# DJATOM/x265-aMod

Hardware: AMD Instinct MI355X
Metric: encoded frames/sec at 1080p & 2160p --preset medium; bit-exact vs CPU ref (higher is better)
Workload: dtype u8

## Files before the change

### include/x265amd.h

```cpp
#ifndef X265AMD_H
#define X265AMD_H

#include <stdint.h>
#include <stddef.h>

#ifdef __cplusplus
extern "C" {
#endif

#ifndef X265AMD_DEPTH
#define X265AMD_DEPTH 8
#endif
#if X265AMD_DEPTH > 8
typedef uint16_t x265amd_pixel;
#else
typedef uint8_t x265amd_pixel;
#endif

#define X265AMD_OK 0
#define X265AMD_EINVAL (-1)
#define X265AMD_EHIP (-2)
#define X265AMD_ENOMEM (-3)

int x265amd_bit_depth(void);
// ... 33 lines not shown
void x265amd_cpy2Dto1D_shr(int cu, int16_t* dst, const int16_t* src, intptr_t srcStride, int shift);
void x265amd_cpy1Dto2D_shl(int cu, int16_t* dst, const int16_t* src, intptr_t dstStride, int shift);
void x265amd_cpy1Dto2D_shr(int cu, int16_t* dst, const int16_t* src, intptr_t dstStride, int shift);
uint32_t x265amd_copy_cnt(int cu, int16_t* coeff, const int16_t* residual, intptr_t resiStride);
int x265amd_count_nonzero(int cu, const int16_t* quantCoeff);

void x265amd_dct(int cu, const int16_t* src, int16_t* dst, intptr_t srcStride);
void x265amd_lowpass_dct(int cu, const int16_t* src, int16_t* dst, intptr_t srcStride);
void x265amd_idct(int cu, const int16_t* src, int16_t* dst, intptr_t dstStride);
void x265amd_dst4x4(const int16_t* src, int16_t* dst, intptr_t srcStride);
void x265amd_idst4x4(const int16_t* src, int16_t* dst, intptr_t dstStride);
uint32_t x265amd_quant(const int16_t* coef, const int32_t* quantCoeff, int32_t* deltaU, int16_t* qCoef, int qBits, int add, int numCoeff);
uint32_t x265amd_nquant(const int16_t* coef, const int32_t* quantCoeff, int16_t* qCoef, int qBits, int add, int numCoeff);
void x265amd_dequant_normal(const int16_t* quantCoef, int16_t* coef, int num, int scale, int shift);
void x265amd_dequant_scaling(const int16_t* src, const int32_t* dequantCoef, int16_t* dst, int num, int mcqp_miper, int shift);

void x265amd_intra_pred(int cu, int mode, pixel_t_* dst, intptr_t dstStride, const pixel_t_* srcPix, int bFilter);
void x265amd_intra_filter(int cu, const pixel_t_* references, pixel_t_* filtered);
void x265amd_intra_allangs(int cu, pixel_t_* dst, pixel_t_* refPix, pixel_t_* filtPix, int bLuma);

void x265amd_luma_hpp(int part, const pixel_t_* src, intptr_t srcStride, pixel_t_* dst, intptr_t dstStride, int coeffIdx);
void x265amd_luma_hps(int part, const pixel_t_* src, intptr_t srcStride, int16_t* dst, intptr_t dstStride, int coeffIdx, int isRowExt);
void x265amd_luma_vpp(int part, const pixel_t_* src, intptr_t srcStride, pixel_t_* dst, intptr_t dstStride, int coeffIdx);
void x265amd_luma_vps(int part, const pixel_t_* src, intptr_t srcStride, int16_t* dst, intptr_t dstStride, int coeffIdx);
void x265amd_luma_vsp(int part, const int16_t* src, intptr_t srcStride, pixel_t_* dst, intptr_t dstStride, int coeffIdx);
void x265amd_luma_vss(int part, const int16_t* src, intptr_t srcStride, int16_t* dst, intptr_t dstStride, int coeffIdx);
void x265amd_luma_hvpp(int part, const pixel_t_* src, intptr_t srcStride, pixel_t_* dst, intptr_t dstStride, int idxX, int idxY);
void x265amd_luma_p2s(int part, const pixel_t_* src, intptr_t srcStride, int16_t* dst, intptr_t dstStride);
void x265amd_chroma_hpp(int csp, int part, const pixel_t_* src, intptr_t srcStride, pixel_t_* dst, intptr_t dstStride, int coeffIdx);
void x265amd_chroma_hps(int csp, int part, const pixel_t_* src, intptr_t srcStride, int16_t* dst, intptr_t dstStride, int coeffIdx, int isRowExt);
void x265amd_chroma_vpp(int csp, int part, const pixel_t_* src, intptr_t srcStride, pixel_t_* dst, intptr_t dstStride, int coeffIdx);
void x265amd_chroma_vps(int csp, int part, const pixel_t_* src, intptr_t srcStride, int16_t* dst, intptr_t dstStride, int coeffIdx);
void x265amd_chroma_vsp(int csp, int part, const int16_t* src, intptr_t srcStride, pixel_t_* dst, intptr_t dstStride, int coeffIdx);
void x265amd_chroma_vss(int csp, int part, const int16_t* src, intptr_t srcStride, int16_t* dst, intptr_t dstStride, int coeffIdx);
void x265amd_chroma_p2s(int csp, int part, const pixel_t_* src, intptr_t srcStride, int16_t* dst, intptr_t dstStride);

enum x265amd_op
{
    X265AMD_OP_SAD = 0, X265AMD_OP_SAD_X3, X265AMD_OP_SAD_X4, X265AMD_OP_SATD, X265AMD_OP_SA8D, X265AMD_OP_SSE_PP,
    X265AMD_OP_SSE_SS, X265AMD_OP_SSD_S, X265AMD_OP_PSY_COST_PP, X265AMD_OP_VAR, X265AMD_OP_CHROMA_SATD, X265AMD_OP_CHROMA_SA8D,
    X265AMD_OP_SUB_PS = 32, X265AMD_OP_ADD_PS, X265AMD_OP_PIXELAVG_PP, X265AMD_OP_ADDAVG, X265AMD_OP_WEIGHT_PP, X265AMD_OP_WEIGHT_SP,
    X265AMD_OP_SCALE2D_64TO32, X265AMD_OP_SCALE1D_128TO64, X265AMD_OP_TRANSPOSE, X265AMD_OP_CPY2DTO1D_SHL, X265AMD_OP_CPY2DTO1D_SHR,
    X265AMD_OP_CPY1DTO2D_SHL, X265AMD_OP_CPY1DTO2D_SHR, X265AMD_OP_COPY_CNT, X265AMD_OP_COUNT_NONZERO,
    X265AMD_OP_DCT = 64, X265AMD_OP_IDCT, X265AMD_OP_DST4, X265AMD_OP_IDST4, X265AMD_OP_QUANT, X265AMD_OP_NQUANT,
    X265AMD_OP_DEQUANT_NORMAL, X265AMD_OP_DEQUANT_SCALING,
    X265AMD_OP_INTRA_PRED = 96, X265AMD_OP_INTRA_FILTER, X265AMD_OP_INTRA_ALLANGS,
    X265AMD_OP_IP_HPP = 128, X265AMD_OP_IP_HPS, X265AMD_OP_IP_VPP, X265AMD_OP_IP_VPS, X265AMD_OP_IP_VSP, X265AMD_OP_IP_VSS,
    X265AMD_OP_IP_HVPP, X265AMD_OP_IP_P2S
};
#define X265AMD_OP_LOWPASS_DCT 80

typedef struct x265amd_job
{
    int32_t op;
    int32_t size;
    int32_t p[6];
    uint64_t a, b, c, d;
    uint64_t e[2];
    int32_t sa, sb, sc, sd;
} x265amd_job;

int x265amd_run_jobs(void* stream, const x265amd_job* d_jobs, int n, int family);


enum { X265AMD_ME_DIA = 0, X265AMD_ME_HEX = 1, X265AMD_ME_UMH = 2, X265AMD_ME_STAR = 3, X265AMD_ME_SEA = 4, X265AMD_ME_FULL = 5 };
#define X265AMD_ME_MAX_CAND 12

typedef struct x265amd_me_job
{
    int16_t x, y;
    uint8_t w, h;
    uint8_t method, subme;
    uint8_t qp, num_cand;
    int16_t merange;
    int16_t mvmin[2], mvmax[2];
    int16_t mvp[2];
    int16_t mvc[X265AMD_ME_MAX_CAND][2];
} x265amd_me_job;

typedef struct x265amd_me_group
{
    int32_t first_job, num_jobs;
    int32_t ref;
    int16_t win_x, win_y;
    int16_t win_w, win_h;
    int16_t fenc_x, fenc_y;
} x265amd_me_group;

typedef struct x265amd_me_result { int16_t mv[2]; int32_t cost; } x265amd_me_result;

typedef struct x265amd_me_ctx x265amd_me_ctx;
x265amd_me_ctx* x265amd_me_open(void);
void x265amd_me_close(x265amd_me_ctx* ctx);
const uint16_t* x265amd_me_host_mvcost(x265amd_me_ctx* ctx, int qp);
int x265amd_me_plan(const x265amd_me_job* jobs, int n, int ref, int max_win_w, int max_win_h, x265amd_me_group* groups, int32_t* order);
int x265amd_me_search(x265amd_me_ctx* ctx, void* stream, const x265amd_pixel* d_fenc, const uint64_t* d_refs, intptr_t stride,
                      const x265amd_me_group* d_groups, int num_groups, const x265amd_me_job* d_jobs, x265amd_me_result* d_out,
                      int max_win_w, int max_win_h, int flags, const uint64_t* d_chroma, intptr_t cstride);
#define X265AMD_ME_FLAG_STAR 1
#define X265AMD_ME_FLAG_CHROMA 2
#define X265AMD_ME_FLAG_FULL 4
#define X265AMD_ME_CHROMA_SATD 0x80

typedef struct x265amd_tu_job
{
    uint64_t fenc, pred;
    uint64_t coeff;
    uint64_t resi;
    uint64_t recon;
    int32_t fenc_stride, pred_stride, resi_stride, recon_stride;
    uint8_t log2_tr_size, ttype, intra, dir_mode, slice_type, qp_scaled, sign_hide;
    uint8_t flags;
} x265amd_tu_job;
#define X265AMD_TU_LOWPASS 1

typedef struct x265amd_tu_result
{
    uint32_t num_sig;
    uint32_t zero_energy, nz_energy;
    uint32_t reserved;
    uint64_t zero_dist, nz_dist;
} x265amd_tu_result;

int x265amd_tu_chain(void* stream, const x265amd_tu_job* d_jobs, int n, x265amd_tu_result* d_out);

#define X265AMD_CTX_COUNT 157
#define X265AMD_CTX_STRIDE 160
typedef struct x265amd_est_bits { int32_t v[184]; } x265amd_est_bits;
typedef struct x265amd_tu_rdoq
{
    uint64_t est_bits;
    int64_t lambda2;
    int32_t lambda;
    int32_t psy_rdoq_scale;
    uint8_t rdoq_level;
    uint8_t tu_depth;
    uint8_t reserved[6];
} x265amd_tu_rdoq;

typedef struct x265amd_intra_tu_job
{
    x265amd_tu_job tu;
    uint64_t nb;
    uint64_t avail;
    int32_t nb_stride;
    uint8_t strong_smoothing;
    uint8_t reserved[11];
} x265amd_intra_tu_job;
int x265amd_intra_tu_chain(void* stream, const x265amd_intra_tu_job* d_jobs, const x265amd_tu_rdoq* d_rdoq, int n, x265amd_tu_result* d_out);

typedef struct x265amd_intra_pu_job
{
    x265amd_intra_tu_job tmpl;
    uint64_t lambda;
    uint32_t rbits, mpm_base;
    uint32_t slot_pixels, slot_coeffs;
    uint8_t preds[3], max_cand;
    uint8_t reserved[4];
} x265amd_intra_pu_job;
typedef struct x265amd_intra_pu_out { int32_t sa8d[35]; uint32_t num_cand; uint8_t modes[16]; } x265amd_intra_pu_out;
int x265amd_intra_pu(void* stream, const x265amd_intra_pu_job* d_job, x265amd_intra_pu_out* d_out, x265amd_tu_result* d_res);

typedef struct x265amd_intra_nxn_job
{
    x265amd_intra_tu_job tmpl[4];
    uint64_t pred_dst[4], layer_dst[4];
    uint64_t lambda, lambda2, psy_scale;
    uint64_t frac_start[4];
    uint32_t scan_frac;
    uint32_t slot_pixels, slot_coeffs;
    uint8_t left_mode[2], above_mode[2];
    uint8_t ctx[X265AMD_CTX_STRIDE];
    uint8_t max_cand, do_chroma;
    uint8_t num_units, unit_log2;
    uint8_t no_picture;
    uint8_t pick_sa8d;
    uint8_t reserved[2];
    x265amd_intra_tu_job ctmpl[2];
    uint64_t crecon_dst[2];
    uint64_t recon_dst[4];
    uint64_t levels_dst, clevels_dst;
    uint64_t chain;
    uint64_t peer;
    uint64_t cu_out;
    uint64_t peer_recon[3];
    uint64_t win_dst[3];
    uint64_t chain_token;
    uint8_t chain_role;
    uint8_t chain_first;
    uint8_t mode_src[4];
    uint8_t chain_index;
    uint8_t reserved2;
    int64_t rdoq_lambda2[3];
    int32_t rdoq_lambda[3];
    int32_t psy_rdoq_scale;
    uint8_t rdoq_level;
    uint8_t rdoq_tu_depth;
    uint8_t rdoq_general;
    uint8_t reserved3[5];
} x265amd_intra_nxn_job;
typedef struct x265amd_intra_chain { uint64_t seq, frac; uint8_t ctx[X265AMD_CTX_STRIDE]; uint8_t mode[4][4]; } x265amd_intra_chain;
typedef struct x265amd_intra_nxn_out
{
    uint8_t mode[4], num_cand[4]; x265amd_tu_result res[4]; int16_t levels[4][16];
    uint32_t psy_energy;
    uint32_t res_energy;
    uint32_t chroma_best, chroma_reserved;
    x265amd_tu_result cres[2];
    int16_t clevels[2][16];
} x265amd_intra_nxn_out;
typedef struct x265amd_intra_peer
{
    x265amd_intra_nxn_out out; uint64_t ready;
    uint8_t fctx[X265AMD_CTX_STRIDE]; uint64_t ffrac, fmv;
} x265amd_intra_peer;
typedef struct x265amd_intra_cu8_result
{
    uint64_t rd_cost, frac_bits;
    uint64_t other_cost;
    uint32_t total_bits, mv_bits, coeff_bits, psy_energy, res_energy, luma_dist, chroma_dist;
    uint32_t status;
    uint8_t part_size;
    uint8_t chroma_dir;
    uint8_t cbf_u, cbf_v, luma_dir[4], cbf_y[4], reserved[4];
    uint8_t ctx[X265AMD_CTX_STRIDE];
    int16_t levels[96];
} x265amd_intra_cu8_result;
int x265amd_intra_nxn(void* stream, const x265amd_intra_nxn_job* d_job, x265amd_intra_nxn_out* d_out);
int x265amd_intra_nxn_list(void* stream, const x265amd_intra_nxn_job* d_jobs, int n, size_t stride_bytes, x265amd_intra_nxn_out* d_out);

int x265amd_tu_chain_rdoq(void* stream, const x265amd_tu_job* d_jobs, const x265amd_tu_rdoq* d_rdoq, int n, x265amd_tu_result* d_out);
void x265amd_rdoq_lambda(int qpScaled, int64_t* lambda2, int32_t* lambda);

void x265amd_entropy_reset(int sliceType, int qp, uint8_t* ctx);
typedef struct x265amd_est_job { uint64_t ctx, est; uint8_t log2_tr_size, is_luma, reserved[6]; } x265amd_est_job;
int x265amd_est_bit(void* stream, const x265amd_est_job* d_jobs, int n);
typedef struct x265amd_coeff_bits_job
{
    uint64_t coeff, ctx_in, ctx_out;
    uint8_t log2_tr_size, ttype, intra, dir_mode, sign_hide, reserved[3];
} x265amd_coeff_bits_job;
int x265amd_coeff_bits(void* stream, const x265amd_coeff_bits_job* d_jobs, int n, uint64_t* d_bits);
int x265amd_coeff_bits_wave(void* stream, const x265amd_coeff_bits_job* d_jobs, int n, uint64_t* d_bits);
typedef struct x265amd_intra_cu_bits_job
{
    uint8_t ctx[X265AMD_CTX_STRIDE];
    uint64_t frac_bits;
    uint8_t log2_cu, nxn, code_part_size, inter_slice, skip_ctx, sign_hide, chroma_dir, cbf_u, cbf_v;
    uint8_t subdiv_flag;
    uint8_t reserved[2];
    uint8_t luma_dir[4], cbf_y[4], preds[4][3];
    uint64_t lev_y[4], lev_u, lev_v;
} x265amd_intra_cu_bits_job;
typedef struct x265amd_intra_cu_bits_out { uint8_t ctx[X265AMD_CTX_STRIDE]; uint64_t frac_bits, mv_frac, skip_frac; } x265amd_intra_cu_bits_out;
int x265amd_intra_cu_bits(void* stream, const x265amd_intra_cu_bits_job* d_jobs, int n, x265amd_intra_cu_bits_out* d_out);
void x265amd_est_bit_host(const uint8_t* ctx, int log2TrSize, int isLuma, int32_t* est);
uint64_t x265amd_code_coeff_bits(const int16_t* coeff, int log2TrSize, int ttype, int bIntra, int dirMode, int signHide, uint8_t* ctx);
uint32_t x265amd_transform_tu_rdoq(const x265amd_pixel* fenc, intptr_t fencStride, const int16_t* resi, intptr_t resiStride, int16_t* coeff,
                                   int log2TrSize, int ttype, int bIntra, int dirMode, int sliceType, int qpScaled, int signHide,
                                   int tuDepth, int rdoqLevel, int psyRdoqScale, const int32_t* est);

uint32_t x265amd_transform_tu(const x265amd_pixel* fenc, intptr_t fencStride, const int16_t* resi, intptr_t resiStride, int16_t* coeff,
                              int log2TrSize, int ttype, int bIntra, int dirMode, int sliceType, int qpScaled, int signHide);
void x265amd_invtransform_tu(int16_t* resi, intptr_t resiStride, const int16_t* coeff, int log2TrSize, int ttype, int bIntra, int qpScaled, uint32_t numSig);

typedef struct x265amd_intra_job
{
    uint64_t recon;
    uint64_t fenc;
    uint64_t avail;
    int32_t recon_stride, fenc_stride;
    uint8_t log2_tr_size;
    uint8_t strong_smoothing;
    uint8_t reserved[6];
} x265amd_intra_job;

int x265amd_intra_scan(void* stream, const x265amd_intra_job* d_jobs, int n, int32_t* d_sa8d, x265amd_pixel* d_neighbours);

typedef struct x265amd_weight { int16_t w, o; uint8_t denom, present; } x265amd_weight;
typedef struct x265amd_mc_job
{
    uint64_t dst_y, dst_u, dst_v;
    int32_t dst_stride, dst_cstride;
    int16_t x, y;
    int16_t cu_x, cu_y;
    uint8_t w, h;
    int8_t ref0, ref1;
    int16_t mv0[2], mv1[2];
    uint8_t slice_type;
    uint8_t flags;
    struct { int16_t w, o; uint8_t denom, present; } wp[2][3];
    uint8_t metric;
    uint8_t chroma_cost;
    uint8_t reserved[4];
} x265amd_mc_job;

int x265amd_motion_compensation(void* stream, const uint64_t* d_planes, intptr_t stride, intptr_t cstride, int pic_w, int pic_h,
                                const x265amd_mc_job* d_jobs, int n);

int x265amd_inter_cost(void* stream, const uint64_t* d_planes, intptr_t stride, intptr_t cstride, int pic_w, int pic_h,
                       const x265amd_mc_job* d_jobs, int n, const uint64_t* d_fenc_planes, intptr_t fenc_stride, intptr_t fenc_cstride,
                       uint32_t* d_cost);

int x265amd_extend_pic_border(void* stream, x265amd_pixel* d_pic, intptr_t stride, int width, int height, int marginX, int marginY);
int x265amd_extend_border_rows(void* stream, x265amd_pixel* d_pic, intptr_t stride, int width, int height, int marginX, int marginY, int y_begin, int y_end);
int x265amd_extend_border_band(void* stream, x265amd_pixel* d_pic, intptr_t stride, int width, int height, int marginX, int marginY, int y_begin, int y_end,
                               int x_begin, int x_end, int left, int right);
int x265amd_extend_border_band_420(void* stream, x265amd_pixel* d_y, x265amd_pixel* d_u, x265amd_pixel* d_v, intptr_t stride, intptr_t cstride, int width, int height,
                                   int marginX, int marginY, int y_begin, int y_end, int x_begin, int x_end, int left, int right);
int x265amd_weight_plane(void* stream, const x265amd_pixel* d_src, x265amd_pixel* d_dst, intptr_t stride, int width, int height,
                         int marginX, int marginY, int inputWeight, int inputOffset, int log2WeightDenom);

#ifndef X265AMD_SURFACE_DEFINED
#define X265AMD_SURFACE_DEFINED
typedef struct x265amd_surface {
    const void* planes[3];
    int32_t stride[3];
    int32_t bitDepth;
    int32_t layout;
    int32_t clipMin, clipMax;
    int32_t reserved;
} x265amd_surface;
#endif
int x265amd_ingest_picture(void* stream, const x265amd_surface* d_src, int srcW, int srcH,
                           x265amd_pixel* d_pic , int W, int H, int marginX, int marginY);
int x265amd_ingest_model(const x265amd_surface* src, int srcW, int srcH, x265amd_pixel* pic, int W, int H, int marginX, int marginY);

#define X265AMD_DB_INTRA 1
#define X265AMD_DB_CBF 2
#define X265AMD_DB_BYPASS 4
#define X265AMD_DB_TU_LEFT 8
#define X265AMD_DB_PU_LEFT 16
#define X265AMD_DB_TU_TOP 32
#define X265AMD_DB_PU_TOP 64
typedef struct x265amd_slice_info x265amd_slice_info;
typedef struct x265amd_mvpred_info x265amd_mvpred_info;
typedef struct x265amd_cu_unit x265amd_cu_unit;
typedef struct x265amd_mv_unit x265amd_mv_unit;
typedef struct x265amd_deblock_unit { uint8_t flags; int8_t qp; int8_t ref[2]; int16_t mv[2][2]; } x265amd_deblock_unit;
int x265amd_deblock_picture(void* stream, x265amd_pixel* d_y, x265amd_pixel* d_u, x265amd_pixel* d_v, intptr_t stride, intptr_t cstride,
                            int width, int height, const x265amd_deblock_unit* d_units, int betaOffsetDiv2, int tcOffsetDiv2,
                            int cbQpOffset, int crQpOffset, int bypassEnabled, int passes);

int x265amd_deblock_rows(void* stream, x265amd_pixel* d_y, x265amd_pixel* d_u, x265amd_pixel* d_v, intptr_t stride, intptr_t cstride,
                         int width, int height, const x265amd_deblock_unit* d_units, int betaOffsetDiv2, int tcOffsetDiv2,
                         int cbQpOffset, int crQpOffset, int bypassEnabled, int passes, int y4_begin, int y4_end);
int x265amd_deblock_rows_cols(void* stream, x265amd_pixel* d_y, x265amd_pixel* d_u, x265amd_pixel* d_v, intptr_t stride, intptr_t cstride,
                              int width, int height, const x265amd_deblock_unit* d_units, int betaOffsetDiv2, int tcOffsetDiv2,
                              int cbQpOffset, int crQpOffset, int bypassEnabled, int passes, int y4_begin, int y4_end, int ctu_col_begin, int ctu_col_end);

int x265amd_deblock_units(const x265amd_slice_info* si, const x265amd_mvpred_info* info, const x265amd_cu_unit* units, const x265amd_mv_unit* motion,
                          x265amd_deblock_unit* out);
int x265amd_deblock_units_rows(const x265amd_slice_info* si, const x265amd_mvpred_info* info, const x265amd_cu_unit* units, const x265amd_mv_unit* motion,
                               x265amd_deblock_unit* out, int y4_begin, int y4_end);
int x265amd_deblock_units_rect(const x265amd_slice_info* si, const x265amd_mvpred_info* info, const x265amd_cu_unit* units, const x265amd_mv_unit* motion,
                               x265amd_deblock_unit* out, int y4_begin, int y4_end, int x4_begin, int x4_end);

typedef struct x265amd_sao_ctu
{
    int8_t type[2];
    uint8_t band_pos[3];
    int8_t offset[3][4];
    uint8_t reserved[3];
} x265amd_sao_ctu;
int x265amd_sao_stats(void* stream, const uint64_t rec_planes[3], const uint64_t fenc_planes[3], intptr_t stride, intptr_t cstride,
                      int width, int height, int32_t* d_count, int32_t* d_offset_org);
int x265amd_sao_apply(void* stream, const uint64_t src_planes[3], const uint64_t dst_planes[3], intptr_t stride, intptr_t cstride,
                      int width, int height, const x265amd_sao_ctu* d_params);
int x265amd_sao_stats_rows(void* stream, const uint64_t rec_planes[3], const uint64_t fenc_planes[3], intptr_t stride, intptr_t cstride,
                           int width, int height, int32_t* d_count, int32_t* d_offset_org, int ctu_row_begin, int ctu_row_end);
int x265amd_sao_apply_rows(void* stream, const uint64_t src_planes[3], const uint64_t dst_planes[3], intptr_t stride, intptr_t cstride,
                           int width, int height, const x265amd_sao_ctu* d_params, int ctu_row_begin, int ctu_row_end);
int x265amd_sao_stats_rows_cols(void* stream, const uint64_t rec_planes[3], const uint64_t fenc_planes[3], intptr_t stride, intptr_t cstride,
                                int width, int height, int32_t* d_count, int32_t* d_offset_org, int ctu_row_begin, int ctu_row_end, int ctu_col_begin, int ctu_col_end);
int x265amd_sao_apply_rows_cols(void* stream, const uint64_t src_planes[3], const uint64_t dst_planes[3], intptr_t stride, intptr_t cstride,
                                int width, int height, const x265amd_sao_ctu* d_params, int ctu_row_begin, int ctu_row_end, int x_begin, int x_end);
enum { X265AMD_SAO_NON_DEBLOCK = 1, X265AMD_SAO_EO01_ONLY = 2 };
int x265amd_sao_stats_opt(void* stream, const uint64_t rec_planes[3], const uint64_t fenc_planes[3], intptr_t stride, intptr_t cstride,
                          int width, int height, int32_t* d_count, int32_t* d_offset_org, int flags);
int x265amd_sao_stats_opt_rows(void* stream, const uint64_t rec_planes[3], const uint64_t fenc_planes[3], intptr_t stride, intptr_t cstride,
                               int width, int height, int32_t* d_count, int32_t* d_offset_org, int flags, int ctu_row_begin, int ctu_row_end);
int x265amd_sao_stats_opt_rows_cols(void* stream, const uint64_t rec_planes[3], const uint64_t fenc_planes[3], intptr_t stride, intptr_t cstride,
                                    int width, int height, int32_t* d_count, int32_t* d_offset_org, int flags, int ctu_row_begin, int ctu_row_end, int ctu_col_begin, int ctu_col_end);
int x265amd_sao_stats_pre(void* stream, const uint64_t rec_planes[3], const uint64_t fenc_planes[3], intptr_t stride, intptr_t cstride,
                          int width, int height, int32_t* d_pre_count, int32_t* d_pre_offset_org);
int x265amd_sao_stats_pre_rows(void* stream, const uint64_t rec_planes[3], const uint64_t fenc_planes[3], intptr_t stride, intptr_t cstride,
                               int width, int height, int32_t* d_pre_count, int32_t* d_pre_offset_org, int ctu_row_begin, int ctu_row_end);
int x265amd_sao_stats_model(const void* const rec_planes[3], const void* const fenc_planes[3], const void* const pre_planes[3], intptr_t stride, intptr_t cstride,
                            int width, int height, int flags, int32_t* pre_count, int32_t* pre_offset_org, int32_t* count, int32_t* offset_org);

enum { X265AMD_FILTER_TOP = 0, X265AMD_FILTER_FULL = 1 };
typedef struct x265amd_filter_step { int32_t kind, row, col_begin, col_end, y4_begin, y4_end, rec_y4_end, rec_x4_begin, rec_x4_end; } x265amd_filter_step;
typedef struct x265amd_filter_finish { int32_t row, x_begin, x_end, y_begin, y_end; } x265amd_filter_finish;
int x265amd_filter_plan(int width, int height, const int32_t* analysed, int32_t* done_top, int32_t* done_full, int32_t* pub_x,
                        int min_chunk, int min_chunk_last, int early_top,
                        x265amd_filter_step* steps, int* num_steps, x265amd_filter_finish* finish, int* num_finish);
int x265amd_filter_ready(int width, int height, const int32_t* analysed, const int32_t* done_top, const int32_t* done_full,
                         int min_chunk, int min_chunk_last, int early_top);

enum { X265AMD_MODE_NONE = 0, X265AMD_MODE_INTER = 1, X265AMD_MODE_INTRA = 2, X265AMD_MODE_SKIP = 3 };
typedef struct x265amd_cu_unit
{
    uint8_t depth;
    uint8_t pred_mode;
    uint8_t part_size;
    uint8_t tu_depth;
    uint8_t luma_dir, chroma_dir;
    uint8_t merge_flag, inter_dir;
    uint8_t cbf[3];
    uint8_t tq_bypass;
    int8_t qp;
    int8_t ref_idx[2];
    uint8_t mvp_idx[2];
    uint8_t reserved;
    int16_t mvd[2][2];
} x265amd_cu_unit;
typedef struct x265amd_slice_info
{
    int32_t pic_width, pic_height;
    int32_t slice_type;
    int32_t slice_qp;
    int32_t num_ref_idx[2];
    int32_t max_num_merge_cand;
    int32_t use_dqp, max_cu_dqp_depth;
    int32_t sign_hide, tq_bypass_enabled;
    int32_t wpp;
    int32_t max_cu_depth;
    int32_t max_amp_depth;
    int32_t tu_log2_min, tu_log2_max;
    int32_t tu_max_depth_inter, tu_max_depth_intra;
} x265amd_slice_info;
#define X265AMD_SLICE_SIGN_HIDE 1
#define X265AMD_SLICE_LOWPASS_DCT 0x100
typedef struct x265amd_cabac x265amd_cabac;
x265amd_cabac* x265amd_cabac_open(const x265amd_slice_info* si, x265amd_cu_unit* units, int bits_only);
void x265amd_cabac_close(x265amd_cabac*);
void x265amd_cabac_set_contexts(x265amd_cabac*, const uint8_t* ctx);
void x265amd_cabac_get_contexts(const x265amd_cabac*, uint8_t* ctx);
int x265amd_cabac_encode_ctu(x265amd_cabac*, int ctu_addr, const int16_t* coeffY, const int16_t* coeffU, const int16_t* coeffV);
uint64_t x265amd_cabac_frac_bits(const x265amd_cabac*);
uint64_t x265amd_cabac_ctu_bits(const x265amd_cabac*);
size_t x265amd_cabac_finish_slice(x265amd_cabac*, uint8_t* out, size_t cap);

typedef struct x265amd_mv_unit { uint8_t pred_mode, inter_dir; int8_t ref_idx[2]; int16_t mv[2][2]; } x265amd_mv_unit;
typedef struct x265amd_mvpred_info
{
    int32_t pic_width, pic_height;
    int32_t is_inter_b, num_ref_idx[2], max_num_merge_cand;
    int32_t temporal_mvp;
    int32_t col_from_l0, check_ldc;
    int32_t poc, ref_poc[2][16];
    int32_t col_poc, col_ref_poc[2][16];
} x265amd_mvpred_info;
typedef struct x265amd_merge_cand { int16_t mv[2][2]; int8_t ref_idx[2]; uint8_t dir; uint8_t reserved; } x265amd_merge_cand;
int x265amd_merge_candidates(const x265amd_mvpred_info* info, const x265amd_mv_unit* cur, const x265amd_mv_unit* col, int cu_x, int cu_y, int log2_cu_size,
                             int part_size, int pu_idx, x265amd_merge_cand* out);
int x265amd_amvp_candidates(const x265amd_mvpred_info* info, const x265amd_mv_unit* cur, const x265amd_mv_unit* col, int cu_x, int cu_y, int log2_cu_size,
                            int part_size, int pu_idx, int list, int ref_idx, int16_t amvp[2][2], int16_t mvc[12][2]);

typedef struct x265amd_inter_search_params
{
    int32_t search_method, subpel_refine, search_range;
    int32_t qp;
    int32_t chroma_mc;
    int32_t ref_pic[2][16];
    int32_t frame_parallel;
    int32_t lazy_sync;
    int32_t lowres_blocks_in_row;
    int32_t me_pic[2][16];
    int32_t weighted;
    x265amd_weight wp[2][16][3];
    uint64_t lowres_mvs[2][16];
} x265amd_inter_search_params;
typedef struct x265amd_inter_cu { int16_t x, y; uint8_t log2_size, part_size; uint8_t reserved[2]; } x265amd_inter_cu;
typedef struct x265amd_pu_result
{
    uint8_t merge_flag, inter_dir;
    int8_t ref_idx[2];
    uint8_t mvp_idx[2];
    uint8_t reserved[2];
    int16_t mv[2][2], mvd[2][2];
} x265amd_pu_result;
int x265amd_pred_inter_search(x265amd_me_ctx* me, void* stream, const x265amd_mvpred_info* info, const x265amd_inter_search_params* sp,
                              x265amd_mv_unit* cur, const x265amd_mv_unit* col, const uint64_t* h_planes, int num_pics, intptr_t stride, intptr_t cstride,
                              const x265amd_inter_cu* cus, int n, x265amd_pu_result* out, int32_t* bits_out, uint64_t d_pred, size_t pred_bytes_per_cu);

typedef struct x265amd_me_detail
{
    int16_t mv[2][2], mvp[2][2];
    int16_t amvp[2][2][2];
    int8_t ref[2]; uint8_t mvp_idx[2];
    uint32_t bits[2], cost[2], mv_cost[2];
    uint32_t list_sel_bits[3];
} x265amd_me_detail;
int x265amd_pred_inter_search_ex(x265amd_me_ctx* me, void* stream, const x265amd_mvpred_info* info, const x265amd_inter_search_params* sp,
                                 x265amd_mv_unit* cur, const x265amd_mv_unit* col, const uint64_t* h_planes, int num_pics, intptr_t stride, intptr_t cstride,
                                 const x265amd_inter_cu* cus, int n, x265amd_pu_result* out, int32_t* bits_out, uint64_t d_pred, size_t pred_bytes_per_cu,
                                 x265amd_me_detail* detail, const uint32_t* ref_masks);

typedef struct x265amd_rd_params
{
    double psy_rd;
    int32_t rd_level;
    int32_t strong_intra_smoothing;
    int32_t rdoq_level;
    int32_t psy_rdoq_scale;
    int32_t fast_intra;
    int32_t limit_tu;
} x265amd_rd_params;
typedef struct x265amd_rd_cu
{
    int16_t x, y;
    uint8_t log2_size;
    int8_t qp;
    uint8_t reserved[2];
    uint64_t frac_bits;
    uint8_t ctx[X265AMD_CTX_STRIDE];
} x265amd_rd_cu;
typedef struct x265amd_rd_result
{
    uint64_t rd_cost, distortion;
    uint64_t frac_bits;
    uint32_t total_bits, mv_bits, coeff_bits, psy_energy, luma_distortion, chroma_distortion, res_energy, reserved;
    uint8_t ctx[X265AMD_CTX_STRIDE];
} x265amd_rd_result;
int x265amd_inter_residual_rd(void* stream, const x265amd_slice_info* si, const x265amd_rd_params* rp, x265amd_cu_unit* units,
                              const uint64_t* h_src, intptr_t stride, intptr_t cstride, const x265amd_rd_cu* cus, int n,
                              x265amd_cu_unit* cu_units, uint64_t d_pred, uint64_t d_recon, size_t tile_bytes,
                              x265amd_rd_result* out, int16_t* coeff_out);

typedef struct x265amd_cu_measure
{
    uint64_t sse[3]; uint32_t psy, sa8d;
    uint32_t sa8d_luma;
    uint32_t src_mean, src_homo, reserved;
} x265amd_cu_measure;
int x265amd_measure_tiles(void* stream, const uint64_t* h_src, intptr_t stride, intptr_t cstride, const x265amd_rd_cu* cus, int n,
                          uint64_t d_tiles, size_t tile_bytes, x265amd_cu_measure* out);
int x265amd_measure_tile_list(void* stream, const uint64_t* h_src, intptr_t stride, intptr_t cstride, const x265amd_rd_cu* cus, int n,
                              const uint64_t* tile_addrs, x265amd_cu_measure* out);
size_t x265amd_inter_rd_scratch_bytes(void);
int x265amd_inter_rd_plan(const x265amd_slice_info* si, const x265amd_rd_cu* cus, int n, const x265amd_cu_unit* cu_units, const uint64_t* src,
                          intptr_t stride, intptr_t cstride, uint64_t pred, size_t tile_bytes, uint64_t scratch, x265amd_tu_job* jobs_out, int cap);
int x265amd_inter_rd_walk(const x265amd_slice_info* si, const x265amd_rd_params* rp, x265amd_cu_unit* units, const x265amd_rd_cu* cus, int n,
                          x265amd_cu_unit* cu_units, const x265amd_tu_result* res, const int16_t* levels, size_t levels_stride_bytes,
                          const x265amd_cu_measure* zero_meas, uint8_t* sel, x265amd_rd_result* out, int16_t* coeff_out);
void x265amd_inter_rd_finish(const x265amd_slice_info* si, const x265amd_rd_params* rp, const x265amd_rd_cu* cus, int n,
                             const x265amd_cu_measure* final_meas, x265amd_rd_result* out);

int x265amd_skip_rd(void* stream, const x265amd_slice_info* si, const x265amd_rd_params* rp, x265amd_cu_unit* units,
                    const uint64_t* h_src, intptr_t stride, intptr_t cstride, const x265amd_rd_cu* cus, int n,
                    x265amd_cu_unit* cu_units, uint64_t d_pred, uint64_t d_recon, size_t tile_bytes, x265amd_rd_result* out);
int x265amd_skip_rd_host(const x265amd_slice_info* si, const x265amd_rd_params* rp, x265amd_cu_unit* units, const x265amd_rd_cu* cus, int n,
                         x265amd_cu_unit* cu_units, const x265amd_cu_measure* meas, x265amd_rd_result* out);

int x265amd_intra_in_inter(void* stream, const x265amd_slice_info* si, const x265amd_rd_params* rp, x265amd_cu_unit* units,
                           const uint64_t* h_src, const uint64_t* h_rec, intptr_t stride, intptr_t cstride, const x265amd_rd_cu* cu,
                           x265amd_cu_unit* cu_units, uint64_t d_pred, uint64_t d_recon, x265amd_rd_result* out, int16_t* coeff_out, uint64_t* info);

int x265amd_check_intra(void* stream, const x265amd_slice_info* si, const x265amd_rd_params* rp, x265amd_cu_unit* units,
                        const uint64_t* h_src, const uint64_t* h_rec, intptr_t stride, intptr_t cstride, const x265amd_rd_cu* cu, int part_size,
                        x265amd_cu_unit* cu_units, uint64_t d_pred, uint64_t d_recon, x265amd_rd_result* out, int16_t* coeff_out);

typedef struct x265amd_analysis_params
{
    double psy_rd;
    int32_t rd_level, early_skip, rskip, limit_refs, b_intra, rect, amp, limit_modes;
    int32_t strong_intra_smoothing;
    int32_t use_sao;
    int32_t rdoq_level, psy_rdoq_scale;
    int32_t fast_intra, limit_tu;
} x265amd_analysis_params;
typedef struct x265amd_cu_stat { uint32_t count[4]; uint32_t pad[2]; uint64_t avg_cost[4]; } x265amd_cu_stat;
typedef struct x265amd_ctu_result { uint64_t rd_cost, distortion, frac_bits; uint32_t total_bits, reserved; uint8_t ctx[X265AMD_CTX_STRIDE]; } x265amd_ctu_result;
int x265amd_compress_ctu_inter(x265amd_me_ctx* me, void* stream, const x265amd_mvpred_info* info, const x265amd_inter_search_params* sp,
                               const x265amd_slice_info* si, const x265amd_analysis_params* ap, x265amd_cu_unit* units, x265amd_mv_unit* cur,
                               const x265amd_mv_unit* col, const uint8_t* ref_depth, const int8_t* ref_qp0, const uint64_t* h_planes, int num_pics,
                               intptr_t stride, intptr_t cstride, x265amd_cu_stat* cu_stat, int ctu_addr, const uint8_t* ctx_in, uint64_t frac_in,
                               int16_t* coeff_out, x265amd_ctu_result* out);

int x265amd_analyse_frame(x265amd_me_ctx* me, void* stream, const x265amd_mvpred_info* info, const x265amd_inter_search_params* sp,
                          const x265amd_slice_info* si, const x265amd_analysis_params* ap, x265amd_cu_unit* units, x265amd_mv_unit* cur,
                          const x265amd_mv_unit* col, const uint8_t* ref_depth, const int8_t* ref_qp0, const uint64_t* h_planes, int num_pics,
                          intptr_t stride, intptr_t cstride, x265amd_cu_stat* cu_stat, int16_t* coeff_out, x265amd_ctu_result* results,
                          uint8_t* slice_data, size_t cap, uint32_t* substream_sizes, int* num_substreams);

typedef struct x265amd_slice_header
{
    int32_t nal_unit_type;
    int32_t temporal_id_plus1;
    int32_t first_in_access_unit;
    int32_t slice_type, poc, last_idr_poc, log2_max_poc_lsb;
    int32_t rps_idx, num_rps_in_sps;
    int32_t num_negative, num_positive, delta_poc[16], used[16];
    int32_t temporal_mvp_enabled, use_sao, sao_luma, sao_chroma, selective_sao;
    int32_t num_ref_idx[2], num_ref_idx_default[2], col_from_l0, col_ref_idx, max_num_merge_cand;
    int32_t slice_qp, pps_init_qp;
    int32_t chroma_qp_offsets_present, cb_qp_offset, cr_qp_offset;
    int32_t deblocking_disabled;
    int32_t slfase_flag;
    int32_t wpp;
    int32_t weighted_pred;
    int32_t luma_log2_weight_denom, chroma_log2_weight_denom;
    int32_t weighted_bipred;
    x265amd_weight wp[2][16][3];
} x265amd_slice_header;
// ... 174 lines not shown
```

### x265-amod_amd/csrc/device_queue.hip

```cpp
#define XA_SERVER_BYTES
#include "x265amd_dev.h"
#include "x265amd_host.h"
#include "xa_queue.h"
#include "xa_fiber.h"
#ifndef XA_PREFETCH_SLOT
#define XA_PREFETCH_SLOT 0
#endif
__shared__ unsigned long long xa_stage_acc[22];
__shared__ long long xa_stage_prev;
__shared__ unsigned long long xa_nxn_acc[4][10];
__shared__ unsigned long long xa_chain_acc[8];
__shared__ long long xa_chain_prev;
__shared__ long long xa_nxn_prev;
__shared__ int xa_nxn_kind;
#ifdef XA_PROFILE_STAGES
#define XA_STAGE(k) do { if (threadIdx.x == 0) { const long long t_ = wall_clock64(); xa_stage_acc[k] += (unsigned long long)(t_ - xa_stage_prev); xa_stage_prev = t_; } } while (0)
#define XA_CHAIN_START() do { if (threadIdx.x == 0) xa_chain_prev = wall_clock64(); } while (0)
#define XA_CHAIN(k) do { if (threadIdx.x == 0) { const long long t_ = wall_clock64(); xa_chain_acc[k] += (unsigned long long)(t_ - xa_chain_prev); xa_chain_prev = t_; } } while (0)
#define XA_NXN_START(kind) do { if (threadIdx.x == 0) { xa_nxn_kind = (kind); xa_nxn_prev = wall_clock64(); } } while (0)
#define XA_NXN(k) do { if (threadIdx.x == 0) { const long long t_ = wall_clock64(); xa_nxn_acc[xa_nxn_kind][k] += (unsigned long long)(t_ - xa_nxn_prev); xa_nxn_prev = t_; } } while (0)
#define XA_LINK_START()
#define XA_LINK(k)
#define XA_LINK_T(k)
#else
#define XA_STAGE(k)
#define XA_CHAIN_START()
#define XA_CHAIN(k)
#define XA_NXN_START(kind)
#define XA_NXN(k)
#define XA_LINK_START() do { if (threadIdx.x == 0) xa_chain_prev = wall_clock64(); } while (0)
#define XA_LINK(k) do { if (threadIdx.x == 0) xa_chain_acc[k] += (unsigned long long)(wall_clock64() - xa_chain_prev); } while (0)
#define XA_LINK_T(k) do { if (threadIdx.x == 0) { const long long t_ = wall_clock64(); xa_chain_acc[k] += (unsigned long long)(t_ - xa_chain_prev); xa_chain_prev = t_; } } while (0)
#endif
#include "tu_dev.h"
#include "intra_dev.h"
#include "mc_dev.h"
#include "me_dev.h"
#include "measure_dev.h"
#include "entropy_dev.h"
#include "intra_pu_dev.h"
#define XA_CHAIN_DEVICE
#include "inter_chain_dev.h"
#define XA_SEARCH_DEVICE
#include "inter_search_dev.h"
#include <immintrin.h>
#include <signal.h>
#include <atomic>
#include <chrono>
#include <condition_variable>
#include <mutex>
#include <string.h>
#include <thread>
#include <vector>

extern __shared__ __attribute__((aligned(16))) char xa_smem[];
__shared__ int xa_q_index;
__device__ uint64_t* xa_dbg_area[256];
#define XA_DBG(c, slot, v) do { if (((c).reserved & 2) && (threadIdx.x & 63) == 0) __hip_atomic_store(&xa_dbg_area[xa_q_index][((threadIdx.x >> 6) * 8 + (slot)) & 63], (uint64_t)(v), __ATOMIC_RELAXED, __HIP_MEMORY_SCOPE_SYSTEM); } while (0)

XA_DEV uint64_t xa_sys_load(const uint64_t* p) { return __hip_atomic_load(p, __ATOMIC_RELAXED, __HIP_MEMORY_SCOPE_SYSTEM); }
XA_DEV void xa_sys_store(uint64_t* p, uint64_t v) { __hip_atomic_store(p, v, __ATOMIC_RELAXED, __HIP_MEMORY_SCOPE_SYSTEM); }

template<bool HOSTDST> XA_DEV void block_copy(char* dst, const char* src, size_t bytes, int tid, int nthr)
{
    if (HOSTDST)
    {
        if ((((uintptr_t)dst | (uintptr_t)src) & 7) == 0)
        {
            const size_t n8 = bytes >> 3;
            for (size_t i = tid; i < n8; i += nthr) xa_sys_store(reinterpret_cast<uint64_t*>(dst) + i, reinterpret_cast<const uint64_t*>(src)[i]);
            for (size_t i = (n8 << 3) + tid; i < bytes; i += nthr) __hip_atomic_store(dst + i, src[i], __ATOMIC_RELAXED, __HIP_MEMORY_SCOPE_SYSTEM);
        }
        else
            for (size_t i = tid; i < bytes; i += nthr) __hip_atomic_store(dst + i, src[i], __ATOMIC_RELAXED, __HIP_MEMORY_SCOPE_SYSTEM);
        return;
    }
    if ((((uintptr_t)dst | (uintptr_t)src) & 15) == 0)
    {
        const size_t n16 = bytes >> 4;
        for (size_t i = tid; i < n16; i += nthr) reinterpret_cast<uint4*>(dst)[i] = reinterpret_cast<const uint4*>(src)[i];
        for (size_t i = (n16 << 4) + tid; i < bytes; i += nthr) dst[i] = src[i];
    }
    else
        for (size_t i = tid; i < bytes; i += nthr) dst[i] = src[i];
}

XA_DEV void block_copy_rects(const XaArgsRects& r, int tid, int nthr)
{
    for (int k = 0; k < r.n; k++)
    {
        const pixel* src = reinterpret_cast<const pixel*>(r.src[k]);
        pixel* dst = reinterpret_cast<pixel*>(r.dst[k]);
        const int w = r.w[k], total = w * r.h[k];
        for (int i = tid; i < total; i += nthr)
        {
            const int y = i / w, x = i - y * w;
            dst[(size_t)y * r.dst_stride[k] + x] = src[(size_t)y * r.src_stride[k] + x];
        }
    }
}

XA_DEV void xa_op_copy(const XaCmd& c, int tid)
{
    constexpr int NT = 64 * XA_SERVER_WAVES;
    const int lane = tid & 63, wv = tid >> 6;
    (void)NT; (void)lane; (void)wv;
    const bool serial = (c.reserved & 1) != 0;
    (void)serial;
    {
        const XaArgsCopy& a = *reinterpret_cast<const XaArgsCopy*>(c.args);
        block_copy<false>(reinterpret_cast<char*>(a.dst), reinterpret_cast<const char*>(a.src), a.bytes, tid, NT);
        if (tid == 0) XA_BYTES(2 * a.bytes);
    }
}

XA_DEV void xa_op_copy2d(const XaCmd& c, int tid)
{
    constexpr int NT = 64 * XA_SERVER_WAVES;
    const int lane = tid & 63, wv = tid >> 6;
    (void)NT; (void)lane; (void)wv;
    const bool serial = (c.reserved & 1) != 0;
    (void)serial;
    {
        const XaArgsCopy2D& a = *reinterpret_cast<const XaArgsCopy2D*>(c.args);
        for (uint64_t y = wv; y < a.height; y += XA_SERVER_WAVES)
            block_copy<false>(reinterpret_cast<char*>(a.dst + y * a.dpitch), reinterpret_cast<const char*>(a.src + y * a.spitch), a.width, lane, 64);
        if (tid == 0) XA_BYTES(2 * a.width * a.height);
    }
}

XA_DEV void xa_op_fill(const XaCmd& c, int tid)
{
    constexpr int NT = 64 * XA_SERVER_WAVES;
    const int lane = tid & 63, wv = tid >> 6;
    (void)NT; (void)lane; (void)wv;
    const bool serial = (c.reserved & 1) != 0;
    (void)serial;
    {
        const XaArgsFill& a = *reinterpret_cast<const XaArgsFill*>(c.args);
        char* d = reinterpret_cast<char*>(a.dst);
        for (size_t i = tid; i < a.bytes; i += NT) d[i] = (char)a.value;
        if (tid == 0) XA_BYTES(a.bytes);
    }
}

XA_DEV void xa_op_copy_rects(const XaCmd& c, int tid)
{
    constexpr int NT = 64 * XA_SERVER_WAVES;
    const int lane = tid & 63, wv = tid >> 6;
    (void)NT; (void)lane; (void)wv;
    const bool serial = (c.reserved & 1) != 0;
    (void)serial;
        block_copy_rects(*reinterpret_cast<const XaArgsRects*>(c.args), tid, NT);
        if (tid == 0)
        {
            const XaArgsRects& r = *reinterpret_cast<const XaArgsRects*>(c.args);
            unsigned long long b = 0;
            for (int k = 0; k < r.n; k++) b += 2ull * (unsigned)r.w[k] * (unsigned)r.h[k] * sizeof(pixel);
            XA_BYTES(b);
        }
}

__device__ __noinline__ void xa_op_mc(const XaCmd& c, int tid)
{
    const int lane = tid & 63, wv = tid >> 6;
    const XaArgsMc a = *reinterpret_cast<const XaArgsMc*>(c.args);
    if (c.op == XA_OP_MC_COST)
    {
        for (int ji = wv; ji < a.n; ji += XA_SERVER_WAVES) wave_mc_job<true>(a, ji, lane);
        return;
    }
    const int wpj = a.n >= XA_SERVER_WAVES ? 1 : XA_SERVER_WAVES / a.n, perRound = XA_SERVER_WAVES / wpj;
    for (int base = 0; base < a.n; base += perRound)
    {
        const int ji = base + wv / wpj, sub = wv % wpj;
        if (wv < perRound * wpj && ji < a.n) wave_mc_job<false>(a, ji, sub * 64 + lane, wpj * 64);
    }
}

__device__ __noinline__ void xa_op_cu_measure(const XaCmd& c, int tid)
{
    constexpr int NT = 64 * XA_SERVER_WAVES;
    const int lane = tid & 63, wv = tid >> 6;
    const XaArgsJobs4 a = *reinterpret_cast<const XaArgsJobs4*>(c.args);
    const CuMeasureJob* jobs = reinterpret_cast<const CuMeasureJob*>(a.a);
    CuMeasure* out = reinterpret_cast<CuMeasure*>(a.b);
    static_assert(sizeof(CuMeasureLds) <= XA_SERVER_LDS, "LDS budget");
    if (a.n <= 2 * XA_SERVER_WAVES)
    {
        CuMeasureLds& s = *reinterpret_cast<CuMeasureLds*>(xa_smem);
        for (int ji = 0; ji < a.n; ji++)
        {
            const CuMeasureJob j = xa_ld_record(jobs + ji);
            block_cu_measure_job(j, out + ji, s, tid, NT);
        }
        return;
    }
    constexpr int W = (XA_SERVER_LDS / (64 * 64 * (int)sizeof(pixel))) < XA_SERVER_WAVES ? (XA_SERVER_LDS / (64 * 64 * (int)sizeof(pixel))) : XA_SERVER_WAVES;
    if (wv < W)
        for (int ji = wv; ji < a.n; ji += W) wave_cu_measure_job(jobs, ji, out, reinterpret_cast<pixel*>(xa_smem) + wv * 64 * 64, lane);
}

__device__ __noinline__ void xa_op_tu_chain(const XaCmd& c, int tid)
{
    constexpr int NT = 64 * XA_SERVER_WAVES;
    const int lane = tid & 63, wv = tid >> 6;
    const XaArgsJobs4 a = *reinterpret_cast<const XaArgsJobs4*>(c.args);
    static_assert((XA_SERVER_WAVES + 1) * sizeof(TuLds) + 64 <= XA_SERVER_LDS, "LDS budget");
    const x265amd_tu_job* jobs = reinterpret_cast<const x265amd_tu_job*>(a.a);
    x265amd_tu_result* out = reinterpret_cast<x265amd_tu_result*>(a.c);
    TuLds& big = reinterpret_cast<TuLds*>(xa_smem)[XA_SERVER_WAVES];
    unsigned long long* red = reinterpret_cast<unsigned long long*>(xa_smem + (XA_SERVER_WAVES + 1) * sizeof(TuLds));
    const bool few = a.n <= 4 * XA_SERVER_WAVES;
    if (few)
        for (int ji = 0; ji < a.n; ji++)
            if (__hip_atomic_load(&jobs[ji].log2_tr_size, __ATOMIC_RELAXED, __HIP_MEMORY_SCOPE_SYSTEM) >= 4) block_tu_chain_job(jobs, ji, out, big, red, tid, NT);
    TuLds& s = reinterpret_cast<TuLds*>(xa_smem)[wv];
    int k = 0;
    for (int ji = 0; ji < a.n; ji++)
    {
        if (few && __hip_atomic_load(&jobs[ji].log2_tr_size, __ATOMIC_RELAXED, __HIP_MEMORY_SCOPE_SYSTEM) >= 4) continue;
        if ((k++ % XA_SERVER_WAVES) == wv) wave_tu_chain_job<false>(jobs, nullptr, ji, out, s, nullptr, lane);
    }
}

__device__ __noinline__ void xa_op_tu_chain_rdoq(const XaCmd& c, int tid)
{
    constexpr int NT = 64 * XA_SERVER_WAVES;
    const int lane = tid & 63, wv = tid >> 6;
    (void)NT; (void)lane; (void)wv;
    const bool serial = (c.reserved & 1) != 0;
    (void)serial;
    {
        const XaArgsJobs4& a = *reinterpret_cast<const XaArgsJobs4*>(c.args);
        constexpr int W = XA_SERVER_LDS / (int)(sizeof(TuLds) + sizeof(RdoqLds));
        static_assert(W >= 1, "LDS budget");
        if (wv < W)
        {
            TuLds& s = reinterpret_cast<TuLds*>(xa_smem)[wv];
            char* rdoqLds = xa_smem + W * sizeof(TuLds) + wv * sizeof(RdoqLds);
            for (int ji = serial ? (wv ? a.n : 0) : wv; ji < a.n; ji += serial ? 1 : W)
                wave_tu_chain_job<true>(reinterpret_cast<const x265amd_tu_job*>(a.a), reinterpret_cast<const x265amd_tu_rdoq*>(a.b), ji, reinterpret_cast<x265amd_tu_result*>(a.c), s, rdoqLds, lane);
        }
    }
}

__device__ __noinline__ void xa_op_intra_tu_chain(const XaCmd& c, int tid)
{
    constexpr int NT = 64 * XA_SERVER_WAVES;
    const int lane = tid & 63, wv = tid >> 6;
    (void)NT; (void)lane; (void)wv;
    const bool serial = (c.reserved & 1) != 0;
    (void)serial;
    {
        const XaArgsJobs4& a = *reinterpret_cast<const XaArgsJobs4*>(c.args);
        static_assert(XA_SERVER_WAVES * (sizeof(TuLds) + sizeof(IntraTuLds)) <= XA_SERVER_LDS, "LDS budget");
        TuLds& s = reinterpret_cast<TuLds*>(xa_smem)[wv];
        IntraTuLds& ip = reinterpret_cast<IntraTuLds*>(xa_smem + XA_SERVER_WAVES * sizeof(TuLds))[wv];
        for (int ji = serial ? (wv ? a.n : 0) : wv; ji < a.n; ji += serial ? 1 : XA_SERVER_WAVES)
            wave_intra_tu_chain_job<false>(reinterpret_cast<const x265amd_intra_tu_job*>(a.a), nullptr, ji, reinterpret_cast<x265amd_tu_result*>(a.c), s, ip, nullptr, lane);
    }
}

__device__ __noinline__ void xa_op_intra_tu_chain_rdoq(const XaCmd& c, int tid)
{
    constexpr int NT = 64 * XA_SERVER_WAVES;
    const int lane = tid & 63, wv = tid >> 6;
    (void)NT; (void)lane; (void)wv;
    const bool serial = (c.reserved & 1) != 0;
    (void)serial;
    {
        const XaArgsJobs4& a = *reinterpret_cast<const XaArgsJobs4*>(c.args);
        constexpr int W = XA_SERVER_LDS / (int)(sizeof(TuLds) + sizeof(IntraTuLds) + sizeof(RdoqLds));
        static_assert(W >= 1, "LDS budget");
        if (wv < W)
        {
            TuLds& s = reinterpret_cast<TuLds*>(xa_smem)[wv];
            IntraTuLds& ip = reinterpret_cast<IntraTuLds*>(xa_smem + W * sizeof(TuLds))[wv];
            char* rdoqLds = xa_smem + W * (sizeof(TuLds) + sizeof(IntraTuLds)) + wv * sizeof(RdoqLds);
            for (int ji = serial ? (wv ? a.n : 0) : wv; ji < a.n; ji += serial ? 1 : W)
                wave_intra_tu_chain_job<true>(reinterpret_cast<const x265amd_intra_tu_job*>(a.a), reinterpret_cast<const x265amd_tu_rdoq*>(a.b), ji,
                                              reinterpret_cast<x265amd_tu_result*>(a.c), s, ip, rdoqLds, lane);
        }
    }
}

__device__ __noinline__ void xa_op_intra_scan(const XaCmd& c, int tid)
{
    constexpr int NT = 64 * XA_SERVER_WAVES;
    const int lane = tid & 63, wv = tid >> 6;
    const XaArgsJobs4 a = *reinterpret_cast<const XaArgsJobs4*>(c.args);
    static_assert(XA_SERVER_WAVES * sizeof(IntraLds) <= XA_SERVER_LDS && sizeof(IntraScanLds) <= XA_SERVER_LDS, "LDS budget");
    const x265amd_intra_job* jobs = reinterpret_cast<const x265amd_intra_job*>(a.a);
    int32_t* out = reinterpret_cast<int32_t*>(a.b);
    pixel* nbOut = reinterpret_cast<pixel*>(a.c);
    if (a.n <= 2 * XA_SERVER_WAVES)
    {
        IntraScanLds& s = *reinterpret_cast<IntraScanLds*>(xa_smem);
        for (int ji = 0; ji < a.n; ji++)
        {
            const x265amd_intra_job j = xa_ld_record(jobs + ji);
            block_intra_scan_job(j, out + (size_t)ji * 35, nbOut ? nbOut + (size_t)ji * 2 * 129 : nullptr, s, tid, NT);
        }
        return;
    }
    IntraLds& s = reinterpret_cast<IntraLds*>(xa_smem)[wv];
    for (int ji = wv; ji < a.n; ji += XA_SERVER_WAVES) wave_intra_scan_job(jobs, ji, out, nbOut, s, lane);
}

__device__ __noinline__ void xa_op_est_bit(const XaCmd& c, int tid)
{
    constexpr int NT = 64 * XA_SERVER_WAVES;
    const int lane = tid & 63, wv = tid >> 6;
    (void)NT; (void)lane; (void)wv;
    const bool serial = (c.reserved & 1) != 0;
    (void)serial;
    {
        const XaArgsJobs4& a = *reinterpret_cast<const XaArgsJobs4*>(c.args);
        for (int ji = serial ? (wv ? a.n : 0) : wv; ji < a.n; ji += serial ? 1 : XA_SERVER_WAVES) wave_est_bit_job(reinterpret_cast<const x265amd_est_job*>(a.a), ji, lane);
    }
}

__device__ __noinline__ void xa_op_intra_pu(const XaCmd& c, int tid)
{
    const XaArgsJobs4 a = *reinterpret_cast<const XaArgsJobs4*>(c.args);
    static_assert(sizeof(IntraScanLds) <= XA_SERVER_LDS && XA_SERVER_WAVES * (sizeof(TuLds) + sizeof(IntraTuLds)) <= XA_SERVER_LDS, "LDS budget");
    block_intra_pu(reinterpret_cast<const x265amd_intra_pu_job*>(a.a), reinterpret_cast<x265amd_intra_pu_out*>(a.b), reinterpret_cast<x265amd_tu_result*>(a.c), xa_smem, tid,
                   64 * XA_SERVER_WAVES);
}

__device__ __noinline__ void xa_op_intra_nxn(const XaCmd& c, int tid)
{
    static_assert(XA_SERVER_WAVES * (sizeof(TuLds) + sizeof(IntraTuLds)) + sizeof(Nxn4Lds) <= XA_SERVER_LDS, "LDS budget (block_intra_nxn: chromaAhead)");
    const XaArgsJobs4 a = *reinterpret_cast<const XaArgsJobs4*>(c.args);
    for (int i = 0; i < (a.n > 0 ? a.n : 1); i++)
        block_intra_nxn(reinterpret_cast<const x265amd_intra_nxn_job*>(a.a + (uint64_t)i * a.c), reinterpret_cast<x265amd_intra_nxn_out*>(a.b), xa_smem, tid, 64 * XA_SERVER_WAVES, XA_SERVER_LDS);
}

__device__ __noinline__ void xa_op_inter_chain(const XaCmd& c, int tid)
// ... 1054 lines not shown
```

### x265-amod_amd/csrc/inter_chain_dev.h

```cpp
#ifndef X265AMD_INTER_CHAIN_DEV_H
#define X265AMD_INTER_CHAIN_DEV_H
#include <stdint.h>

struct alignas(16) XaMapUnit { uint8_t pred_mode, inter_dir; int8_t ref_idx[2]; int16_t mv[2][2]; uint8_t depth, pad[3]; };

struct XaChainNode { int16_t x, y; uint8_t log2, flags, next, parent; };
enum { XA_CHAIN_END = 0, XA_CHAIN_NOTSKIP = 1, XA_CHAIN_GUARD = 2 };
enum { XA_CHAIN_MAX_NODES = 85 };

struct XaChainCuOut
{
    uint32_t node; uint8_t cand, dir; int8_t ref_idx[2];
    int16_t mv[2][2];
    x265amd_cu_measure meas;
};
struct XaChainStop
{
    uint32_t valid, node;
    uint8_t cand, dir; int8_t ref_idx[2]; int16_t mv[2][2];
    uint8_t cbf[3], reserved0;
    uint32_t total_bits, mv_bits, coeff_bits, psy_energy, sa8d, sa8d_luma;
    uint64_t rd_cost, luma_dist, chroma_dist, frac;
    x265amd_cu_measure meas;
    uint8_t ctx[X265AMD_CTX_STRIDE];
    int16_t levels[1024 + 2 * 256];
};
struct alignas(8) XaChainStopHead
{
    uint32_t valid, node; uint8_t cand, dir; int8_t ref_idx[2]; int16_t mv[2][2]; uint8_t cbf[3], reserved0;
    uint32_t total_bits, mv_bits, coeff_bits, psy_energy, sa8d, sa8d_luma; uint64_t rd_cost, luma_dist, chroma_dist, frac; x265amd_cu_measure meas;
};
static_assert(sizeof(XaChainStopHead) == offsetof(XaChainStop, ctx), "the stop record's head");
struct XaChainOut { uint32_t count, stop_node, reason, reserved; uint64_t frac; uint64_t ticks[8]; uint8_t ctx[X265AMD_CTX_STRIDE]; XaChainStop stop; XaChainCuOut cu[XA_CHAIN_MAX_NODES]; };

struct alignas(8) XaChainJob
{
    x265amd_mvpred_info info;
    int32_t ref_pic[2][16];
    uint64_t planes;
    uint64_t cur, col;
    uint64_t tiles; uint64_t tile_bytes;
    uint64_t out;
    uint64_t nodes;
    int32_t stride, cstride, num_pics, w4;
    int32_t start, end, num_nodes;
    int32_t tiles_per_depth, cand_tile0, split_recon_tile;
    int32_t skip_recon_tile, merge_recon_tile, chain64_off;
    int32_t frame_parallel, search_range, chroma_sa8d, slice_type, qp_luma, qp_chroma, tu_log2_max;
    int32_t guard_on, guard_r0, guard_r1, guard_need;
    int32_t ctu_x, ctu_y, tu_flags;
    uint64_t lambda;
    uint64_t lambda2;
    uint32_t psy_rd;
    int32_t rd_level, sign_hide, max_cu_depth, dbg;
    uint64_t scratch;
    uint64_t frac;
    uint8_t ctx[X265AMD_CTX_STRIDE];
    int32_t use_dqp, max_dqp_depth;
    int32_t first_qp;
    int32_t previous_qp;
    int32_t prev_qp;
    int32_t dqp_reserved;
    struct QpSet { uint64_t lambda, lambda2; uint32_t psy_rd; int32_t qp_luma, qp_chroma, qp; } qps[5];
    int8_t last_src[4];
    int8_t last_val[4], left_val[4], above_val[4];
    uint8_t anc_flags[4];
    uint8_t dqp_pad[4];
};

#ifdef XA_CHAIN_DEVICE

struct ChainCand { int16_t mv[2][2]; int8_t ref_idx[2]; uint8_t dir, valid; };

struct ChainLds
{
    XaChainJob job;
    XaChainNode nodes[XA_CHAIN_MAX_NODES + 3];
    x265amd_mc_job mc[5];
    CuMeasureJob mj;
    x265amd_cu_measure meas[5];
    ChainCand cand[5];
    int nc, stop, best, anyLevel, count, skipWins;
    unsigned int acc[5][3][16];
    unsigned long long red[XA_SERVER_WAVES];
    x265amd_tu_job tu[12];
    x265amd_tu_result tr[12];
    uint64_t frac;
    uint8_t ctx[X265AMD_CTX_STRIDE], ctxS[X265AMD_CTX_STRIDE], ctxB[X265AMD_CTX_STRIDE], ctxD[X265AMD_CTX_STRIDE], ctxQ[X265AMD_CTX_STRIDE];
    uint64_t fracS, fracD;
    uint32_t rdBits[3], rdPsy, rdCbf[3], rdPad; uint64_t rdCost, rdLuma, rdChroma;
    uint32_t step[256];
    unsigned long long ticks[8]; long long tprev;
    uint8_t used[XA_CHAIN_MAX_NODES + 3];
    int firstQp, dqp, dqpTwice;
    int qgVal[4]; uint32_t qgDone;
};
#define XA_CHAIN_HEADER 8192
#define XA_CHAIN_T(k) do { if (tid == 0) { const long long t_ = wall_clock64(); S.ticks[k] += (unsigned long long)(t_ - S.tprev); S.tprev = t_; } } while (0)

XA_DEV XaMapUnit chain_ld_unit(const XaMapUnit* p)
{
    union { XaMapUnit u; uint64_t w[2]; } v;
    v.w[0] = __hip_atomic_load(reinterpret_cast<const uint64_t*>(p), __ATOMIC_RELAXED, __HIP_MEMORY_SCOPE_SYSTEM);
    v.w[1] = __hip_atomic_load(reinterpret_cast<const uint64_t*>(p) + 1, __ATOMIC_RELAXED, __HIP_MEMORY_SCOPE_SYSTEM);
    return v.u;
}
XA_DEV void chain_st_unit(XaMapUnit* p, const XaMapUnit& u)
{
    union { XaMapUnit u; uint64_t w[2]; } v;
    v.u = u;
    __hip_atomic_store(reinterpret_cast<uint64_t*>(p), v.w[0], __ATOMIC_RELAXED, __HIP_MEMORY_SCOPE_SYSTEM);
    __hip_atomic_store(reinterpret_cast<uint64_t*>(p) + 1, v.w[1], __ATOMIC_RELAXED, __HIP_MEMORY_SCOPE_SYSTEM);
}

XA_DEV unsigned chain_z(int x, int y)
{
    unsigned r = 0;
#pragma unroll
    for (int b = 0; b < 4; b++) r |= (((unsigned)(x >> 2) >> b) & 1u) << (2 * b) | (((unsigned)(y >> 2) >> b) & 1u) << (2 * b + 1);
    return r;
}
XA_DEV bool chain_inter(bool have, const XaMapUnit& u) { return have && (u.pred_mode == X265AMD_MODE_INTER || u.pred_mode == X265AMD_MODE_SKIP); }
XA_DEV bool chain_same_motion(const XaMapUnit& a, const XaMapUnit& b)
{
    if (a.inter_dir != b.inter_dir) return false;
    for (int l = 0; l < 2; l++)
        if ((a.inter_dir & (1 << l)) && (a.mv[l][0] != b.mv[l][0] || a.mv[l][1] != b.mv[l][1] || a.ref_idx[l] != b.ref_idx[l])) return false;
    return true;
}
XA_DEV void chain_scale(int& mx, int& my, int curPOC, int curRefPOC, int colPOC, int colRefPOC)
{
    const int d = colPOC - colRefPOC, b = curPOC - curRefPOC;
    if (d == b) return;
    const int tdb = b < -128 ? -128 : (b > 127 ? 127 : b), tdd = d < -128 ? -128 : (d > 127 ? 127 : d);
    const int x = (0x4000 + abs(tdd / 2)) / tdd;
    int s = (tdb * x + 32) >> 6;
    s = s < -4096 ? -4096 : (s > 4095 ? 4095 : s);
    int ax = (s * mx + 127 + (s * mx < 0)) >> 8, ay = (s * my + 127 + (s * my < 0)) >> 8;
    mx = ax < -32768 ? -32768 : (ax > 32767 ? 32767 : ax); my = ay < -32768 ? -32768 : (ay > 32767 ? 32767 : ay);
}
XA_DEV bool chain_col_mvp(const XaChainJob& J, int& mx, int& my, int list, const XaMapUnit& u, const XaMapUnit& c)
{
    const x265amd_mvpred_info& I = J.info;
    if (u.pred_mode == X265AMD_MODE_NONE || c.pred_mode == X265AMD_MODE_INTRA) return false;
    int cl = I.check_ldc ? list : I.col_from_l0;
    int ci = c.ref_idx[cl];
    if (ci < 0) { cl = !cl; ci = c.ref_idx[cl]; if (ci < 0) return false; }
    mx = c.mv[cl][0]; my = c.mv[cl][1];
    chain_scale(mx, my, I.poc, I.ref_poc[list][0], I.col_poc, I.col_ref_poc[cl][ci]);
    return true;
}

XA_DEV int chain_merge_candidates(const XaChainJob& J, int px, int py, int size, ChainCand* out)
{
    const x265amd_mvpred_info& I = J.info;
    const XaMapUnit* cur = reinterpret_cast<const XaMapUnit*>(J.cur);
    const int maxCand = I.max_num_merge_cand, isB = I.is_inter_b, w4 = J.w4, W = I.pic_width, H = I.pic_height;
    for (int i = 0; i < 5; i++) { out[i].mv[0][0] = out[i].mv[0][1] = out[i].mv[1][0] = out[i].mv[1][1] = 0; out[i].ref_idx[0] = out[i].ref_idx[1] = -1; out[i].dir = 0; out[i].valid = 0; }
    const int ltx = px, lty = py, rtx = px + size - 4, lby = py + size - 4;
    bool hA1 = ltx - 4 >= 0, hB1 = lty - 4 >= 0, hB2 = ltx - 4 >= 0 && lty - 4 >= 0, hB0, hA0;
    {
        hB0 = false;
        if (rtx + 4 < W && lty - 4 >= 0)
        {
            const int ux = rtx & 63, uy = lty & 63;
            if (ux < 60) hB0 = uy ? chain_z(ux, uy) > chain_z(ux + 4, uy - 4) : true;
            else hB0 = uy == 0;
        }
        hA0 = false;
        if (lby + 4 < H && ltx - 4 >= 0)
        {
            const int ux = ltx & 63, uy = lby & 63;
            if (uy < 60) hA0 = ux ? chain_z(ux, uy) > chain_z(ux - 4, uy + 4) : true;
        }
    }
    XaMapUnit a1, b1, b0, a0, b2;
    a1 = b1 = b0 = a0 = b2 = XaMapUnit{};
    if (hA1) a1 = chain_ld_unit(cur + (lby >> 2) * w4 + ((ltx - 4) >> 2));
    if (hB1) b1 = chain_ld_unit(cur + ((lty - 4) >> 2) * w4 + (rtx >> 2));
    if (hB0) b0 = chain_ld_unit(cur + ((lty - 4) >> 2) * w4 + ((rtx + 4) >> 2));
    if (hA0) a0 = chain_ld_unit(cur + ((lby + 4) >> 2) * w4 + ((ltx - 4) >> 2));
    if (hB2) b2 = chain_ld_unit(cur + ((lty - 4) >> 2) * w4 + ((ltx - 4) >> 2));
    XaMapUnit hU = XaMapUnit{}, hC = XaMapUnit{}, cU = XaMapUnit{}, cC = XaMapUnit{};
    bool haveH = false;
    if (I.temporal_mvp)
    {
        const XaMapUnit* col = reinterpret_cast<const XaMapUnit*>(J.col);
        const int rbx = px + size - 4, rby = py + size - 4;
        if (rbx + 4 < W && rby + 4 < H && (rby & 63) < 60)
        {
            const int hx = rbx + 4, hy = rby + 4;
            haveH = true;
            hU = chain_ld_unit(col + (hy >> 2) * w4 + (hx >> 2)); hC = chain_ld_unit(col + ((hy & ~15) >> 2) * w4 + ((hx & ~15) >> 2));
        }
        const int cx = px + size / 2, cy = py + size / 2;
        cU = chain_ld_unit(col + (cy >> 2) * w4 + (cx >> 2)); cC = chain_ld_unit(col + ((cy & ~15) >> 2) * w4 + ((cx & ~15) >> 2));
    }
    int count = 0;
    auto take = [&](const XaMapUnit& u) {
        out[count].dir = u.inter_dir;
        out[count].mv[0][0] = u.mv[0][0]; out[count].mv[0][1] = u.mv[0][1]; out[count].ref_idx[0] = u.ref_idx[0];
        if (isB) { out[count].mv[1][0] = u.mv[1][0]; out[count].mv[1][1] = u.mv[1][1]; out[count].ref_idx[1] = u.ref_idx[1]; }
        return ++count == maxCand;
    };
    const bool availA1 = chain_inter(hA1, a1);
    if (availA1 && take(a1)) return maxCand;
    const bool availB1 = chain_inter(hB1, b1);
    if (availB1 && (!availA1 || !chain_same_motion(a1, b1)) && take(b1)) return maxCand;
    const bool availB0 = chain_inter(hB0, b0);
    if (availB0 && (!availB1 || !chain_same_motion(b1, b0)) && take(b0)) return maxCand;
    const bool availA0 = chain_inter(hA0, a0);
    if (availA0 && (!availA1 || !chain_same_motion(a1, a0)) && take(a0)) return maxCand;
    if (count < 4)
    {
        if (chain_inter(hB2, b2) && (!availA1 || !chain_same_motion(a1, b2)) && (!availB1 || !chain_same_motion(b1, b2)) && take(b2)) return maxCand;
    }
    if (I.temporal_mvp)
    {
        int dir = 0;
        for (int list = 0; list < (isB ? 2 : 1); list++)
        {
            int mx = 0, my = 0;
            bool ok = haveH && chain_col_mvp(J, mx, my, list, hU, hC);
            if (!ok) ok = chain_col_mvp(J, mx, my, list, cU, cC);
            if (ok) { dir |= 1 << list; out[count].mv[list][0] = (int16_t)mx; out[count].mv[list][1] = (int16_t)my; out[count].ref_idx[list] = 0; }
        }
        if (dir) { out[count].dir = (uint8_t)dir; if (++count == maxCand) return maxCand; }
    }
    if (isB)
    {
        const unsigned cutoff = (unsigned)(count * (count - 1));
        unsigned pl0 = 0xEDC984, pl1 = 0xB73621;
        for (unsigned k = 0; k < cutoff; k++, pl0 >>= 2, pl1 >>= 2)
        {
            const int i = pl0 & 3, j = pl1 & 3;
            if ((out[i].dir & 1) && (out[j].dir & 2))
            {
                const int r0 = out[i].ref_idx[0], r1 = out[j].ref_idx[1];
                if (!(I.ref_poc[0][r0] == I.ref_poc[1][r1] && out[i].mv[0][0] == out[j].mv[1][0] && out[i].mv[0][1] == out[j].mv[1][1]))
                {
                    out[count].mv[0][0] = out[i].mv[0][0]; out[count].mv[0][1] = out[i].mv[0][1]; out[count].ref_idx[0] = (int8_t)r0;
                    out[count].mv[1][0] = out[j].mv[1][0]; out[count].mv[1][1] = out[j].mv[1][1]; out[count].ref_idx[1] = (int8_t)r1;
                    out[count].dir = 3;
                    if (++count == maxCand) return maxCand;
                }
            }
        }
    }
    const int numRef = isB ? (I.num_ref_idx[0] < I.num_ref_idx[1] ? I.num_ref_idx[0] : I.num_ref_idx[1]) : I.num_ref_idx[0];
    int r = 0, refcnt = 0;
    while (count < maxCand)
    {
        out[count].dir = isB ? 3 : 1;
        out[count].mv[0][0] = out[count].mv[0][1] = 0; out[count].ref_idx[0] = (int8_t)r;
        if (isB) { out[count].mv[1][0] = out[count].mv[1][1] = 0; out[count].ref_idx[1] = (int8_t)r; }
        count++;
        if (refcnt == numRef - 1) r = 0;
        else { ++r; ++refcnt; }
    }
    return count;
}

XA_DEV bool chain_reach_ok(const XaChainJob& J, int x, int y, int size, const ChainCand& c)
{
    if (!J.guard_on) return true;
    const int W = J.info.pic_width, H = J.info.pic_height;
    for (int l = 0; l < 2; l++)
    {
        if (!(c.dir & (1 << l)) || c.ref_idx[l] < 0) continue;
        const int xmax = (W + 8 - x - 1) << 2, xmin = -((64 + 8 + x - 1) << 2), ymax = (H + 8 - y - 1) << 2, ymin = -((64 + 8 + y - 1) << 2);
        const int mvx = min(xmax, max(xmin, (int)c.mv[l][0])), mvy = min(ymax, max(ymin, (int)c.mv[l][1]));
        const int y0 = y + (mvy >> 2) - 4, y1 = y + size - 1 + (mvy >> 2) + 5, x1 = x + size - 1 + (mvx >> 2) + 5;
        const int need = x1 >= W - 1 ? W : max(0, x1 + 1);
        const int r0 = min(max(y0, 0), H - 1) >> 6, r1 = min(max(y1, 0), H - 1) >> 6;
        if (r0 < J.guard_r0 || r1 > J.guard_r1 || need > J.guard_need) return false;
    }
    return true;
}

template<class V> XA_DEV void chain_copy_rows(pixel* dst, long ds, const pixel* src, int ss, int log2N, int tid, int nthr)
{
    constexpr int U = (int)(sizeof(V) / sizeof(pixel));
    const int N = 1 << log2N, perRow = N / U, total = perRow * N;
    for (int i = tid; i < total; i += nthr)
    {
        const int yy = i / perRow, xx = (i - yy * perRow) * U;
        *reinterpret_cast<V*>(dst + (long)yy * ds + xx) = *reinterpret_cast<const V*>(src + yy * ss + xx);
    }
}
XA_DEV void chain_copy_plane(pixel* dst, long ds, const pixel* src, int ss, int log2N, bool chroma, int tid, int nthr)
{
    if (sizeof(pixel) == 1) { if (chroma) chain_copy_rows<uint32_t>(dst, ds, src, ss, log2N, tid, nthr); else chain_copy_rows<uint64_t>(dst, ds, src, ss, log2N, tid, nthr); }
    else { if (chroma) chain_copy_rows<uint64_t>(dst, ds, src, ss, log2N, tid, nthr); else chain_copy_rows<uint4>(dst, ds, src, ss, log2N, tid, nthr); }
}

template<int TAPS> XA_DEV int chain_pred_tile(const x265amd_mc_job& j, const McSetup& su, const McPlane& P, const pixel* fenc, int fs, int tx, int ty, int lane)
{
    const int x = 8 * tx + (lane & 7), y = 8 * ty + (lane >> 3);
    const int v = mc_one<TAPS>(P, j, su.mode, su.lsel, x, y);
    P.dst[(long)y * P.dstStride + x] = (pixel)v;
    return xa_wave_sum(abs(xa_lane_had8x8((int)fenc[y * fs + x] - v, lane)));
}

template<class G> XA_DEV uint32_t chain_tu_levels(TuLds& s, const pixel* fenc, int fs, const pixel* pred, int ps, int log2N, int ttype, int sliceType, int qpScaled, int lowpass, const G& g)
{
    const int N = 1 << log2N;
    for (int i = g.idx; i < N * N; i += g.step())
    {
        const int y = i >> log2N, x = i & (N - 1);
        s.a[i] = (int16_t)((int)fenc[y * fs + x] - (int)pred[y * ps + x]);
    }
    g.sync();
    return grp_tu_forward(s, log2N, ttype, 0, 0, sliceType, qpScaled, 0, lowpass, g);
}


#if XA_DEPTH < 10
typedef uint32_t chain_sse_t;
#else
typedef uint64_t chain_sse_t;
#endif
XA_DEV uint64_t chain_cost(const XaChainJob& J, chain_sse_t dist, uint32_t bits, uint32_t energy)
{
    return J.psy_rd ? (uint64_t)dist + ((J.lambda * J.psy_rd * energy) >> 24) + (((uint64_t)bits * J.lambda2) >> 8) : (uint64_t)dist + (((uint64_t)bits * J.lambda2 + 128) >> 8);
}
enum { CC_SPLIT = 0, CC_SKIP = 3, CC_MERGE_FLAG = 6, CC_MERGE_IDX = 7, CC_PART_SIZE = 8, CC_PRED_MODE = 12, CC_QT_CBF = 28, CC_QT_ROOT_CBF = 38 };
XA_DEV uint64_t chain_merge_index(uint8_t* ctx, uint32_t idx, uint32_t numCand)
{
    uint64_t f = 0;
    if (numCand > 1)
    {
        f += cb_bin(ctx + CC_MERGE_IDX, idx != 0);
        if (idx != 0) f += 32768ull * (idx - (idx == numCand - 1));
    }
    return f;
}
XA_DEV int chain_split_ctx(const XaChainJob& J, int x, int y, int depth)
{
    const XaMapUnit* cur = reinterpret_cast<const XaMapUnit*>(J.cur);
    int c = 0;
    if (x > 0) { const XaMapUnit l = chain_ld_unit(cur + (y >> 2) * J.w4 + ((x - 4) >> 2)); c += l.pred_mode != X265AMD_MODE_NONE && l.depth > depth; }
    if (y > 0) { const XaMapUnit a = chain_ld_unit(cur + ((y - 4) >> 2) * J.w4 + (x >> 2)); c += a.pred_mode != X265AMD_MODE_NONE && a.depth > depth; }
    return c;
}
XA_DEV int chain_skip_ctx(const XaChainJob& J, int x, int y)
{
    const XaMapUnit* cur = reinterpret_cast<const XaMapUnit*>(J.cur);
    int c = 0;
    if (x > 0) { const XaMapUnit l = chain_ld_unit(cur + (y >> 2) * J.w4 + ((x - 4) >> 2)); c += l.pred_mode == X265AMD_MODE_SKIP; }
    if (y > 0) { const XaMapUnit a = chain_ld_unit(cur + ((y - 4) >> 2) * J.w4 + (x >> 2)); c += a.pred_mode == X265AMD_MODE_SKIP; }
    return c;
}
XA_DEV void chain_split_flag(const XaChainJob& J, uint8_t* ctx, uint64_t& frac, int x, int y, int depth, uint32_t flag)
{
    if (J.rd_level == 2) return;
    frac &= 32767;
    frac += cb_bin(ctx + CC_SPLIT + chain_split_ctx(J, x, y, depth), flag);
}

XA_DEV uint64_t chain_dqp_bits(uint8_t* cx, int dqp)
{
    const uint32_t a = (uint32_t)(dqp < 0 ? -dqp : dqp);
    uint64_t f = cb_bin(&cx[16], a ? 1u : 0u);
    if (a)
    {
        uint32_t sym = a < 5 ? a : 5;
        const bool codeLast = 5 > sym;
        while (--sym) f += cb_bin(&cx[17], 1u);
        if (codeLast) f += cb_bin(&cx[17], 0u);
        if (a >= 5)
        {
            uint32_t symbol = a - 5, count = 0, n = 0;
            while (symbol >= (1u << count)) { n++; symbol -= 1u << count; count++; }
            f += (uint64_t)32768 * (n + 1 + count);
        }
        f += 32768;
    }
    return f;
}
XA_DEV int chain_qg_qp(const ChainLds& S, int j, int hostVal) { return (S.qgDone >> j) & 1u ? S.qgVal[j] : hostVal; }
XA_DEV int chain_ref_qp(const ChainLds& S, int k)
{
    const XaChainJob& J = S.job;
    const int last = J.last_src[k] < 0 ? J.prev_qp : chain_qg_qp(S, J.last_src[k], J.last_val[k]);
    if (J.max_dqp_depth == 0 || k == 0) return last;
    const int l = (k & 1) ? chain_qg_qp(S, k - 1, J.left_val[k]) : last;
    const int a = (k & 2) ? chain_qg_qp(S, k - 2, J.above_val[k]) : last;
    return (l + a + 1) >> 1;
}

XA_DEV void chain_merge_rd(ChainLds& S, int x, int y, int log2, int best, int lane)
{
    const XaChainJob& J = S.job;
    const uint32_t numCand = (uint32_t)J.info.max_num_merge_cand;
    for (int i = lane; i < X265AMD_CTX_STRIDE; i += 64) { const uint8_t v = S.ctx[i]; S.ctxS[i] = v; S.ctxB[i] = v; S.ctxD[i] = v; }
    xa_wave_sync();
    const int skipCtx = chain_skip_ctx(J, x, y);
    const x265amd_cu_measure m0 = S.meas[best];
    const chain_sse_t predDist = (chain_sse_t)((chain_sse_t)m0.sse[0] + (chain_sse_t)m0.sse[1] + (chain_sse_t)m0.sse[2]);
    const uint32_t predPsy = J.psy_rd ? m0.psy : 0;
    uint64_t fS = S.frac & 32767;
    if (lane == 0)
    {
        fS += cb_bin(S.ctxS + CC_SKIP + skipCtx, 1);
        fS += chain_merge_index(S.ctxS, (uint32_t)best, numCand);
        S.fracS = fS;
    }
    xa_wave_sync();
    fS = S.fracS;
    const uint64_t skipCost = chain_cost(J, predDist, (uint32_t)(fS >> 15), predPsy);
    bool anyLevel = false;
    for (int p = 0; p < 3; p++) anyLevel |= S.tr[p].num_sig != 0;
    if (!anyLevel) { if (lane == 0) S.skipWins = 1; return; }
    const int logs[3] = { log2, log2 - 1 < 2 ? 2 : log2 - 1, log2 - 1 < 2 ? 2 : log2 - 1 };
    uint32_t cbf[3], singleBits[3];
    chain_sse_t singleDist[3];
    uint32_t energyY = 0;
    uint64_t fB = S.frac & 32767;
    for (int p = 0; p < 3; p++)
    {
        const x265amd_tu_result r = S.tr[p];
        cbf[p] = r.num_sig != 0;
        const uint32_t latest = (uint32_t)(fB >> 15);
        if (cbf[p]) fB += wave_coeff_bits(S.ctxB, S.ctxB, reinterpret_cast<const int16_t*>(S.tu[p].coeff), logs[p], p, 0, 0, J.sign_hide, S.step, lane);
        xa_wave_sync();
        singleBits[p] = (uint32_t)(fB >> 15) - (p ? latest : 0);
        const chain_sse_t zeroDist = (chain_sse_t)r.zero_dist;
        const uint32_t zeroEnergy = J.psy_rd ? r.zero_energy : 0;
        if (cbf[p])
        {
            const uint8_t st = S.ctxB[CC_QT_CBF + (p ? 2 : 1)];
            const uint32_t nzCbfBits = (uint32_t)(((fB & 32767) + en_bits[st ^ 1]) >> 15), nullBits = (uint32_t)(((fB & 32767) + en_bits[st ^ 0]) >> 15);
            const chain_sse_t nzDist = (chain_sse_t)r.nz_dist;
            const uint32_t nzEnergy = J.psy_rd ? r.nz_energy : 0;
            const uint64_t singleCost = chain_cost(J, nzDist, nzCbfBits + singleBits[p], nzEnergy), nullCost = chain_cost(J, zeroDist, nullBits, zeroEnergy);
            if (nullCost < singleCost) { cbf[p] = 0; singleBits[p] = 0; singleDist[p] = zeroDist; if (!p) energyY = zeroEnergy; }
            else { singleDist[p] = nzDist; if (!p) energyY = nzEnergy; }
        }
        else { singleBits[p] = 0; singleDist[p] = zeroDist; if (!p) energyY = zeroEnergy; }
    }
    chain_sse_t fullDist = 0;
    fullDist += singleDist[0]; fullDist += singleDist[1]; fullDist += singleDist[2];
    const uint64_t fullCost = chain_cost(J, fullDist, singleBits[0] + singleBits[1] + singleBits[2], energyY);
    const uint32_t cbf0Bits = (uint32_t)(((S.frac & 32767) + en_bits[S.ctx[CC_QT_ROOT_CBF] ^ 0]) >> 15);
    if (chain_cost(J, predDist, cbf0Bits, predPsy) < fullCost) cbf[0] = cbf[1] = cbf[2] = 0;
    if (!(cbf[0] | cbf[1] | cbf[2])) { if (lane == 0) S.skipWins = 1; return; }
    uint64_t fD = S.frac & 32767;
    if (lane == 0)
    {
        fD += cb_bin(S.ctxD + CC_SKIP + skipCtx, 0);
        S.rdBits[2] = (uint32_t)(fD >> 15);
        fD += cb_bin(S.ctxD + CC_PRED_MODE, 0);
        fD += cb_bin(S.ctxD + CC_PART_SIZE, 1);
        fD += cb_bin(S.ctxD + CC_MERGE_FLAG, 1);
        fD += chain_merge_index(S.ctxD, (uint32_t)best, numCand);
        S.rdBits[1] = (uint32_t)(fD >> 15) - S.rdBits[2];
        fD += cb_bin(S.ctxD + CC_QT_CBF + 2, cbf[1]);
        fD += cb_bin(S.ctxD + CC_QT_CBF + 2, cbf[2]);
        if (cbf[1] | cbf[2]) fD += cb_bin(S.ctxD + CC_QT_CBF + 1, cbf[0]);
        if (J.use_dqp) fD += chain_dqp_bits(S.ctxD, S.dqp);
    }
    xa_wave_sync();
    fD = __shfl(fD, 0, 64);
    for (int p = 0; p < 3; p++)
    {
        if (cbf[p]) fD += wave_coeff_bits(S.ctxD, S.ctxD, reinterpret_cast<const int16_t*>(S.tu[p].coeff), logs[p], p, 0, 0, J.sign_hide, S.step, lane);
        xa_wave_sync();
    }
    const uint32_t bits0 = (uint32_t)(fD >> 15);
    uint32_t again = 0;
    if (J.use_dqp && S.dqpTwice)
    {
        if (lane == 0) S.fracD = (fD & 32767) + chain_dqp_bits(S.ctxD, S.dqp);
        xa_wave_sync();
        fD = S.fracD;
        again = (uint32_t)(fD >> 15);
    }
    chain_sse_t dist = 0;
    dist += cbf[0] ? (chain_sse_t)S.tr[0].nz_dist : (chain_sse_t)S.tr[0].zero_dist;
    chain_sse_t cd = cbf[1] ? (chain_sse_t)S.tr[1].nz_dist : (chain_sse_t)S.tr[1].zero_dist;
    cd += cbf[2] ? (chain_sse_t)S.tr[2].nz_dist : (chain_sse_t)S.tr[2].zero_dist;
    dist += cd;
    const uint32_t psy = J.psy_rd ? (cbf[0] ? S.tr[0].nz_energy : S.tr[0].zero_energy) : 0;
    const uint32_t totalBits = bits0 + again;
    const uint64_t mergeCost = chain_cost(J, dist, totalBits, psy);
    if (lane == 0)
    {
        S.skipWins = mergeCost < skipCost ? 0 : 1;
        S.fracD = fD; S.rdBits[0] = totalBits; S.rdPad = again; S.rdPsy = psy; S.rdCbf[0] = cbf[0]; S.rdCbf[1] = cbf[1]; S.rdCbf[2] = cbf[2];
        S.rdCost = mergeCost; S.rdLuma = (uint64_t)(dist - cd); S.rdChroma = (uint64_t)cd;
    }
}

XA_DEV void chain_merge_rd64(ChainLds& S, int x, int y, int log2, int best, int lane, uint32_t sig)
{
    const XaChainJob& J = S.job;
    const uint32_t numCand = (uint32_t)J.info.max_num_merge_cand;
    const int L = log2 - 1, C = L - 1;
    for (int i = lane; i < X265AMD_CTX_STRIDE; i += 64) { const uint8_t v = S.ctx[i]; S.ctxS[i] = v; S.ctxB[i] = v; S.ctxD[i] = v; S.ctxQ[i] = v; }
    xa_wave_sync();
    const int skipCtx = chain_skip_ctx(J, x, y);
    const x265amd_cu_measure m0 = S.meas[best];
    const chain_sse_t predDist = (chain_sse_t)((chain_sse_t)m0.sse[0] + (chain_sse_t)m0.sse[1] + (chain_sse_t)m0.sse[2]);
    const uint32_t predPsy = J.psy_rd ? m0.psy : 0;
    uint64_t fS = S.frac & 32767;
    if (lane == 0)
    {
        fS += cb_bin(S.ctxS + CC_SKIP + skipCtx, 1);
        fS += chain_merge_index(S.ctxS, (uint32_t)best, numCand);
        S.fracS = fS;
    }
    xa_wave_sync();
    fS = S.fracS;
    const uint64_t skipCost = chain_cost(J, predDist, (uint32_t)(fS >> 15), predPsy);
    uint32_t cbf[12];
    uint32_t treeBits = 0, treeEnergy = predPsy;
    chain_sse_t treeDist = predDist;
    uint64_t fN = S.frac & 32767;
    for (int q = 0; q < 4; q++)
    {
        uint64_t fB = fN & 32767;
        for (int p = 0; p < 3; p++)
        {
            const int k = p * 4 + q, lg = p ? C : L;
            if (!((sig >> k) & 1)) { cbf[k] = 0; continue; }
            const x265amd_tu_result r = S.tr[k];
            uint32_t c = r.num_sig != 0;
            const uint32_t latest = (uint32_t)(fB >> 15);
            if (c) fB += wave_coeff_bits(S.ctxB, S.ctxB, reinterpret_cast<const int16_t*>(S.tu[k].coeff), lg, p, 0, 0, J.sign_hide, S.step, lane);
            xa_wave_sync();
            uint32_t single = (uint32_t)(fB >> 15) - (p ? latest : 0);
            const chain_sse_t zeroDist = (chain_sse_t)r.zero_dist;
            const uint32_t zeroEnergy = J.psy_rd ? r.zero_energy : 0;
            chain_sse_t dist = zeroDist;
            uint32_t energy = zeroEnergy;
            if (c)
            {
                const uint8_t st = S.ctxB[CC_QT_CBF + (p ? 3 : 0)];
                const uint32_t nzCbfBits = (uint32_t)(((fB & 32767) + en_bits[st ^ 1]) >> 15), nullBits = (uint32_t)(((fB & 32767) + en_bits[st ^ 0]) >> 15);
                const chain_sse_t nzDist = (chain_sse_t)r.nz_dist;
                const uint32_t nzEnergy = J.psy_rd ? r.nz_energy : 0;
                const uint64_t singleCost = chain_cost(J, nzDist, nzCbfBits + single, nzEnergy), nullCost = chain_cost(J, zeroDist, nullBits, zeroEnergy);
                if (nullCost < singleCost) { c = 0; single = 0; }
                else { dist = nzDist; energy = nzEnergy; }
            }
            else single = 0;
            cbf[k] = c;
            treeBits += single; treeDist = treeDist - zeroDist + dist;
            if (!p) treeEnergy = treeEnergy - zeroEnergy + energy;
        }
        for (int i = lane; i < X265AMD_CTX_STRIDE; i += 64) S.ctxB[i] = S.ctxQ[i];
        xa_wave_sync();
        if (lane == 0)
        {
            uint64_t f = fN & 32767;
            f += cb_bin(S.ctxB + CC_QT_CBF + 3, cbf[4 + q]);
            f += cb_bin(S.ctxB + CC_QT_CBF + 3, cbf[8 + q]);
            f += cb_bin(S.ctxB + CC_QT_CBF + 0, cbf[q]);
            S.fracD = f;
        }
        xa_wave_sync();
        fN = S.fracD;
        for (int i = lane; i < X265AMD_CTX_STRIDE; i += 64) S.ctxQ[i] = S.ctxB[i];
        xa_wave_sync();
    }
    const uint32_t ycbf = cbf[0] | cbf[1] | cbf[2] | cbf[3], ucbf = cbf[4] | cbf[5] | cbf[6] | cbf[7], vcbf = cbf[8] | cbf[9] | cbf[10] | cbf[11];
    for (int i = lane; i < X265AMD_CTX_STRIDE; i += 64) S.ctxQ[i] = S.ctx[i];
    xa_wave_sync();
    if (lane == 0)
    {
        uint64_t f = S.frac & 32767;
        f += cb_bin(S.ctxQ + CC_QT_CBF + 2, ucbf);
        f += cb_bin(S.ctxQ + CC_QT_CBF + 2, vcbf);
        for (int q = 0; q < 4; q++)
        {
            if (ucbf) f += cb_bin(S.ctxQ + CC_QT_CBF + 3, cbf[4 + q]);
            if (vcbf) f += cb_bin(S.ctxQ + CC_QT_CBF + 3, cbf[8 + q]);
            f += cb_bin(S.ctxQ + CC_QT_CBF + 0, cbf[q]);
        }
        S.fracD = f;
    }
    xa_wave_sync();
    treeBits += (uint32_t)(S.fracD >> 15);
    const uint64_t treeCost = chain_cost(J, treeDist, treeBits, treeEnergy);
    const uint32_t cbf0Bits = (uint32_t)(((S.frac & 32767) + en_bits[S.ctx[CC_QT_ROOT_CBF] ^ 0]) >> 15);
    if (chain_cost(J, predDist, cbf0Bits, predPsy) < treeCost || !(ycbf | ucbf | vcbf)) { if (lane == 0) S.skipWins = 1; return; }
    uint64_t fD = S.frac & 32767;
    if (lane == 0)
    {
        fD += cb_bin(S.ctxD + CC_SKIP + skipCtx, 0);
        fD += cb_bin(S.ctxD + CC_PRED_MODE, 0);
        fD += cb_bin(S.ctxD + CC_PART_SIZE, 1);
        fD += cb_bin(S.ctxD + CC_MERGE_FLAG, 1);
        fD += chain_merge_index(S.ctxD, (uint32_t)best, numCand);
        fD += cb_bin(S.ctxD + CC_QT_CBF + 2, ucbf);
        fD += cb_bin(S.ctxD + CC_QT_CBF + 2, vcbf);
    }
    bool dqpPending = J.use_dqp != 0;
    for (int q = 0; q < 4; q++)
    {
        const bool any = (cbf[q] | cbf[4 + q] | cbf[8 + q]) != 0;
        if (lane == 0)
        {
            if (ucbf) fD += cb_bin(S.ctxD + CC_QT_CBF + 3, cbf[4 + q]);
            if (vcbf) fD += cb_bin(S.ctxD + CC_QT_CBF + 3, cbf[8 + q]);
            fD += cb_bin(S.ctxD + CC_QT_CBF + 0, cbf[q]);
            if (any && dqpPending) fD += chain_dqp_bits(S.ctxD, S.dqp);
        }
        if (any) dqpPending = false;
        xa_wave_sync();
        fD = __shfl(fD, 0, 64);
        for (int p = 0; p < 3; p++)
        {
            const int k = p * 4 + q;
            if (cbf[k]) fD += wave_coeff_bits(S.ctxD, S.ctxD, reinterpret_cast<const int16_t*>(S.tu[k].coeff), p ? C : L, p, 0, 0, J.sign_hide, S.step, lane);
            xa_wave_sync();
        }
    }
    const uint32_t bits0 = (uint32_t)(fD >> 15);
    uint32_t again = 0;
    if (J.use_dqp && S.dqpTwice)
    {
        if (lane == 0) S.fracD = (fD & 32767) + chain_dqp_bits(S.ctxD, S.dqp);
        xa_wave_sync();
        again = (uint32_t)(S.fracD >> 15);
    }
    chain_sse_t dist = predDist;
    uint32_t psy = predPsy;
    for (int k = 0; k < 12; k++) if (cbf[k]) dist = dist - (chain_sse_t)S.tr[k].zero_dist + (chain_sse_t)S.tr[k].nz_dist;
    if (J.psy_rd) for (int k = 0; k < 4; k++) if (cbf[k]) psy = psy - S.tr[k].zero_energy + S.tr[k].nz_energy;
    const uint64_t mergeCost = chain_cost(J, dist, bits0 + again, psy);
    if (lane == 0) S.skipWins = mergeCost < skipCost ? 0 : 1;
}

XA_DEV void block_inter_chain(const XaChainJob* jobAddr, char* smem, int tid)
{
    constexpr int NT = 64 * XA_SERVER_WAVES;
    const int lane = tid & 63, wv = tid >> 6;
    static_assert(sizeof(ChainLds) <= XA_CHAIN_HEADER, "chain header");
    static_assert(XA_CHAIN_HEADER + sizeof(CuMeasureLds) <= XA_SERVER_LDS && XA_CHAIN_HEADER + (XA_SERVER_WAVES + 1) * sizeof(TuLds) <= XA_SERVER_LDS, "LDS budget");
    ChainLds& S = *reinterpret_cast<ChainLds*>(smem);
    CuMeasureLds& ML = *reinterpret_cast<CuMeasureLds*>(smem + XA_CHAIN_HEADER);
    TuLds* TL = reinterpret_cast<TuLds*>(smem + XA_CHAIN_HEADER);
    __syncthreads();
    {
        const uint64_t* src = reinterpret_cast<const uint64_t*>(jobAddr);
        uint64_t* dst = reinterpret_cast<uint64_t*>(&S.job);
        for (int i = tid; i < (int)(sizeof(XaChainJob) / 8); i += NT) dst[i] = __hip_atomic_load(src + i, __ATOMIC_RELAXED, __HIP_MEMORY_SCOPE_SYSTEM);
    }
    __syncthreads();
    {
        const uint64_t* src = reinterpret_cast<const uint64_t*>(S.job.nodes);
        uint64_t* dst = reinterpret_cast<uint64_t*>(S.nodes);
        for (int i = tid; i < S.job.num_nodes; i += NT) dst[i] = __hip_atomic_load(src + i, __ATOMIC_RELAXED, __HIP_MEMORY_SCOPE_SYSTEM);
        if (tid == 0)
        {
            S.count = 0; S.stop = 0; S.frac = S.job.frac; for (int k = 0; k < 8; k++) S.ticks[k] = 0; S.tprev = wall_clock64();
            S.firstQp = S.job.first_qp; S.qgDone = 0; S.dqp = 0; S.dqpTwice = 0; S.rdPad = 0;
        }
        for (int i = tid; i < 256; i += NT) S.step[i] = en_step.v[i];
        if (tid == 1) __hip_atomic_store(reinterpret_cast<uint64_t*>(&reinterpret_cast<XaChainOut*>(S.job.out)->stop), (uint64_t)0, __ATOMIC_RELAXED, __HIP_MEMORY_SCOPE_SYSTEM);
        for (int i = tid; i < X265AMD_CTX_STRIDE; i += NT) S.ctx[i] = S.job.ctx[i];
    }
    __syncthreads();
    const XaChainJob& J = S.job;
    if (tid == 0)
        for (int p = S.nodes[J.start].parent; p != 255; p = S.nodes[p].parent) S.used[p] = J.anc_flags[(6 - S.nodes[p].log2) & 3];
    const uint64_t* planes = reinterpret_cast<const uint64_t*>(J.planes);
    const uint64_t* srcPlanes = planes + 3 * (J.num_pics - 1);
    const uint64_t* recPlanes = planes + 3 * (J.num_pics - 2);
    XaChainOut* out = reinterpret_cast<XaChainOut*>(J.out);
    const size_t isz = sizeof(pixel);
    int node = J.start, reason = XA_CHAIN_END;
    while (node < J.end)
    {
        const XaChainNode N = S.nodes[node];
        const int flags = S.firstQp >= J.previous_qp ? N.flags & 3 : (N.flags >> 2) & 3;
        if (tid == 0) S.used[node] = (uint8_t)flags;
        if (!(flags & 1)) { node++; continue; }
        const int x = N.x, y = N.y, log2 = N.log2, size = 1 << log2, depth = 6 - log2;
        const int qg = J.max_dqp_depth == 0 ? 0 : ((y - J.ctu_y) >> 5) * 2 + ((x - J.ctu_x) >> 5);
        if (J.use_dqp)
        {
            __syncthreads();
            if (tid == 0)
            {
                const XaChainJob::QpSet q = J.qps[J.max_dqp_depth == 0 || depth == 0 ? 0 : 1 + qg];
                XaChainJob& W = S.job;
                W.lambda = q.lambda; W.lambda2 = q.lambda2; W.psy_rd = q.psy_rd; W.qp_luma = q.qp_luma; W.qp_chroma = q.qp_chroma;
                const int bd = 6 * (X265AMD_DEPTH - 8);
                S.dqp = (q.qp - chain_ref_qp(S, depth == 0 ? 0 : qg) + 78 + bd + (bd / 2)) % (52 + bd) - 26 - (bd / 2);
                S.dqpTwice = depth <= J.max_dqp_depth;
            }
            __syncthreads();
        }
        if (wv == 0)
        {
            ChainCand* cand = S.cand;
            const int nc = chain_merge_candidates(J, x, y, size, cand);
            bool stop = false;
            for (int i = 0; i < nc; i++)
            {
                const bool below = J.frame_parallel && (cand[i].mv[0][1] >= (J.search_range + 1) * 4 || cand[i].mv[1][1] >= (J.search_range + 1) * 4);
                cand[i].valid = !below;
                if (!below && !chain_reach_ok(J, x, y, size, cand[i])) stop = true;
            }
            if (lane == 0)
            {
                S.nc = nc; S.stop = stop ? XA_CHAIN_GUARD : 0; S.anyLevel = 0;
                for (int i = 0; i < nc; i++)
                {
                    x265amd_mc_job& j = S.mc[i];
                    const uint64_t tile = J.tiles + (uint64_t)(depth * J.tiles_per_depth + J.cand_tile0 + i) * J.tile_bytes;
                    j = x265amd_mc_job{};
                    j.dst_y = tile; j.dst_u = tile + 4096 * isz; j.dst_v = j.dst_u + 1024 * isz;
                    j.dst_stride = 64; j.dst_cstride = 32;
                    j.x = (int16_t)x; j.y = (int16_t)y; j.cu_x = (int16_t)x; j.cu_y = (int16_t)y; j.w = (uint8_t)size; j.h = (uint8_t)size;
                    j.ref0 = (cand[i].dir & 1) && cand[i].ref_idx[0] >= 0 ? (int8_t)J.ref_pic[0][cand[i].ref_idx[0]] : -1;
                    j.ref1 = (cand[i].dir & 2) && cand[i].ref_idx[1] >= 0 ? (int8_t)J.ref_pic[1][cand[i].ref_idx[1]] : -1;
                    j.mv0[0] = cand[i].mv[0][0]; j.mv0[1] = cand[i].mv[0][1]; j.mv1[0] = cand[i].mv[1][0]; j.mv1[1] = cand[i].mv[1][1];
                    j.slice_type = (uint8_t)!J.info.is_inter_b; j.flags = 3;
                }
            }
        }
        __syncthreads();
        XA_CHAIN_T(0);
        if (S.stop) { reason = S.stop; break; }
        const int nc = S.nc;
        if (tid == 0)
        {
            unsigned long long b = 9ull * sizeof(XaMapUnit) + 3ull * size * size / 2 * sizeof(pixel) * 3;
            for (int i = 0; i < nc; i++)
                if (S.cand[i].valid)
                    b += (unsigned long long)((S.cand[i].dir & 1) + ((S.cand[i].dir >> 1) & 1)) * ((unsigned)(size + 7) * (size + 7) + 2u * (unsigned)(size / 2 + 3) * (size / 2 + 3)) * sizeof(pixel) +
                         3ull * size * size / 2 * sizeof(pixel);
            XA_BYTES(b);
        }
        for (int i = tid; i < 5 * 3 * 16; i += NT) (&S.acc[0][0][0])[i] = 0;
        __syncthreads();
        {
            const int C = size >> 1;
            const int tY = size >> 3, nY = tY * tY, tC = C >> 3, nC = tC * tC;
            const int perCand = nY + (nC ? 2 * nC : 1);
            const int total = nc * perCand;
            for (int t0 = wv; t0 < total; t0 += 4 * XA_SERVER_WAVES)
            {
                int v[4], sv[4], grp[4], pl4[4], ci4[4];
                pixel* dp[4];
#pragma unroll
                for (int q = 0; q < 4; q++)
                {
                    const int t = t0 + q * XA_SERVER_WAVES;
                    grp[q] = -1; v[q] = 0; sv[q] = 0; dp[q] = nullptr; pl4[q] = 0; ci4[q] = 0;
                    if (t >= total) continue;
                    const int ci = t / perCand, r = t - ci * perCand;
                    if (!S.cand[ci].valid) continue;
                    const x265amd_mc_job& j = S.mc[ci];
                    const McSetup su = mc_setup(j, J.info.pic_width, J.info.pic_height);
                    ci4[q] = ci;
                    if (r < nY)
                    {
                        const McPlane P = mc_plane_of(j, su, planes, J.stride, J.cstride, 0);
                        const int ty = r / tY, tx = r - ty * tY, xx = 8 * tx + (lane & 7), yy = 8 * ty + (lane >> 3);
                        v[q] = mc_one<8>(P, j, su.mode, su.lsel, xx, yy);
                        sv[q] = (reinterpret_cast<const pixel*>(srcPlanes[0]) + (size_t)y * J.stride + x)[(size_t)yy * J.stride + xx];
                        dp[q] = P.dst + (long)yy * P.dstStride + xx;
                        pl4[q] = 0; grp[q] = size == 8 ? 0 : (ty >> 1) * (size >> 4) + (tx >> 1);
                    }
                    else if (nC)
                    {
                        const int u = r - nY, pl = 1 + u / nC, k = u % nC, ty = k / tC, tx = k - ty * tC, xx = 8 * tx + (lane & 7), yy = 8 * ty + (lane >> 3);
                        const McPlane P = mc_plane_of(j, su, planes, J.stride, J.cstride, pl);
                        v[q] = mc_one<4>(P, j, su.mode, su.lsel, xx, yy);
                        sv[q] = (reinterpret_cast<const pixel*>(srcPlanes[pl]) + (size_t)(y >> 1) * J.cstride + (x >> 1))[(size_t)yy * J.cstride + xx];
                        dp[q] = P.dst + (long)yy * P.dstStride + xx;
                        pl4[q] = pl; grp[q] = C == 8 ? 0 : (ty >> 1) * (C >> 4) + (tx >> 1);
                    }
                    else
                    {
                        const int pl = 1 + ((lane >> 4) & 1), l = lane & 15, xx = l & 3, yy = l >> 2;
                        if (lane < 32)
                        {
                            const McPlane P = mc_plane_of(j, su, planes, J.stride, J.cstride, pl);
                            v[q] = mc_one<4>(P, j, su.mode, su.lsel, xx, yy);
                            sv[q] = (reinterpret_cast<const pixel*>(srcPlanes[pl]) + (size_t)(y >> 1) * J.cstride + (x >> 1))[yy * J.cstride + xx];
                            dp[q] = P.dst + (long)yy * P.dstStride + xx;
                        }
                        grp[q] = 64;
                    }
                }
#pragma unroll
                for (int q = 0; q < 4; q++)
                {
                    if (grp[q] < 0) continue;
                    if (dp[q]) *dp[q] = (pixel)v[q];
                    if (grp[q] == 64)
                    {
                        const int sum = xa_row16_sum(abs(xa_lane_had4x4(sv[q] - v[q], lane)));
                        if (lane < 32 && (lane & 15) == 0) S.acc[ci4[q]][1 + ((lane >> 4) & 1)][0] = (unsigned int)sum;
                    }
                    else
                    {
                        const int raw = xa_wave_sum(abs(xa_lane_had8x8(sv[q] - v[q], lane)));
                        if (lane == 0) atomicAdd(&S.acc[ci4[q]][pl4[q]][grp[q]], (unsigned int)raw);
                    }
                }
            }
        }
        asm volatile("s_waitcnt vmcnt(0)" ::: "memory");
        __syncthreads();
        XA_CHAIN_T(1);
        if (tid == 0)
        {
            uint64_t bestCost = ~0ull;
            int best = -1;
            const uint64_t lambda = J.lambda;
            const int C = size >> 1, gY = size == 8 ? 1 : (size >> 4) * (size >> 4), gC = C <= 8 ? 1 : (C >> 4) * (C >> 4);
            for (int i = 0; i < nc; i++)
            {
                if (!S.cand[i].valid) continue;
                unsigned int sy = 0, sc = 0;
                for (int k = 0; k < gY; k++) sy += (S.acc[i][0][k] + 2) >> 2;
                for (int pl = 1; pl < 3; pl++)
                {
                    if (C == 4) sc += S.acc[i][pl][0] >> 1;
                    else for (int k = 0; k < gC; k++) sc += (S.acc[i][pl][k] + 2) >> 2;
                }
                S.meas[i].sa8d_luma = sy; S.meas[i].sa8d = sy + sc;
                const uint32_t bits = (uint32_t)(i + (i < nc - 1));
                const uint32_t d = J.chroma_sa8d ? sy + sc : sy;
                const uint64_t c = d + ((bits * lambda + 128) >> 8);
                if (c < bestCost) { bestCost = c; best = i; }
            }
            S.best = best;
        }
        __syncthreads();
        XA_CHAIN_T(2);
        const int best = S.best;
        if (best < 0) { reason = XA_CHAIN_NOTSKIP; break; }
        if (log2 > J.tu_log2_max)
        {
            const int L = J.tu_log2_max, C = L - 1;
            const int ntL = size >> L, ntC = (size >> 1) >> C, nLuma = ntL * ntL, nChroma = ntC * ntC;
            const pixel* tile = reinterpret_cast<const pixel*>(S.mc[best].dst_y);
            const int total = nLuma + 2 * nChroma;
            auto geo = [&](int k, const pixel*& fenc, int& fs, const pixel*& pred, int& ps, int& lg, int& tt, int& qp) {
                if (k < nLuma)
                {
                    const int ty = k / ntL, tx = k - ty * ntL, n = 1 << L;
                    fenc = reinterpret_cast<const pixel*>(srcPlanes[0]) + (size_t)(y + ty * n) * J.stride + x + tx * n; fs = J.stride;
                    pred = tile + (size_t)ty * n * 64 + tx * n; ps = 64; lg = L; tt = 0; qp = J.qp_luma;
                }
                else
                {
                    const int p = 1 + (k - nLuma) / nChroma, kk = (k - nLuma) % nChroma, ty = kk / ntC, tx = kk - ty * ntC, n = 1 << C;
                    fenc = reinterpret_cast<const pixel*>(srcPlanes[p]) + (size_t)((y >> 1) + ty * n) * J.cstride + (x >> 1) + tx * n; fs = J.cstride;
                    pred = tile + 4096 + (size_t)(p - 1) * 1024 + (size_t)ty * n * 32 + tx * n; ps = 32; lg = C; tt = p; qp = J.qp_chroma;
                }
            };
            const bool tree = nLuma == 4 && L == 5 && XA_SERVER_WAVES >= 8 && !J.chain64_off;
            int small = 0;
            for (int k = 0; k < total; k++)
            {
                const pixel* fenc; const pixel* pred; int fs, ps, lg, tt, qp;
                geo(k, fenc, fs, pred, ps, lg, tt, qp);
                if (lg >= 5)
                {
                    __syncthreads();
                    const uint32_t ns = chain_tu_levels(TL[XA_SERVER_WAVES], fenc, fs, pred, ps, lg, tt, J.slice_type, qp, J.tu_flags, XaBlock{ tid, NT, S.red });
                    if (ns && tid == 0) S.anyLevel |= 1 << k;
                    __syncthreads();
                    if (S.anyLevel && !tree) break;
                }
                else
                {
                    if ((small % XA_SERVER_WAVES) == wv)
                    {
                        const uint32_t ns = chain_tu_levels(TL[wv], fenc, fs, pred, ps, lg, tt, J.slice_type, qp, J.tu_flags, XaWave{ lane });
                        if (ns && lane == 0) atomicOr(&S.anyLevel, 1 << k);
                    }
                    small++;
                }
            }
            __syncthreads();
            const uint32_t sig = (uint32_t)S.anyLevel;
            auto hand_over = [&]() {
                if (tid == 64)
                {
                    const ChainCand c = S.cand[best];
                    XaChainStopHead h{};
                    h.valid = 2; h.node = (uint32_t)node; h.cand = (uint8_t)best; h.dir = c.dir;
                    for (int l = 0; l < 2; l++) { const bool used = (c.dir >> l) & 1; h.ref_idx[l] = used ? c.ref_idx[l] : -1; h.mv[l][0] = used ? c.mv[l][0] : 0; h.mv[l][1] = used ? c.mv[l][1] : 0; }
                    h.sa8d = S.meas[best].sa8d; h.sa8d_luma = S.meas[best].sa8d_luma;
                    xa_st_result(reinterpret_cast<XaChainStopHead*>(&out->stop), h);
                }
                asm volatile("s_waitcnt vmcnt(0)" ::: "memory");
                __syncthreads();
            };
            if (sig && !tree) { hand_over(); reason = XA_CHAIN_NOTSKIP; break; }
            if (tid == 0)
            {
                CuMeasureJob& m = S.mj;
                m.fenc[0] = srcPlanes[0] + ((uint64_t)y * J.stride + x) * isz;
                m.fenc[1] = srcPlanes[1] + ((uint64_t)(y >> 1) * J.cstride + (x >> 1)) * isz;
                m.fenc[2] = srcPlanes[2] + ((uint64_t)(y >> 1) * J.cstride + (x >> 1)) * isz;
                m.pred = S.mc[best].dst_y;
                m.recon = J.tiles + (uint64_t)(depth * J.tiles_per_depth + J.cand_tile0 + 5) * J.tile_bytes;
                m.resi = 0; m.sel = 0; m.fenc_stride = J.stride; m.fenc_cstride = J.cstride; m.log2_size = log2; m.assemble = 0;
            }
            __syncthreads();
            block_cu_measure_job(S.mj, &S.meas[best], ML, tid, NT);
            __syncthreads();
            if (sig)
            {
                if (tid < 12)
                {
                    const int k = tid, p = k >> 2;
                    x265amd_tu_job& j = S.tu[k];
                    j = x265amd_tu_job{};
                    S.tr[k] = x265amd_tu_result{};
                    if ((sig >> k) & 1)
                    {
                        const pixel* fenc; const pixel* pred; int fs, ps, lg, tt, qp;
                        geo(k, fenc, fs, pred, ps, lg, tt, qp);
                        const int n = 1 << lg;
                        const uint64_t off = p ? 4096 + (uint64_t)(k - 4) * 256 : (uint64_t)k * 1024;
                        j.fenc = (uint64_t)(uintptr_t)fenc; j.pred = (uint64_t)(uintptr_t)pred;
                        j.coeff = J.scratch + off * 2;
                        j.resi = J.scratch + 6144 * 2 + off * 2;
                        j.recon = J.scratch + 6144 * 4 + off * isz;
                        j.fenc_stride = fs; j.pred_stride = ps; j.resi_stride = n; j.recon_stride = n;
                        j.log2_tr_size = (uint8_t)lg; j.ttype = (uint8_t)tt; j.intra = 0; j.dir_mode = 0; j.slice_type = (uint8_t)J.slice_type;
                        j.qp_scaled = (uint8_t)qp; j.sign_hide = (uint8_t)J.sign_hide; j.flags = (uint8_t)J.tu_flags;
                    }
                }
                __syncthreads();
                for (int k = 0; k < 4; k++)
                    if ((sig >> k) & 1)
                    {
                        grp_tu_measure<false>(TL[XA_SERVER_WAVES], nullptr, S.tu[k], nullptr, reinterpret_cast<const pixel*>(S.tu[k].pred), 64, &S.tr[k], XaBlock{ tid, NT, S.red });
                        __syncthreads();
                    }
                {
                    int idx = 0;
                    for (int k = 4; k < 12; k++)
                        if ((sig >> k) & 1)
                        {
                            if (idx == wv) wave_tu_measure<false>(TL[wv], nullptr, S.tu[k], nullptr, reinterpret_cast<const pixel*>(S.tu[k].pred), 32, &S.tr[k], lane);
                            idx++;
                        }
                }
                asm volatile("s_waitcnt vmcnt(0)" ::: "memory");
                __syncthreads();
                if (wv == 0) chain_merge_rd64(S, x, y, log2, best, lane, sig);
                __syncthreads();
                if (!S.skipWins) { hand_over(); reason = XA_CHAIN_NOTSKIP; break; }
            }
            if (wv == 0)
            {
                for (int i = lane; i < X265AMD_CTX_STRIDE; i += 64) S.ctxS[i] = S.ctx[i];
                xa_wave_sync();
                if (lane == 0)
                {
                    uint64_t fS = S.frac & 32767;
                    fS += cb_bin(S.ctxS + CC_SKIP + chain_skip_ctx(J, x, y), 1);
                    fS += chain_merge_index(S.ctxS, (uint32_t)best, (uint32_t)J.info.max_num_merge_cand);
                    S.fracS = fS;
                }
            }
            __syncthreads();
            XA_CHAIN_T(3);
        }
        else
        {
            const int C = log2 - 1 < 2 ? 2 : log2 - 1;
            if (tid < 3)
            {
                const int p = tid, n = p ? 1 << C : size;
                x265amd_tu_job& j = S.tu[p];
                j = x265amd_tu_job{};
                const pixel* tile = reinterpret_cast<const pixel*>(S.mc[best].dst_y);
                j.fenc = p ? srcPlanes[p] + ((uint64_t)(y >> 1) * J.cstride + (x >> 1)) * isz : srcPlanes[0] + ((uint64_t)y * J.stride + x) * isz;
                j.pred = (uint64_t)(uintptr_t)(p ? tile + 4096 + (size_t)(p - 1) * 1024 : tile);
                const uint64_t off = p ? 1024 + (uint64_t)(p - 1) * 256 : 0;
                j.coeff = J.scratch + off * 2;
                j.resi = J.scratch + 1536 * 2 + off * 2;
                j.recon = J.scratch + 1536 * 4 + off * isz;
                j.fenc_stride = p ? J.cstride : J.stride; j.pred_stride = p ? 32 : 64; j.resi_stride = n; j.recon_stride = n;
                j.log2_tr_size = (uint8_t)(p ? C : log2); j.ttype = (uint8_t)p; j.intra = 0; j.dir_mode = 0; j.slice_type = (uint8_t)J.slice_type;
                j.qp_scaled = (uint8_t)(p ? J.qp_chroma : J.qp_luma); j.sign_hide = (uint8_t)J.sign_hide; j.flags = (uint8_t)J.tu_flags;
            }
            __syncthreads();
            if (log2 == 5)
            {
                grp_tu_measure<false>(TL[XA_SERVER_WAVES], nullptr, S.tu[0], nullptr, reinterpret_cast<const pixel*>(S.tu[0].pred), 64, &S.tr[0], XaBlock{ tid, NT, S.red });
                __syncthreads();
                if (wv < 2) wave_tu_measure<false>(TL[wv], nullptr, S.tu[1 + wv], nullptr, reinterpret_cast<const pixel*>(S.tu[1 + wv].pred), 32, &S.tr[1 + wv], lane);
            }
            else if (wv < 3) wave_tu_measure<false>(TL[wv], nullptr, S.tu[wv], nullptr, reinterpret_cast<const pixel*>(S.tu[wv].pred), wv ? 32 : 64, &S.tr[wv], lane);
            asm volatile("s_waitcnt vmcnt(0)" ::: "memory");
            __syncthreads();
            XA_CHAIN_T(3);
            if (tid == 0)
            {
                x265amd_cu_measure& m = S.meas[best];
                m.sse[0] = S.tr[0].zero_dist; m.sse[1] = S.tr[1].zero_dist; m.sse[2] = S.tr[2].zero_dist; m.psy = S.tr[0].zero_energy;
                m.src_mean = 0; m.src_homo = 0; m.reserved = 0;
            }
            __syncthreads();
            if (wv == 0) chain_merge_rd(S, x, y, log2, best, lane);
            __syncthreads();
            XA_CHAIN_T(4);
            if (!S.skipWins)
            {
                const pixel* tile = reinterpret_cast<const pixel*>(S.mc[best].dst_y);
                pixel* tm = reinterpret_cast<pixel*>(J.tiles + (uint64_t)(depth * J.tiles_per_depth + J.merge_recon_tile) * J.tile_bytes);
                pixel* ts = reinterpret_cast<pixel*>(J.tiles + (uint64_t)(depth * J.tiles_per_depth + J.skip_recon_tile) * J.tile_bytes);
                for (int p = 0; p < 3; p++)
                {
                    const int lg = p ? C : log2, off = p ? 4096 + (p - 1) * 1024 : 0, st = p ? 32 : 64;
                    chain_copy_plane(ts + off, st, tile + off, st, lg, p != 0, tid, NT);
                    if (S.rdCbf[p]) chain_copy_plane(tm + off, st, reinterpret_cast<const pixel*>(S.tu[p].recon), 1 << lg, lg, p != 0, tid, NT);
                    else chain_copy_plane(tm + off, st, tile + off, st, lg, p != 0, tid, NT);
                }
                XaChainStop* sp = &out->stop;
                for (int p = 0; p < 3; p++)
                {
                    const int lg = p ? C : log2, n2 = 1 << (2 * lg);
                    const int16_t* lv = reinterpret_cast<const int16_t*>(S.tu[p].coeff);
                    int16_t* dst = sp->levels + (p ? 1024 + (p - 1) * 256 : 0);
                    for (int i = tid; i < n2 / 4; i += NT)
                    {
                        const uint64_t w = *reinterpret_cast<const uint64_t*>(lv + 4 * i);
                        __hip_atomic_store(reinterpret_cast<uint64_t*>(dst + 4 * i), w, __ATOMIC_RELAXED, __HIP_MEMORY_SCOPE_SYSTEM);
                    }
                }
                if (tid < X265AMD_CTX_STRIDE / 8) __hip_atomic_store(reinterpret_cast<uint64_t*>(sp->ctx) + tid, reinterpret_cast<const uint64_t*>(S.ctxD)[tid], __ATOMIC_RELAXED, __HIP_MEMORY_SCOPE_SYSTEM);
                if (tid == 64)
                {
                    const ChainCand c = S.cand[best];
                    XaChainStopHead h;
                    h.valid = 1; h.node = (uint32_t)node; h.cand = (uint8_t)best; h.dir = c.dir;
                    for (int l = 0; l < 2; l++) { const bool used = (c.dir >> l) & 1; h.ref_idx[l] = used ? c.ref_idx[l] : -1; h.mv[l][0] = used ? c.mv[l][0] : 0; h.mv[l][1] = used ? c.mv[l][1] : 0; }
                    h.cbf[0] = (uint8_t)S.rdCbf[0]; h.cbf[1] = (uint8_t)S.rdCbf[1]; h.cbf[2] = (uint8_t)S.rdCbf[2]; h.reserved0 = 0;
                    h.total_bits = S.rdBits[0]; h.mv_bits = S.rdBits[1]; h.coeff_bits = S.rdBits[0] - S.rdPad - S.rdBits[1] - S.rdBits[2]; h.psy_energy = S.rdPsy;
                    h.sa8d = S.meas[best].sa8d; h.sa8d_luma = S.meas[best].sa8d_luma;
                    h.rd_cost = S.rdCost; h.luma_dist = S.rdLuma; h.chroma_dist = S.rdChroma; h.frac = S.fracD; h.meas = S.meas[best];
                    xa_st_result(reinterpret_cast<XaChainStopHead*>(sp), h);
                }
                asm volatile("s_waitcnt vmcnt(0)" ::: "memory");
                __syncthreads();
                reason = XA_CHAIN_NOTSKIP; break;
            }
        }
        {
            const ChainCand c = S.cand[best];
            XaMapUnit u{};
            u.pred_mode = X265AMD_MODE_SKIP; u.inter_dir = c.dir; u.depth = (uint8_t)depth;
            for (int l = 0; l < 2; l++)
            {
                const bool used = (c.dir >> l) & 1;
                u.ref_idx[l] = used ? c.ref_idx[l] : -1; u.mv[l][0] = used ? c.mv[l][0] : 0; u.mv[l][1] = used ? c.mv[l][1] : 0;
            }
            XaMapUnit* cur = reinterpret_cast<XaMapUnit*>(J.cur);
            const int n4 = size >> 2;
            if (!(J.dbg & 1)) for (int i = tid; i < n4 * n4; i += NT) chain_st_unit(cur + ((y >> 2) + i / n4) * J.w4 + (x >> 2) + (i % n4), u);
            const pixel* s0 = reinterpret_cast<const pixel*>(S.mc[best].dst_y);
            const int half = size >> 1;
            if (!(J.dbg & 2)) {
            chain_copy_plane(reinterpret_cast<pixel*>(recPlanes[0]) + (size_t)y * J.stride + x, J.stride, s0, 64, log2, false, tid, NT);
            chain_copy_plane(reinterpret_cast<pixel*>(recPlanes[1]) + (size_t)(y >> 1) * J.cstride + (x >> 1), J.cstride, s0 + 4096, 32, log2 - 1, true, tid, NT);
            chain_copy_plane(reinterpret_cast<pixel*>(recPlanes[2]) + (size_t)(y >> 1) * J.cstride + (x >> 1), J.cstride, s0 + 5120, 32, log2 - 1, true, tid, NT);
            }
            (void)half;
            for (int da = depth - 1; da >= 0 && !(J.dbg & 4); da--)
            {
                const int asize = 64 >> da, ax = J.ctu_x + ((x - J.ctu_x) & ~(asize - 1)), ay = J.ctu_y + ((y - J.ctu_y) & ~(asize - 1));
                pixel* t = reinterpret_cast<pixel*>(J.tiles + (uint64_t)(da * J.tiles_per_depth + J.split_recon_tile) * J.tile_bytes);
                chain_copy_plane(t + (size_t)(y - ay) * 64 + (x - ax), 64, s0, 64, log2, false, tid, NT);
                chain_copy_plane(t + 4096 + (size_t)((y - ay) >> 1) * 32 + ((x - ax) >> 1), 32, s0 + 4096, 32, log2 - 1, true, tid, NT);
                chain_copy_plane(t + 5120 + (size_t)((y - ay) >> 1) * 32 + ((x - ax) >> 1), 32, s0 + 5120, 32, log2 - 1, true, tid, NT);
            }
            if (tid == 0)
            {
                XA_BYTES((unsigned long long)(size >> 2) * (size >> 2) * sizeof(XaMapUnit) + 3ull * size * size / 2 * sizeof(pixel) * (1 + depth) + sizeof(XaChainCuOut));
                XaChainCuOut o{};
                o.node = (uint32_t)node; o.cand = (uint8_t)best; o.dir = c.dir; o.ref_idx[0] = u.ref_idx[0]; o.ref_idx[1] = u.ref_idx[1];
                o.mv[0][0] = u.mv[0][0]; o.mv[0][1] = u.mv[0][1]; o.mv[1][0] = u.mv[1][0]; o.mv[1][1] = u.mv[1][1];
                o.meas = S.meas[best];
                if (!(J.dbg & 8)) xa_st_result(&out->cu[S.count], o);
                S.count++;
            }
        }
        asm volatile("s_waitcnt vmcnt(0)" ::: "memory");
        __syncthreads();
        XA_CHAIN_T(5);
        if (tid < X265AMD_CTX_STRIDE) S.ctx[tid] = S.ctxS[tid];
        __syncthreads();
        if (tid == 0)
        {
            uint64_t f = S.fracS;
            if (depth < J.max_cu_depth) chain_split_flag(J, S.ctx, f, x, y, depth, 0);
            for (int p = N.parent; p != 255 && S.nodes[p].next == N.next; p = S.nodes[p].parent)
                if (S.used[p] & 2) chain_split_flag(J, S.ctx, f, S.nodes[p].x, S.nodes[p].y, 6 - S.nodes[p].log2, 1);
            S.frac = f;
            S.ticks[6] += 1;
            if (J.use_dqp)
            {
                const bool origin = x == J.ctu_x && y == J.ctu_y;
                if (depth <= J.max_dqp_depth)
// ... 37 lines not shown
```

### x265-amod_amd/csrc/inter_search_dev.h

```cpp
#ifndef X265AMD_INTER_SEARCH_DEV_H
#define X265AMD_INTER_SEARCH_DEV_H
#include <stdint.h>

struct XaSearchRef { int16_t amvp[2][2]; int16_t mvc[12][2]; int32_t num_mvc, ref_pic, ref_idx, reserved; };
enum { XA_SEARCH_MAX_REFS = 8 };

struct alignas(8) XaSearchJob
{
    XaSearchRef ref[XA_SEARCH_MAX_REFS];
    int32_t num_refs, x, y, log2;
    int32_t pic_w, pic_h, stride, cstride, num_pics, num_ref_idx0;
    int32_t search_method, subme, merange, me_qp, frame_parallel, search_range, lag_pixels, list_sel_bits0;
    uint64_t me_lambda;
    uint64_t mvcost, bitsize, me_tables;
    uint64_t planes, luma_tab;
    uint64_t pred_tile, recon_tile, scratch, out;
    uint64_t lambda, lambda2;
    uint32_t psy_rd;
    int32_t qp_luma, qp_chroma, sign_hide, chroma_sa8d, rd_level, skip_ctx, do_rd, slice_type;
    int32_t dqp;
    int32_t tu_flags, reserved2;
    uint64_t frac;
    uint8_t ctx[X265AMD_CTX_STRIDE];
};

struct XaSearchOut
{
    uint32_t valid; int32_t best;
    int16_t mv[2], mvp[2]; int32_t mvp_idx; uint32_t bits, cost, mv_cost;
    uint32_t sa8d, sa8d_luma;
    uint8_t cbf[3], rd_done;
    uint32_t total_bits, mv_bits, coeff_bits, psy_energy, res_energy, reserved1;
    uint64_t rd_cost, luma_dist, chroma_dist, frac;
    uint8_t ctx[X265AMD_CTX_STRIDE];
    int16_t levels[1024 + 2 * 256];
};

#ifdef XA_SEARCH_DEVICE

struct SearchLds
{
    XaSearchJob job;
    x265amd_mc_job mc[2 * XA_SEARCH_MAX_REFS];
    uint32_t cost[4 * XA_SEARCH_MAX_REFS];
    XaCmd cmd;
    int mvpIdx[XA_SEARCH_MAX_REFS];
    int best, bestMvpIdx; int bestMv[2], bestMvp[2]; uint32_t bestBits, bestCost, bestMvCost;
    unsigned int acc[3][16];
    uint32_t sa8d, sa8dLuma;
    x265amd_tu_job tu[3];
    x265amd_tu_result tr[3];
    uint8_t ctxB[X265AMD_CTX_STRIDE], ctxD[X265AMD_CTX_STRIDE];
    uint32_t rdBits[3], rdPsy, rdCbf[3], rdPad; uint64_t rdCost, rdLuma, rdChroma, fracD;
    uint32_t step[256];
    unsigned long long red[XA_SERVER_WAVES];
};
#define XA_SEARCH_HEADER 8192
#define XA_SEARCH_LDS_BELOW (XA_SERVER_LDS - XA_SEARCH_HEADER)

XA_DEV void search_clip_mv(int& mx, int& my, int cuX, int cuY, int picW, int picH)
{
    const int xmax = (picW + 8 - cuX - 1) << 2, xmin = -((64 + 8 + cuX - 1) << 2), ymax = (picH + 8 - cuY - 1) << 2, ymin = -((64 + 8 + cuY - 1) << 2);
    mx = min(xmax, max(xmin, mx)); my = min(ymax, max(ymin, my));
}
XA_DEV uint32_t search_bitcost(const float* bs, int mx, int my, int px, int py) { return (uint32_t)(bs[abs(mx - px)] + bs[abs(my - py)] + 0.5f); }

XA_DEV uint64_t search_amvp_bits(uint8_t* ctx, int refIdx, int numRefIdx, int mvdx, int mvdy, int mvpIdx)
{
    enum { C_REF_NO = 24, C_MV_RES = 26, C_MVP_IDX = 151 };
    uint64_t f = 0;
    if (numRefIdx > 1)
    {
        uint32_t ref = (uint32_t)refIdx;
        f += cb_bin(ctx + C_REF_NO, ref > 0);
        if (ref > 0)
        {
            const uint32_t refNum = (uint32_t)numRefIdx - 2;
            if (refNum)
            {
                ref--;
                f += cb_bin(ctx + C_REF_NO + 1, ref > 0);
                if (ref > 0) f += 32768ull * (ref - (ref == refNum));
            }
        }
    }
    f += cb_bin(ctx + C_MV_RES, mvdx != 0); f += cb_bin(ctx + C_MV_RES, mvdy != 0);
    const uint32_t ha = (uint32_t)abs(mvdx), va = (uint32_t)abs(mvdy);
    if (mvdx) f += cb_bin(ctx + C_MV_RES + 1, ha > 1);
    if (mvdy) f += cb_bin(ctx + C_MV_RES + 1, va > 1);
    auto egBins = [](uint32_t symbol) { uint32_t count = 1, n = 0; while (symbol >= (1u << count)) { n++; symbol -= 1u << count; count++; } return n + 1 + count; };
    if (mvdx) { if (ha > 1) f += 32768ull * egBins(ha - 2); f += 32768ull; }
    if (mvdy) { if (va > 1) f += 32768ull * egBins(va - 2); f += 32768ull; }
    f += cb_bin(ctx + C_MVP_IDX, (uint32_t)mvpIdx);
    return f;
}

template<class JOB> XA_DEV uint64_t search_cost(const JOB& J, chain_sse_t dist, uint32_t bits, uint32_t energy)
{
    return J.psy_rd ? (uint64_t)dist + ((J.lambda * J.psy_rd * energy) >> 24) + (((uint64_t)bits * J.lambda2) >> 8) : (uint64_t)dist + (((uint64_t)bits * J.lambda2 + 128) >> 8);
}

XA_DEV void search_inter_rd(SearchLds& S, int log2, int lane)
{
    const XaSearchJob& J = S.job;
    for (int i = lane; i < X265AMD_CTX_STRIDE; i += 64) { const uint8_t v = J.ctx[i]; S.ctxB[i] = v; S.ctxD[i] = v; }
    xa_wave_sync();
    const chain_sse_t predDist = (chain_sse_t)((chain_sse_t)S.tr[0].zero_dist + (chain_sse_t)S.tr[1].zero_dist + (chain_sse_t)S.tr[2].zero_dist);
    const uint32_t predPsy = J.psy_rd ? S.tr[0].zero_energy : 0;
    const int logs[3] = { log2, log2 - 1 < 2 ? 2 : log2 - 1, log2 - 1 < 2 ? 2 : log2 - 1 };
    uint32_t cbf[3], singleBits[3];
    chain_sse_t singleDist[3];
    uint32_t energyY = 0;
    uint64_t fB = J.frac & 32767;
    bool anyLevel = false;
    for (int p = 0; p < 3; p++) anyLevel |= S.tr[p].num_sig != 0;
    if (anyLevel)
    {
        for (int p = 0; p < 3; p++)
        {
            const x265amd_tu_result r = S.tr[p];
            cbf[p] = r.num_sig != 0;
            const uint32_t latest = (uint32_t)(fB >> 15);
            if (cbf[p]) fB += wave_coeff_bits(S.ctxB, S.ctxB, reinterpret_cast<const int16_t*>(S.tu[p].coeff), logs[p], p, 0, 0, J.sign_hide, S.step, lane);
            xa_wave_sync();
            singleBits[p] = (uint32_t)(fB >> 15) - (p ? latest : 0);
            const chain_sse_t zeroDist = (chain_sse_t)r.zero_dist;
            const uint32_t zeroEnergy = J.psy_rd ? r.zero_energy : 0;
            if (cbf[p])
            {
                const uint8_t st = S.ctxB[CC_QT_CBF + (p ? 2 : 1)];
                const uint32_t nzCbfBits = (uint32_t)(((fB & 32767) + en_bits[st ^ 1]) >> 15), nullBits = (uint32_t)(((fB & 32767) + en_bits[st ^ 0]) >> 15);
                const chain_sse_t nzDist = (chain_sse_t)r.nz_dist;
                const uint32_t nzEnergy = J.psy_rd ? r.nz_energy : 0;
                const uint64_t singleCost = search_cost(J, nzDist, nzCbfBits + singleBits[p], nzEnergy), nullCost = search_cost(J, zeroDist, nullBits, zeroEnergy);
                if (nullCost < singleCost) { cbf[p] = 0; singleBits[p] = 0; singleDist[p] = zeroDist; if (!p) energyY = zeroEnergy; }
                else { singleDist[p] = nzDist; if (!p) energyY = nzEnergy; }
            }
            else { singleBits[p] = 0; singleDist[p] = zeroDist; if (!p) energyY = zeroEnergy; }
        }
        chain_sse_t fullDist = 0;
        fullDist += singleDist[0]; fullDist += singleDist[1]; fullDist += singleDist[2];
        const uint64_t fullCost = search_cost(J, fullDist, singleBits[0] + singleBits[1] + singleBits[2], energyY);
        const uint32_t cbf0Bits = (uint32_t)(((J.frac & 32767) + en_bits[J.ctx[CC_QT_ROOT_CBF] ^ 0]) >> 15);
        if (search_cost(J, predDist, cbf0Bits, predPsy) < fullCost) cbf[0] = cbf[1] = cbf[2] = 0;
    }
    else
    {
        cbf[0] = cbf[1] = cbf[2] = 0;
    }
    const uint32_t rootCbf = cbf[0] | cbf[1] | cbf[2];
    uint64_t fD = J.frac & 32767;
    if (lane == 0)
    {
        const XaSearchRef& R = J.ref[S.best];
        fD += cb_bin(S.ctxD + CC_SKIP + J.skip_ctx, 0);
        S.rdBits[2] = (uint32_t)(fD >> 15);
        fD += cb_bin(S.ctxD + CC_PRED_MODE, 0);
        fD += cb_bin(S.ctxD + CC_PART_SIZE, 1);
        fD += cb_bin(S.ctxD + CC_MERGE_FLAG, 0);
        fD += search_amvp_bits(S.ctxD, R.ref_idx, J.num_ref_idx0, S.bestMv[0] - S.bestMvp[0], S.bestMv[1] - S.bestMvp[1], S.bestMvpIdx);
        S.rdBits[1] = (uint32_t)(fD >> 15) - S.rdBits[2];
        fD += cb_bin(S.ctxD + CC_QT_ROOT_CBF, rootCbf);
        if (rootCbf)
        {
            fD += cb_bin(S.ctxD + CC_QT_CBF + 2, cbf[1]);
            fD += cb_bin(S.ctxD + CC_QT_CBF + 2, cbf[2]);
            if (cbf[1] | cbf[2]) fD += cb_bin(S.ctxD + CC_QT_CBF + 1, cbf[0]);
            if (J.dqp) fD += chain_dqp_bits(S.ctxD, (int)(int8_t)(J.dqp & 0xff));
        }
    }
    xa_wave_sync();
    fD = __shfl(fD, 0, 64);
    if (rootCbf)
        for (int p = 0; p < 3; p++)
        {
            if (cbf[p]) fD += wave_coeff_bits(S.ctxD, S.ctxD, reinterpret_cast<const int16_t*>(S.tu[p].coeff), logs[p], p, 0, 0, J.sign_hide, S.step, lane);
            xa_wave_sync();
        }
    chain_sse_t dist = 0;
    dist += cbf[0] ? (chain_sse_t)S.tr[0].nz_dist : (chain_sse_t)S.tr[0].zero_dist;
    chain_sse_t cd = cbf[1] ? (chain_sse_t)S.tr[1].nz_dist : (chain_sse_t)S.tr[1].zero_dist;
    cd += cbf[2] ? (chain_sse_t)S.tr[2].nz_dist : (chain_sse_t)S.tr[2].zero_dist;
    dist += cd;
    const uint32_t psy = J.psy_rd ? (cbf[0] ? S.tr[0].nz_energy : S.tr[0].zero_energy) : 0;
    if (lane == 0)
    {
        uint32_t bits = (uint32_t)(fD >> 15), again = 0;
        if (rootCbf && (J.dqp >> 17))
        {
            fD = (fD & 32767) + chain_dqp_bits(S.ctxD, (int)(int8_t)(J.dqp & 0xff));
            again = (uint32_t)(fD >> 15);
            bits += again;
        }
        S.fracD = fD; S.rdBits[0] = bits; S.rdPad = again; S.rdPsy = psy; S.rdCbf[0] = cbf[0]; S.rdCbf[1] = cbf[1]; S.rdCbf[2] = cbf[2];
        S.rdCost = search_cost(J, dist, bits, psy); S.rdLuma = (uint64_t)(dist - cd); S.rdChroma = (uint64_t)cd;
    }
}

__device__ __noinline__ void xa_op_me_call(int which, const XaCmd& c, int tid);

XA_DEV void block_inter_search(const XaSearchJob* jobAddr, char* smem, int tid)
{
    constexpr int NT = 64 * XA_SERVER_WAVES;
    const int lane = tid & 63, wv = tid >> 6;
    static_assert(sizeof(SearchLds) <= XA_SEARCH_HEADER, "search header");
    static_assert((XA_SERVER_WAVES + 1) * sizeof(TuLds) <= XA_SEARCH_LDS_BELOW, "LDS budget");
    SearchLds& S = *reinterpret_cast<SearchLds*>(smem + XA_SEARCH_LDS_BELOW);
    TuLds* TL = reinterpret_cast<TuLds*>(smem);
    __syncthreads();
    {
        const uint64_t* src = reinterpret_cast<const uint64_t*>(jobAddr);
        uint64_t* dst = reinterpret_cast<uint64_t*>(&S.job);
        for (int i = tid; i < (int)(sizeof(XaSearchJob) / 8); i += NT) dst[i] = __hip_atomic_load(src + i, __ATOMIC_RELAXED, __HIP_MEMORY_SCOPE_SYSTEM);
        for (int i = tid; i < 256; i += NT) S.step[i] = en_step.v[i];
    }
    __syncthreads();
    const XaSearchJob& J = S.job;
    const uint64_t* planes = reinterpret_cast<const uint64_t*>(J.planes);
    const uint64_t* srcPlanes = planes + 3 * (J.num_pics - 1);
    XaSearchOut* out = reinterpret_cast<XaSearchOut*>(J.out);
    const size_t isz = sizeof(pixel);
    const int x = J.x, y = J.y, log2 = J.log2, size = 1 << log2, nr = J.num_refs;
    x265amd_me_job* meJobs = reinterpret_cast<x265amd_me_job*>(J.scratch);
    x265amd_me_group* meGroups = reinterpret_cast<x265amd_me_group*>(J.scratch + 4096);
    x265amd_me_result* meOut = reinterpret_cast<x265amd_me_result*>(J.scratch + 5120);
    const uint64_t predScratch = J.scratch + 8192, tuScratch = J.scratch + 8192 + (uint64_t)2 * XA_SEARCH_MAX_REFS * 4096 * isz;
    if (tid == 0)
        for (int r = 0; r < nr; r++)
            for (int k = 0; k < 2; k++)
            {
                x265amd_mc_job& j = S.mc[2 * r + k];
                j = x265amd_mc_job{};
                int mx = J.ref[r].amvp[k][0], my = J.ref[r].amvp[k][1];
                search_clip_mv(mx, my, x, y, J.pic_w, J.pic_h);
                j.dst_y = predScratch + (uint64_t)(2 * r + k) * 4096 * isz; j.dst_stride = size;
                j.x = (int16_t)x; j.y = (int16_t)y; j.cu_x = (int16_t)x; j.cu_y = (int16_t)y; j.w = (uint8_t)size; j.h = (uint8_t)size;
                j.ref0 = (int8_t)J.ref[r].ref_pic; j.ref1 = -1; j.mv0[0] = (int16_t)mx; j.mv0[1] = (int16_t)my;
                j.slice_type = 1; j.flags = 1; j.metric = 1; j.chroma_cost = 0;
                S.cost[2 * (2 * r + k)] = 0;
            }
    __syncthreads();
    {
        XaArgsMc a;
        a.planes = planes; a.stride = J.stride; a.cstride = J.cstride; a.picW = J.pic_w; a.picH = J.pic_h; a.jobs = nullptr; a.n = 2 * nr;
        a.fencPlanes = srcPlanes; a.fstride = J.stride; a.fcstride = J.cstride; a.cost = S.cost;
        for (int t = wv; t < 2 * nr; t += XA_SERVER_WAVES)
        {
            const int r = t >> 1;
            const bool differ = J.ref[r].amvp[0][0] != J.ref[r].amvp[1][0] || J.ref[r].amvp[0][1] != J.ref[r].amvp[1][1];
            if (differ) wave_mc_rec<true>(a, S.mc[t], t, lane);
        }
    }
    __syncthreads();
    if (tid == 0)
    {
        int maxW = 80, maxH = 80;
        for (int r = 0; r < nr; r++)
        {
            const XaSearchRef& R = J.ref[r];
            int idx = 0;
            if (R.amvp[0][0] != R.amvp[1][0] || R.amvp[0][1] != R.amvp[1][1])
            {
                uint32_t c2[2] = { S.cost[2 * (2 * r)], S.cost[2 * (2 * r + 1)] };
                if (J.frame_parallel)
                    for (int k = 0; k < 2; k++) if (R.amvp[k][1] >= (J.search_range + 1) * 4) c2[k] = 1u << 28;
                idx = c2[0] <= c2[1] ? 0 : 1;
            }
            S.mvpIdx[r] = idx;
            const int mvpx = R.amvp[idx][0], mvpy = R.amvp[idx][1];
            int mnx = mvpx - (J.merange << 2), mny = mvpy - (J.merange << 2), mxx = mvpx + (J.merange << 2), mxy = mvpy + (J.merange << 2);
            search_clip_mv(mnx, mny, x, y, J.pic_w, J.pic_h); search_clip_mv(mxx, mxy, x, y, J.pic_w, J.pic_h);
            const int maxLen = (1 << 15) - 1;
            mnx = max(mnx, -maxLen); mny = max(mny, -maxLen); mxx = min(mxx, maxLen); mxy = min(mxy, maxLen);
            mnx >>= 2; mny >>= 2; mxx >>= 2; mxy >>= 2;
            mny = min(mny, J.lag_pixels); mxy = min(mxy, J.lag_pixels);
            mxy = max(mxy, mny);
            x265amd_me_job j{};
            j.x = (int16_t)x; j.y = (int16_t)y; j.w = (uint8_t)size; j.h = (uint8_t)size;
            j.method = (uint8_t)J.search_method; j.subme = (uint8_t)J.subme; j.qp = (uint8_t)J.me_qp; j.num_cand = (uint8_t)R.num_mvc; j.merange = (int16_t)J.merange;
            j.mvmin[0] = (int16_t)mnx; j.mvmin[1] = (int16_t)mny; j.mvmax[0] = (int16_t)mxx; j.mvmax[1] = (int16_t)mxy;
            j.mvp[0] = (int16_t)mvpx; j.mvp[1] = (int16_t)mvpy;
            for (int k = 0; k < R.num_mvc; k++) { j.mvc[k][0] = R.mvc[k][0]; j.mvc[k][1] = R.mvc[k][1]; }
            meJobs[r] = j;
            int x0 = x + mnx - 6, y0 = y + mny - 6, x1 = x + size + mxx + 10, y1 = y + size + mxy + 7;
            int w = (x1 - x0 + 3) & ~3, h = y1 - y0;
            if (w > 192) { x0 += (w - 192) / 2; w = 192; }
            if (h > 192) { y0 += (h - 192) / 2; h = 192; }
            x265amd_me_group g{};
            g.first_job = r; g.num_jobs = 1; g.ref = R.ref_pic; g.win_x = (int16_t)x0; g.win_y = (int16_t)y0; g.win_w = (int16_t)w; g.win_h = (int16_t)h;
            g.fenc_x = (int16_t)((x >> 6) << 6); g.fenc_y = (int16_t)((y >> 6) << 6);
            meGroups[r] = g;
            maxW = max(maxW, w); maxH = max(maxH, h);
        }
        MeParams p;
        p.fenc = reinterpret_cast<const pixel*>(srcPlanes[0]); p.refs = reinterpret_cast<const uint64_t*>(J.luma_tab); p.chroma = nullptr; p.stride = J.stride; p.cstride = J.cstride;
        p.groups = meGroups; p.jobs = meJobs; p.out = meOut; p.tables = reinterpret_cast<const uint16_t*>(J.me_tables); p.maxWinW = maxW; p.maxWinH = maxH;
        S.cmd = XaCmd{};
        S.cmd.count = (uint32_t)nr;
        static_assert(sizeof(MeParams) <= sizeof(S.cmd.args), "MeParams is a command's argument record");
        *reinterpret_cast<MeParams*>(S.cmd.args) = p;
    }
    asm volatile("s_waitcnt vmcnt(0)" ::: "memory");
    __syncthreads();
    xa_op_me_call((J.search_method & 0x7f) == X265AMD_ME_STAR ? 1 : 0, S.cmd, tid);
    __syncthreads();
    xa_op_me_call(2, S.cmd, tid);
    asm volatile("s_waitcnt vmcnt(0)" ::: "memory");
    __syncthreads();
    if (tid == 0)
    {
        const float* bs = reinterpret_cast<const float*>(J.bitsize);
        const uint16_t* mvc = reinterpret_cast<const uint16_t*>(J.mvcost);
        auto getCost = [&](uint32_t bits) { return (uint32_t)((bits * J.me_lambda + 128) >> 8); };
        S.best = -1; S.bestCost = 0xFFFFFFFFu;
        for (int r = 0; r < nr; r++)
        {
            const XaSearchRef& R = J.ref[r];
            const x265amd_me_result res = meOut[r];
            int mvpIdx = S.mvpIdx[r];
            const int mx = res.mv[0], my = res.mv[1];
            uint32_t bits = (uint32_t)J.list_sel_bits0 + 1 + (uint32_t)(R.ref_idx + (R.ref_idx < J.num_ref_idx0 - 1));
            bits += search_bitcost(bs, mx, my, R.amvp[mvpIdx][0], R.amvp[mvpIdx][1]);
            const uint32_t mvCost = (uint32_t)mvc[mx - R.amvp[mvpIdx][0]] + (uint32_t)mvc[my - R.amvp[mvpIdx][1]];
            uint32_t cc = ((uint32_t)res.cost - mvCost) + getCost(bits);
            const int diffBits = (int)search_bitcost(bs, mx, my, R.amvp[!mvpIdx][0], R.amvp[!mvpIdx][1]) - (int)search_bitcost(bs, mx, my, R.amvp[mvpIdx][0], R.amvp[mvpIdx][1]);
            if (diffBits < 0)
            {
                mvpIdx = !mvpIdx;
                const uint32_t orig = bits;
                bits = orig + diffBits;
                cc = (cc - getCost(orig)) + getCost(bits);
            }
            if (cc < S.bestCost)
            {
                S.best = r; S.bestCost = cc; S.bestBits = bits; S.bestMvCost = mvCost; S.bestMvpIdx = mvpIdx;
                S.bestMv[0] = mx; S.bestMv[1] = my; S.bestMvp[0] = R.amvp[mvpIdx][0]; S.bestMvp[1] = R.amvp[mvpIdx][1];
            }
        }
        if (S.best >= 0)
        {
            x265amd_mc_job& j = S.mc[0];
            j = x265amd_mc_job{};
            j.dst_y = J.pred_tile; j.dst_u = J.pred_tile + 4096 * isz; j.dst_v = j.dst_u + 1024 * isz; j.dst_stride = 64; j.dst_cstride = 32;
            j.x = (int16_t)x; j.y = (int16_t)y; j.cu_x = (int16_t)x; j.cu_y = (int16_t)y; j.w = (uint8_t)size; j.h = (uint8_t)size;
            j.ref0 = (int8_t)J.ref[S.best].ref_pic; j.ref1 = -1; j.mv0[0] = (int16_t)S.bestMv[0]; j.mv0[1] = (int16_t)S.bestMv[1];
            j.slice_type = 1; j.flags = 3;
        }
    }
    if (tid == 0)
        XA_BYTES(sizeof(XaSearchJob) + (unsigned long long)2 * nr * ((unsigned)(size + 7) * (size + 7) + (unsigned)size * size) * sizeof(pixel) +
                 ((unsigned long long)(size + 7) * (size + 7) + 2ull * (size / 2 + 3) * (size / 2 + 3) + 6ull * size * size) * sizeof(pixel) + 256 + 3ull * size * size);
    for (int i = tid; i < 3 * 16; i += NT) (&S.acc[0][0])[i] = 0;
    __syncthreads();
    if (S.best < 0)
    {
        if (tid == 0) { struct alignas(8) H { uint32_t valid; int32_t best; } h{ 1u, -1 }; xa_st_result(reinterpret_cast<H*>(out), h); }
        return;
    }
    {
        const int C = size >> 1;
        const int tY = size >> 3, nY = tY * tY, tC = C >> 3, nC = tC * tC;
        const int total = nY + (nC ? 2 * nC : 1);
        const x265amd_mc_job& j = S.mc[0];
        const McSetup su = mc_setup(j, J.pic_w, J.pic_h);
        for (int t = wv; t < total; t += XA_SERVER_WAVES)
        {
            if (t < nY)
            {
                const McPlane P = mc_plane_of(j, su, planes, J.stride, J.cstride, 0);
                const int ty = t / tY, tx = t - ty * tY;
                const int raw = chain_pred_tile<8>(j, su, P, reinterpret_cast<const pixel*>(srcPlanes[0]) + (size_t)y * J.stride + x, J.stride, tx, ty, lane);
                if (lane == 0) atomicAdd(&S.acc[0][size == 8 ? 0 : (ty >> 1) * (size >> 4) + (tx >> 1)], (unsigned int)raw);
            }
            else if (nC)
            {
                const int u = t - nY, pl = 1 + u / nC, k = u % nC, ty = k / tC, tx = k - ty * tC;
                const McPlane P = mc_plane_of(j, su, planes, J.stride, J.cstride, pl);
                const int raw = chain_pred_tile<4>(j, su, P, reinterpret_cast<const pixel*>(srcPlanes[pl]) + (size_t)(y >> 1) * J.cstride + (x >> 1), J.cstride, tx, ty, lane);
                if (lane == 0) atomicAdd(&S.acc[pl][C == 8 ? 0 : (ty >> 1) * (C >> 4) + (tx >> 1)], (unsigned int)raw);
            }
            else
            {
                const int pl = 1 + ((lane >> 4) & 1), l = lane & 15, xx = l & 3, yy = l >> 2;
                int d = 0;
                if (lane < 32)
                {
                    const McPlane P = mc_plane_of(j, su, planes, J.stride, J.cstride, pl);
                    const int v = mc_one<4>(P, j, su.mode, su.lsel, xx, yy);
                    P.dst[(long)yy * P.dstStride + xx] = (pixel)v;
                    d = (int)(reinterpret_cast<const pixel*>(srcPlanes[pl]) + (size_t)(y >> 1) * J.cstride + (x >> 1))[yy * J.cstride + xx] - v;
                }
                const int sum = xa_row16_sum(abs(xa_lane_had4x4(d, lane)));
                if (lane < 32 && l == 0) S.acc[pl][0] = (unsigned int)sum;
            }
        }
    }
    asm volatile("s_waitcnt vmcnt(0)" ::: "memory");
    __syncthreads();
    if (tid == 0)
    {
        const int C = size >> 1, gY = size == 8 ? 1 : (size >> 4) * (size >> 4), gC = C <= 8 ? 1 : (C >> 4) * (C >> 4);
        unsigned int sy = 0, sc = 0;
        for (int k = 0; k < gY; k++) sy += (S.acc[0][k] + 2) >> 2;
        for (int pl = 1; pl < 3; pl++)
        {
            if (C == 4) sc += S.acc[pl][0] >> 1;
            else for (int k = 0; k < gC; k++) sc += (S.acc[pl][k] + 2) >> 2;
        }
        S.sa8dLuma = sy; S.sa8d = sy + sc;
    }
    const bool doRd = J.do_rd && log2 <= 5;
    if (doRd)
    {
        const int C = log2 - 1 < 2 ? 2 : log2 - 1;
        if (tid < 3)
        {
            const int p = tid, n = p ? 1 << C : size;
            x265amd_tu_job& j = S.tu[p];
            j = x265amd_tu_job{};
            const pixel* tile = reinterpret_cast<const pixel*>(J.pred_tile);
            j.fenc = p ? srcPlanes[p] + ((uint64_t)(y >> 1) * J.cstride + (x >> 1)) * isz : srcPlanes[0] + ((uint64_t)y * J.stride + x) * isz;
            j.pred = (uint64_t)(uintptr_t)(p ? tile + 4096 + (size_t)(p - 1) * 1024 : tile);
            const uint64_t off = p ? 1024 + (uint64_t)(p - 1) * 256 : 0;
            j.coeff = tuScratch + off * 2;
            j.resi = tuScratch + 1536 * 2 + off * 2;
            j.recon = tuScratch + 1536 * 4 + off * isz;
            j.fenc_stride = p ? J.cstride : J.stride; j.pred_stride = p ? 32 : 64; j.resi_stride = n; j.recon_stride = n;
            j.log2_tr_size = (uint8_t)(p ? C : log2); j.ttype = (uint8_t)p; j.intra = 0; j.dir_mode = 0; j.slice_type = (uint8_t)J.slice_type;
            j.qp_scaled = (uint8_t)(p ? J.qp_chroma : J.qp_luma); j.sign_hide = (uint8_t)J.sign_hide; j.flags = (uint8_t)J.tu_flags;
        }
        __syncthreads();
        if (log2 == 5)
        {
            grp_tu_measure<false>(TL[XA_SERVER_WAVES], nullptr, S.tu[0], nullptr, reinterpret_cast<const pixel*>(S.tu[0].pred), 64, &S.tr[0], XaBlock{ tid, NT, S.red });
            __syncthreads();
            if (wv < 2) wave_tu_measure<false>(TL[wv], nullptr, S.tu[1 + wv], nullptr, reinterpret_cast<const pixel*>(S.tu[1 + wv].pred), 32, &S.tr[1 + wv], lane);
        }
        else if (wv < 3) wave_tu_measure<false>(TL[wv], nullptr, S.tu[wv], nullptr, reinterpret_cast<const pixel*>(S.tu[wv].pred), wv ? 32 : 64, &S.tr[wv], lane);
        asm volatile("s_waitcnt vmcnt(0)" ::: "memory");
        __syncthreads();
        if (wv == 0) search_inter_rd(S, log2, lane);
        __syncthreads();
        const pixel* tile = reinterpret_cast<const pixel*>(J.pred_tile);
        pixel* tr = reinterpret_cast<pixel*>(J.recon_tile);
        for (int p = 0; p < 3; p++)
        {
            const int lg = p ? C : log2, off = p ? 4096 + (p - 1) * 1024 : 0, st = p ? 32 : 64;
            if (S.rdCbf[p]) chain_copy_plane(tr + off, st, reinterpret_cast<const pixel*>(S.tu[p].recon), 1 << lg, lg, p != 0, tid, NT);
            else chain_copy_plane(tr + off, st, tile + off, st, lg, p != 0, tid, NT);
        }
        for (int p = 0; p < 3; p++)
        {
            const int lg = p ? C : log2, n2 = 1 << (2 * lg);
            const int16_t* lv = reinterpret_cast<const int16_t*>(S.tu[p].coeff);
            int16_t* dst = out->levels + (p ? 1024 + (p - 1) * 256 : 0);
            for (int i = tid; i < n2 / 4; i += NT)
                __hip_atomic_store(reinterpret_cast<uint64_t*>(dst + 4 * i), *reinterpret_cast<const uint64_t*>(lv + 4 * i), __ATOMIC_RELAXED, __HIP_MEMORY_SCOPE_SYSTEM);
        }
        if (tid < X265AMD_CTX_STRIDE / 8) __hip_atomic_store(reinterpret_cast<uint64_t*>(out->ctx) + tid, reinterpret_cast<const uint64_t*>(S.ctxD)[tid], __ATOMIC_RELAXED, __HIP_MEMORY_SCOPE_SYSTEM);
    }
    __syncthreads();
    if (tid == 64)
    {
        struct alignas(8) Head
        {
            uint32_t valid; int32_t best; int16_t mv[2], mvp[2]; int32_t mvp_idx; uint32_t bits, cost, mv_cost; uint32_t sa8d, sa8d_luma; uint8_t cbf[3], rd_done;
            uint32_t total_bits, mv_bits, coeff_bits, psy_energy, res_energy, reserved1; uint64_t rd_cost, luma_dist, chroma_dist, frac;
        } h;
        h.valid = 1; h.best = S.best; h.mv[0] = (int16_t)S.bestMv[0]; h.mv[1] = (int16_t)S.bestMv[1]; h.mvp[0] = (int16_t)S.bestMvp[0]; h.mvp[1] = (int16_t)S.bestMvp[1];
        h.mvp_idx = S.bestMvpIdx; h.bits = S.bestBits; h.cost = S.bestCost; h.mv_cost = S.bestMvCost; h.sa8d = S.sa8d; h.sa8d_luma = S.sa8dLuma;
        h.cbf[0] = doRd ? (uint8_t)S.rdCbf[0] : 0; h.cbf[1] = doRd ? (uint8_t)S.rdCbf[1] : 0; h.cbf[2] = doRd ? (uint8_t)S.rdCbf[2] : 0; h.rd_done = doRd ? 1 : 0;
        h.total_bits = doRd ? S.rdBits[0] : 0; h.mv_bits = doRd ? S.rdBits[1] : 0; h.coeff_bits = doRd ? S.rdBits[0] - S.rdPad - S.rdBits[1] - S.rdBits[2] : 0;
        h.psy_energy = doRd ? S.rdPsy : 0; h.res_energy = doRd ? (uint32_t)S.tr[0].zero_dist : 0; h.reserved1 = 0;
        h.rd_cost = doRd ? S.rdCost : 0; h.luma_dist = doRd ? S.rdLuma : 0; h.chroma_dist = doRd ? S.rdChroma : 0; h.frac = doRd ? S.fracD : 0;
        static_assert(sizeof(Head) == offsetof(XaSearchOut, ctx), "the search result's head");
        xa_st_result(reinterpret_cast<Head*>(out), h);
    }
}

#endif
#endif
```

### x265-amod_amd/csrc/mc_kernels.hip

```cpp
#include "x265amd_dev.h"
#include "x265amd_host.h"

#include "mc_dev.h"
#include "xa_queue.h"

template<bool COST>
__global__ __launch_bounds__(64 * MC_WAVES) void k_motion_compensation(XaArgsMc a)
{
    const int ji = blockIdx.x * MC_WAVES + (threadIdx.x >> 6);
    if (ji >= a.n) return;
    wave_mc_job<COST>(a, ji, xa_lane());
}

extern "C" int x265amd_motion_compensation(void* stream, const uint64_t* d_planes, intptr_t stride, intptr_t cstride, int pic_w, int pic_h,
                                           const x265amd_mc_job* d_jobs, int n)
{
    if (n <= 0) return X265AMD_OK;
    if (!d_planes || !d_jobs) return xa_fail(X265AMD_EINVAL, "x265amd_motion_compensation: bad arguments");
    const XaArgsMc qa = { d_planes, (long)stride, (long)cstride, pic_w, pic_h, d_jobs, n, nullptr, 0L, 0L, nullptr };
    hipError_t e;
    XA_LAUNCH(e, stream, XA_OP_MC, n, qa, k_motion_compensation<false>, dim3((n + MC_WAVES - 1) / MC_WAVES), dim3(64 * MC_WAVES), 0, qa);
    if (e != hipSuccess) return xa_fail(X265AMD_EHIP, hipGetErrorString(e));
    return X265AMD_OK;
}

extern "C" int x265amd_inter_cost(void* stream, const uint64_t* d_planes, intptr_t stride, intptr_t cstride, int pic_w, int pic_h,
                                  const x265amd_mc_job* d_jobs, int n, const uint64_t* d_fenc_planes, intptr_t fenc_stride, intptr_t fenc_cstride,
                                  uint32_t* d_cost)
{
    if (n <= 0) return X265AMD_OK;
    if (!d_planes || !d_jobs || !d_fenc_planes || !d_cost) return xa_fail(X265AMD_EINVAL, "x265amd_inter_cost: bad arguments");
    const XaArgsMc qa = { d_planes, (long)stride, (long)cstride, pic_w, pic_h, d_jobs, n, d_fenc_planes, (long)fenc_stride, (long)fenc_cstride, d_cost };
    hipError_t e;
    XA_LAUNCH(e, stream, XA_OP_MC_COST, n, qa, k_motion_compensation<true>, dim3((n + MC_WAVES - 1) / MC_WAVES), dim3(64 * MC_WAVES), 0, qa);
    if (e != hipSuccess) return xa_fail(X265AMD_EHIP, hipGetErrorString(e));
    return X265AMD_OK;
}
```

Before: 102.8.

## Stage CU reference windows in LDS for batched motion-compensated prediction cost

Adds a cu_pred_cost device routine that copies each candidate's reference windows and the source block into LDS once, then runs separable interpolation, bi-averaging and 4x4 Hadamard/SAD per 4x4 tile from LDS. The in-device search path uses it for large CUs when scoring AMVP candidates and the final prediction, replacing per-pixel global-memory mc_one calls. It also skips the third ME call unless me_redo reports it is needed. A new standalone kernel and API entry point expose the same routine. The cost is much more code, heavy LDS use that can lower occupancy, and risk to bit-exactness in the hand-written filter arithmetic.

```diff
diff --git a/include/x265amd.h b/include/x265amd.h
--- a/include/x265amd.h
+++ b/include/x265amd.h
@@ -359,6 +359,10 @@
                        const x265amd_mc_job* d_jobs, int n, const uint64_t* d_fenc_planes, intptr_t fenc_stride, intptr_t fenc_cstride,
                        uint32_t* d_cost);
 
+int x265amd_cu_pred_cost(void* stream, const uint64_t* d_planes, intptr_t stride, intptr_t cstride, int pic_w, int pic_h,
+                         const x265amd_mc_job* d_jobs, int n, const uint64_t* d_fenc_planes, intptr_t fenc_stride, intptr_t fenc_cstride,
+                         uint32_t* d_cost, int cands_per_cu);
+
 int x265amd_extend_pic_border(void* stream, x265amd_pixel* d_pic, intptr_t stride, int width, int height, int marginX, int marginY);
 int x265amd_extend_border_rows(void* stream, x265amd_pixel* d_pic, intptr_t stride, int width, int height, int marginX, int marginY, int y_begin, int y_end);
 int x265amd_extend_border_band(void* stream, x265amd_pixel* d_pic, intptr_t stride, int width, int height, int marginX, int marginY, int y_begin, int y_end,
diff --git a/x265-amod_amd/csrc/cu_pred_dev.h b/x265-amod_amd/csrc/cu_pred_dev.h
--- /dev/null
+++ b/x265-amod_amd/csrc/cu_pred_dev.h
@@ -0,0 +1,336 @@
+#ifndef X265AMD_CU_PRED_DEV_H
+#define X265AMD_CU_PRED_DEV_H
+#include "mc_dev.h"
+
+enum { CU_PRED_MAX_CANDS = 16, CU_PRED_MAX_SLOTS = 10, CU_PRED_HEADER = 1280, CU_PRED_ACC = 3 * 16 };
+
+struct CuPredWin { uint64_t g; uint32_t lds; int32_t strideBytes; uint16_t rows, rowBytes; uint8_t xf, yf, pad[2]; };
+struct CuPredCand { int16_t mv[2][2]; int8_t ref[2], slot[2]; uint8_t mode, lsel, ndir, pad; };
+struct CuPredHead
+{
+    uint32_t coef[16];
+    CuPredCand cand[CU_PRED_MAX_CANDS];
+    CuPredWin win[3 + 3 * CU_PRED_MAX_SLOTS];
+};
+static_assert(sizeof(CuPredHead) <= CU_PRED_HEADER, "cu_pred header");
+
+constexpr int cu_pred_pitch(int n, int taps) { return ((n + taps - 1) * (int)sizeof(pixel) + 14) & ~7; }
+constexpr int cu_pred_src_bytes(int size) { return size * cu_pred_pitch(size, 8) + 2 * (size / 2) * cu_pred_pitch(size / 2, 4); }
+constexpr int cu_pred_slot_bytes(int size) { return (size + 7) * cu_pred_pitch(size, 8) + 2 * (size / 2 + 3) * cu_pred_pitch(size / 2, 4); }
+constexpr int cu_pred_min_lds(int size) { return CU_PRED_HEADER + cu_pred_src_bytes(size) + 2 * cu_pred_slot_bytes(size) + 32; }
+
+template<int NP> XA_DEV void cu_pred_row(const char* lds, uint32_t off, int px[NP])
+{
+    constexpr int ND = (NP * (int)sizeof(pixel) + 3) / 4;
+    const uint32_t* p = reinterpret_cast<const uint32_t*>(lds + (off & ~3u));
+    uint32_t raw[ND + 1];
+#pragma unroll
+    for (int i = 0; i <= ND; i++) raw[i] = p[i];
+    const uint32_t sh = off & 3;
+#pragma unroll
+    for (int i = 0; i < ND; i++) raw[i] = __builtin_amdgcn_alignbyte(raw[i + 1], raw[i], sh);
+#pragma unroll
+    for (int k = 0; k < NP; k++)
+        px[k] = sizeof(pixel) == 1 ? (int)__builtin_amdgcn_ubfe(raw[k >> 2], 8 * (k & 3), 8) : (int)__builtin_amdgcn_ubfe(raw[k >> 1], 16 * (k & 1), 16);
+}
+
+template<int TAPS> XA_DEV void cu_pred_tile(const char* lds, const uint32_t* coef, const CuPredWin& w, int pitch, int tx, int ty, bool shrt, int out[16])
+{
+    constexpr int NP = TAPS + 3;
+    const int headRoom = XA_IF_INTERNAL_PREC - XA_DEPTH;
+    const int shiftH = XA_IF_FILTER_PREC - headRoom, offH = (int)((unsigned)-XA_IF_INTERNAL_OFFS << shiftH);
+    const int xf = w.xf, yf = w.yf;
+    int cx[TAPS];
+    uint64_t cy;
+    if (TAPS == 8)
+    {
+        const uint32_t lo = coef[2 * xf], hi = coef[2 * xf + 1];
+#pragma unroll
+        for (int t = 0; t < 4; t++) { cx[t] = (int)(int8_t)(lo >> (8 * t)); cx[4 + t] = (int)(int8_t)(hi >> (8 * t)); }
+        cy = (uint64_t)coef[2 * yf] | ((uint64_t)coef[2 * yf + 1] << 32);
+    }
+    else
+    {
+        const uint32_t c = coef[8 + xf];
+#pragma unroll
+        for (int t = 0; t < 4; t++) cx[t] = (int)(int8_t)(c >> (8 * t));
+        cy = coef[8 + yf];
+    }
+    if (!yf) cy = 1;
+    const int nrows = yf ? NP : 4;
+#pragma unroll
+    for (int k = 0; k < 16; k++) out[k] = 0;
+#pragma unroll 1
+    for (int rr = 0; rr < nrows; rr++)
+    {
+        const int row = ty + rr;
+        const uint32_t off = w.lds + (uint32_t)(row * pitch) + (((uint32_t)w.g + (uint32_t)(row * w.strideBytes)) & 7u) + (uint32_t)tx * (uint32_t)sizeof(pixel);
+        int px[NP], t[4];
+        cu_pred_row<NP>(lds, off, px);
+        if (xf)
+        {
+#pragma unroll
+            for (int x = 0; x < 4; x++)
+            {
+                int hs = 0;
+#pragma unroll
+                for (int k = 0; k < TAPS; k++) hs += px[x + k] * cx[k];
+                t[x] = (yf || shrt) ? (int)(int16_t)((hs + offH) >> shiftH) : xa_clip3(0, XA_PIXEL_MAX, (int)(int16_t)((hs + (1 << (XA_IF_FILTER_PREC - 1))) >> XA_IF_FILTER_PREC));
+            }
+        }
+        else
+        {
+#pragma unroll
+            for (int x = 0; x < 4; x++) t[x] = (yf || !shrt) ? px[x] : (int)(int16_t)((int16_t)(px[x] << headRoom) - (int16_t)XA_IF_INTERNAL_OFFS);
+        }
+#pragma unroll
+        for (int r = 0; r < 4; r++)
+        {
+            const int k = rr - r;
+            const int c = (unsigned)k < (unsigned)TAPS ? (int)(int8_t)(cy >> (8 * k)) : 0;
+#pragma unroll
+            for (int x = 0; x < 4; x++) out[4 * r + x] += t[x] * c;
+        }
+    }
+    if (yf)
+    {
+        const int shiftV = XA_IF_FILTER_PREC + headRoom, offV = (1 << (shiftV - 1)) + (XA_IF_INTERNAL_OFFS << XA_IF_FILTER_PREC);
+#pragma unroll
+        for (int k = 0; k < 16; k++)
+        {
+            const int s = out[k];
+            if (xf) out[k] = shrt ? (int)(int16_t)(s >> XA_IF_FILTER_PREC) : xa_clip3(0, XA_PIXEL_MAX, (int)(int16_t)((s + offV) >> shiftV));
+            else out[k] = shrt ? (int)(int16_t)((s + offH) >> shiftH) : xa_clip3(0, XA_PIXEL_MAX, (int)(int16_t)((s + (1 << (XA_IF_FILTER_PREC - 1))) >> XA_IF_FILTER_PREC));
+        }
+    }
+}
+
+XA_DEV void cu_pred_had4x4(int d[16])
+{
+#pragma unroll
+    for (int y = 0; y < 4; y++)
+    {
+        const int s01 = d[4 * y] + d[4 * y + 1], e01 = d[4 * y] - d[4 * y + 1], s23 = d[4 * y + 2] + d[4 * y + 3], e23 = d[4 * y + 2] - d[4 * y + 3];
+        d[4 * y] = s01 + s23; d[4 * y + 1] = s01 - s23; d[4 * y + 2] = e01 + e23; d[4 * y + 3] = e01 - e23;
+    }
+#pragma unroll
+    for (int x = 0; x < 4; x++)
+    {
+        const int s01 = d[x] + d[4 + x], e01 = d[x] - d[4 + x], s23 = d[8 + x] + d[12 + x], e23 = d[8 + x] - d[12 + x];
+        d[x] = s01 + s23; d[4 + x] = s01 - s23; d[8 + x] = e01 + e23; d[12 + x] = e01 - e23;
+    }
+}
+
+static __device__ __noinline__ void cu_pred_cost(char* lds, int ldsBytes, const x265amd_mc_job* jobs, int n, uint32_t valid, const uint64_t* planes, long stride, long cstride,
+                                          int picW, int picH, const uint64_t* srcPlanes, long fstride, long fcstride, unsigned int* acc, int accStride, bool sad, int tid, int nthr)
+{
+    static_assert(cu_pred_min_lds(64) <= 64 * 1024, "the smallest batch -- one bi-predicted 64x64 candidate -- fits a 64 KB area");
+    constexpr int isz = (int)sizeof(pixel);
+    CuPredHead& H = *reinterpret_cast<CuPredHead*>(lds);
+    const int size = jobs[0].w, C = size >> 1, lg = 31 - __builtin_clz(size);
+    const int pitchY = cu_pred_pitch(size, 8), pitchC = cu_pred_pitch(C, 4);
+    const int srcBytes = size * pitchY + 2 * C * pitchC, slotBytes = (size + 7) * pitchY + 2 * (C + 3) * pitchC;
+    const int maxSlots = min((int)CU_PRED_MAX_SLOTS, (ldsBytes - CU_PRED_HEADER - srcBytes - 32) / slotBytes);
+    const int px0 = jobs[0].x, py0 = jobs[0].y;
+    __syncthreads();
+    if (tid < 16)
+    {
+        uint32_t c = 0;
+        for (int k = 0; k < 4; k++)
+        {
+            const int v = tid < 8 ? xa_tbl.lumaFilter[tid >> 1][4 * (tid & 1) + k] : xa_tbl.chromaFilter[tid - 8][k];
+            c |= (uint32_t)(uint8_t)(int8_t)v << (8 * k);
+        }
+        H.coef[tid] = c;
+    }
+    if (tid < n)
+    {
+        const McSetup su = mc_setup(jobs[tid], picW, picH);
+        CuPredCand c{};
+        for (int l = 0; l < 2; l++) { c.mv[l][0] = (int16_t)su.mv[l][0]; c.mv[l][1] = (int16_t)su.mv[l][1]; c.ref[l] = (int8_t)su.refs[l]; c.slot[l] = -1; }
+        c.mode = (uint8_t)su.mode; c.lsel = (uint8_t)su.lsel;
+        c.ndir = !((valid >> tid) & 1) ? 0 : (su.mode == 2 ? 2 : 1);
+        if (su.mode != 2) c.ref[su.lsel ^ 1] = -1;
+        H.cand[tid] = c;
+    }
+    if (tid >= 64 && tid < 67)
+    {
+        const int c = tid - 64, nn = c ? C : size;
+        CuPredWin w{};
+        w.strideBytes = (int32_t)((c ? fcstride : fstride) * isz);
+        w.g = srcPlanes[c] + (uint64_t)((long)(c ? py0 >> 1 : py0) * (c ? fcstride : fstride) + (c ? px0 >> 1 : px0)) * isz;
+        w.lds = (uint32_t)(CU_PRED_HEADER + (c == 0 ? 0 : size * pitchY + (c - 1) * C * pitchC));
+        w.rows = (uint16_t)nn; w.rowBytes = (uint16_t)(nn * isz);
+        H.win[c] = w;
+    }
+    for (int i = tid; i < n * accStride; i += nthr) { const int ci = i / accStride; if (i - ci * accStride < (sad ? 1 : (int)CU_PRED_ACC)) acc[i] = 0; }
+    __syncthreads();
+    const int tY = lg - 3;
+    const int nY = 1 << (2 * tY), nC = size >= 16 ? nY >> 2 : 0;
+    const int quadsPer = sad ? nY : nY + (nC ? 2 * nC : 1), itemsPer = 4 * quadsPer;
+    int c0 = 0;
+    while (c0 < n)
+    {
+        int c1 = c0, used = 0;
+        while (c1 < n && used + H.cand[c1].ndir <= maxSlots) { used += H.cand[c1].ndir; c1++; }
+        if (c1 == c0) break;
+        if (tid >= c0 && tid < c1 && H.cand[tid].ndir)
+        {
+            int slot = 0;
+            for (int k = c0; k < tid; k++) slot += H.cand[k].ndir;
+            CuPredCand& cd = H.cand[tid];
+            for (int l = 0; l < 2; l++)
+            {
+                if (cd.ref[l] < 0) { cd.slot[l] = -1; continue; }
+                cd.slot[l] = (int8_t)slot;
+                const int mx = cd.mv[l][0], my = cd.mv[l][1];
+                uint32_t at = (uint32_t)(CU_PRED_HEADER + srcBytes + slot * slotBytes);
+                for (int c = 0; c < 3; c++)
+                {
+                    const int nn = c ? C : size, taps = c ? 4 : 8, half = taps / 2 - 1, sh = c ? 3 : 2, msk = c ? 7 : 3;
+                    const long st = c ? cstride : stride;
+                    CuPredWin w{};
+                    w.xf = (uint8_t)(mx & msk); w.yf = (uint8_t)(my & msk);
+                    w.strideBytes = (int32_t)(st * isz);
+                    w.g = planes[3 * cd.ref[l] + c] + (uint64_t)(((long)((c ? py0 >> 1 : py0) + (my >> sh) - (w.yf ? half : 0))) * st + (c ? px0 >> 1 : px0) + (mx >> sh) - (w.xf ? half : 0)) * isz;
+                    w.lds = at;
+                    w.rows = (uint16_t)(nn + (w.yf ? taps - 1 : 0)); w.rowBytes = (uint16_t)((nn + (w.xf ? taps - 1 : 0)) * isz);
+                    H.win[3 + 3 * slot + c] = w;
+                    at += (uint32_t)((nn + taps - 1) * (c ? pitchC : pitchY));
+                }
+                slot++;
+            }
+        }
+        __syncthreads();
+        for (int cls = 0; cls < (sad ? 1 : 2); cls++)
+        {
+            const int first = c0 ? (cls ? 2 : 1) : 0, nw = (cls ? 2 : 1) * (used + 1);
+            const int pitch = cls ? pitchC : pitchY, cpr = pitch >> 3, maxRows = cls ? C + 3 : size + 7, per = maxRows * cpr;
+            const int total = (nw - first) * per;
+            for (int i0 = tid; i0 < total; i0 += 4 * nthr)
+            {
+                uint64_t v[4];
+                uint32_t to[4];
+#pragma unroll
+                for (int q = 0; q < 4; q++)
+                {
+                    const int i = i0 + q * nthr;
+                    to[q] = 0xFFFFFFFFu; v[q] = 0;
+                    if (i >= total) continue;
+                    const int k = first + i / per, rem = i % per, r = rem / cpr, c = rem - r * cpr;
+                    const CuPredWin& w = H.win[cls ? 3 * (k >> 1) + 1 + (k & 1) : 3 * k];
+                    if (r >= w.rows) continue;
+                    const uint64_t a = w.g + (uint64_t)((long)r * w.strideBytes);
+                    if (c * 8 >= (int)(a & 7) + w.rowBytes) continue;
+                    v[q] = *reinterpret_cast<const uint64_t*>((a & ~(uint64_t)7) + (uint64_t)(c * 8));
+                    to[q] = w.lds + (uint32_t)(r * pitch + c * 8);
+                }
+#pragma unroll
+                for (int q = 0; q < 4; q++) if (to[q] != 0xFFFFFFFFu) *reinterpret_cast<uint64_t*>(lds + to[q]) = v[q];
+            }
+        }
+        __syncthreads();
+        const int total = (c1 - c0) * itemsPer;
+        for (int it = tid; it < total; it += nthr)
+        {
+            const int cb = it / itemsPer, r = it - cb * itemsPer, q = r >> 2, sub = r & 3, ci = c0 + cb;
+            const CuPredCand cd = H.cand[ci];
+            if (!cd.ndir) continue;
+            int pl, bx, by, lgB;
+            bool pair4 = false;
+            if (q < nY) { pl = 0; by = q >> tY; bx = q & ((1 << tY) - 1); lgB = tY; }
+            else if (nC) { const int u = q - nY; pl = 1 + (u >= nC); const int k = u & (nC - 1); lgB = tY - 1; by = k >> lgB; bx = k & ((1 << lgB) - 1); }
+            else { pair4 = true; pl = 1 + (sub & 1); bx = by = 0; lgB = 0; if (sub >= 2) continue; }
+            const int tx = pair4 ? 0 : 8 * bx + 4 * (sub & 1), ty = pair4 ? 0 : 8 * by + 4 * (sub >> 1);
+            const int pitch = pl ? pitchC : pitchY;
+            int v[16];
+#pragma unroll
+            for (int k = 0; k < 16; k++) v[k] = 0;
+            const bool bi = cd.mode == 2;
+#pragma unroll 1
+            for (int l = 0; l < 2; l++)
+            {
+                if (cd.slot[l] < 0) continue;
+                const CuPredWin w = H.win[3 + 3 * cd.slot[l] + pl];
+                int o[16];
+                if (pl == 0) cu_pred_tile<8>(lds, H.coef, w, pitch, tx, ty, bi, o);
+                else cu_pred_tile<4>(lds, H.coef, w, pitch, tx, ty, bi, o);
+#pragma unroll
+                for (int k = 0; k < 16; k++) v[k] += o[k];
+            }
+            if (bi)
+            {
+                const int shift = XA_IF_INTERNAL_PREC - XA_DEPTH + 1, offset = (1 << (shift - 1)) + 2 * XA_IF_INTERNAL_OFFS;
+#pragma unroll
+                for (int k = 0; k < 16; k++) v[k] = xa_clip3(0, XA_PIXEL_MAX, (v[k] + offset) >> shift);
+            }
+            if (!sad)
+            {
+                const x265amd_mc_job& j = jobs[ci];
+                const int ds = pl ? j.dst_cstride : j.dst_stride;
+                pixel* dp = reinterpret_cast<pixel*>(pl == 0 ? j.dst_y : (pl == 1 ? j.dst_u : j.dst_v)) + (long)ty * ds + tx;
+                if constexpr (sizeof(pixel) == 2)
+                {
+#pragma unroll
+                    for (int y = 0; y < 4; y++)
+                        *reinterpret_cast<uint64_t*>(dp + (long)y * ds) = (uint64_t)(uint32_t)(v[4 * y] | (v[4 * y + 1] << 16)) | ((uint64_t)(uint32_t)(v[4 * y + 2] | (v[4 * y + 3] << 16)) << 32);
+                }
+                else
+                {
+                    uint32_t p[4];
+#pragma unroll
+                    for (int y = 0; y < 4; y++) p[y] = (uint32_t)(v[4 * y] | (v[4 * y + 1] << 8) | (v[4 * y + 2] << 16) | (v[4 * y + 3] << 24));
+                    if (pair4)
+                    {
+#pragma unroll
+                        for (int y = 0; y < 4; y++) *reinterpret_cast<uint32_t*>(dp + (long)y * ds) = p[y];
+                    }
+                    else
+                    {
+                        const bool odd = sub & 1;
+                        const uint32_t r0 = (uint32_t)xa_lane_xor<1>((int)(odd ? p[0] : p[2])), r1 = (uint32_t)xa_lane_xor<1>((int)(odd ? p[1] : p[3]));
+                        pixel* d8 = odd ? dp - 4 + 2l * ds : dp;
+                        *reinterpret_cast<uint64_t*>(d8) = odd ? (uint64_t)r0 | ((uint64_t)p[2] << 32) : (uint64_t)p[0] | ((uint64_t)r0 << 32);
+                        *reinterpret_cast<uint64_t*>(d8 + ds) = odd ? (uint64_t)r1 | ((uint64_t)p[3] << 32) : (uint64_t)p[1] | ((uint64_t)r1 << 32);
+                    }
+                }
+            }
+            {
+                const CuPredWin w = H.win[pl];
+#pragma unroll
+                for (int y = 0; y < 4; y++)
+                {
+                    const int row = ty + y;
+                    int s[4];
+                    cu_pred_row<4>(lds, w.lds + (uint32_t)(row * pitch) + (((uint32_t)w.g + (uint32_t)(row * w.strideBytes)) & 7u) + (uint32_t)(tx * isz), s);
+#pragma unroll
+                    for (int x = 0; x < 4; x++) v[4 * y + x] = s[x] - v[4 * y + x];
+                }
+            }
+            int sum = 0;
+            if (sad)
+            {
+#pragma unroll
+                for (int k = 0; k < 16; k++) sum += abs(v[k]);
+            }
+            else
+            {
+                cu_pred_had4x4(v);
+                if (!pair4)
+                {
+#pragma unroll
+                    for (int k = 0; k < 16; k++) { v[k] = xa_butterfly<1>(v[k], sub); v[k] = xa_butterfly<2>(v[k], sub); }
+                }
+#pragma unroll
+                for (int k = 0; k < 16; k++) sum += abs(v[k]);
+            }
+            if (pair4) { acc[ci * accStride + pl * 16] = (unsigned int)sum; continue; }
+            sum += xa_lane_xor<1>(sum); sum += xa_lane_xor<2>(sum);
+            if (sub == 0) atomicAdd(&acc[ci * accStride + pl * 16 + ((sad || lgB == 0) ? 0 : (by >> 1) * (1 << (lgB - 1)) + (bx >> 1))], (unsigned int)sum);
+        }
+        __syncthreads();
+        c0 = c1;
+    }
+}
+
+#endif
diff --git a/x265-amod_amd/csrc/device_queue.hip b/x265-amod_amd/csrc/device_queue.hip
--- a/x265-amod_amd/csrc/device_queue.hip
+++ b/x265-amod_amd/csrc/device_queue.hip
@@ -35,6 +35,7 @@
 #include "tu_dev.h"
 #include "intra_dev.h"
 #include "mc_dev.h"
+#include "cu_pred_dev.h"
 #include "me_dev.h"
 #include "measure_dev.h"
 #include "entropy_dev.h"
diff --git a/x265-amod_amd/csrc/inter_chain_dev.h b/x265-amod_amd/csrc/inter_chain_dev.h
--- a/x265-amod_amd/csrc/inter_chain_dev.h
+++ b/x265-amod_amd/csrc/inter_chain_dev.h
@@ -294,14 +294,6 @@
     else { if (chroma) chain_copy_rows<uint64_t>(dst, ds, src, ss, log2N, tid, nthr); else chain_copy_rows<uint4>(dst, ds, src, ss, log2N, tid, nthr); }
 }
 
-template<int TAPS> XA_DEV int chain_pred_tile(const x265amd_mc_job& j, const McSetup& su, const McPlane& P, const pixel* fenc, int fs, int tx, int ty, int lane)
-{
-    const int x = 8 * tx + (lane & 7), y = 8 * ty + (lane >> 3);
-    const int v = mc_one<TAPS>(P, j, su.mode, su.lsel, x, y);
-    P.dst[(long)y * P.dstStride + x] = (pixel)v;
-    return xa_wave_sum(abs(xa_lane_had8x8((int)fenc[y * fs + x] - v, lane)));
-}
-
 template<class G> XA_DEV uint32_t chain_tu_levels(TuLds& s, const pixel* fenc, int fs, const pixel* pred, int ps, int log2N, int ttype, int sliceType, int qpScaled, int lowpass, const G& g)
 {
     const int N = 1 << log2N;
@@ -736,76 +728,12 @@
                          3ull * size * size / 2 * sizeof(pixel);
             XA_BYTES(b);
         }
-        for (int i = tid; i < 5 * 3 * 16; i += NT) (&S.acc[0][0][0])[i] = 0;
-        __syncthreads();
-        {
-            const int C = size >> 1;
-            const int tY = size >> 3, nY = tY * tY, tC = C >> 3, nC = tC * tC;
-            const int perCand = nY + (nC ? 2 * nC : 1);
-            const int total = nc * perCand;
-            for (int t0 = wv; t0 < total; t0 += 4 * XA_SERVER_WAVES)
-            {
-                int v[4], sv[4], grp[4], pl4[4], ci4[4];
-                pixel* dp[4];
-#pragma unroll
-                for (int q = 0; q < 4; q++)
-                {
-                    const int t = t0 + q * XA_SERVER_WAVES;
-                    grp[q] = -1; v[q] = 0; sv[q] = 0; dp[q] = nullptr; pl4[q] = 0; ci4[q] = 0;
-                    if (t >= total) continue;
-                    const int ci = t / perCand, r = t - ci * perCand;
-                    if (!S.cand[ci].valid) continue;
-                    const x265amd_mc_job& j = S.mc[ci];
-                    const McSetup su = mc_setup(j, J.info.pic_width, J.info.pic_height);
-                    ci4[q] = ci;
-                    if (r < nY)
-                    {
-                        const McPlane P = mc_plane_of(j, su, planes, J.stride, J.cstride, 0);
-                        const int ty = r / tY, tx = r - ty * tY, xx = 8 * tx + (lane & 7), yy = 8 * ty + (lane >> 3);
-                        v[q] = mc_one<8>(P, j, su.mode, su.lsel, xx, yy);
-                        sv[q] = (reinterpret_cast<const pixel*>(srcPlanes[0]) + (size_t)y * J.stride + x)[(size_t)yy * J.stride + xx];
-                        dp[q] = P.dst + (long)yy * P.dstStride + xx;
-                        pl4[q] = 0; grp[q] = size == 8 ? 0 : (ty >> 1) * (size >> 4) + (tx >> 1);
-                    }
-                    else if (nC)
-                    {
-                        const int u = r - nY, pl = 1 + u / nC, k = u % nC, ty = k / tC, tx = k - ty * tC, xx = 8 * tx + (lane & 7), yy = 8 * ty + (lane >> 3);
-                        const McPlane P = mc_plane_of(j, su, planes, J.stride, J.cstride, pl);
-                        v[q] = mc_one<4>(P, j, su.mode, su.lsel, xx, yy);
-                        sv[q] = (reinterpret_cast<const pixel*>(srcPlanes[pl]) + (size_t)(y >> 1) * J.cstride + (x >> 1))[(size_t)yy * J.cstride + xx];
-                        dp[q] = P.dst + (long)yy * P.dstStride + xx;
-                        pl4[q] = pl; grp[q] = C == 8 ? 0 : (ty >> 1) * (C >> 4) + (tx >> 1);
-                    }
-                    else
-                    {
-                        const int pl = 1 + ((lane >> 4) & 1), l = lane & 15, xx = l & 3, yy = l >> 2;
-                        if (lane < 32)
-                        {
-                            const McPlane P = mc_plane_of(j, su, planes, J.stride, J.cstride, pl);
-                            v[q] = mc_one<4>(P, j, su.mode, su.lsel, xx, yy);
-                            sv[q] = (reinterpret_cast<const pixel*>(srcPlanes[pl]) + (size_t)(y >> 1) * J.cstride + (x >> 1))[yy * J.cstride + xx];
-                            dp[q] = P.dst + (long)yy * P.dstStride + xx;
-                        }
-                        grp[q] = 64;
-                    }
-                }
-#pragma unroll
-                for (int q = 0; q < 4; q++)
-                {
-                    if (grp[q] < 0) continue;
-                    if (dp[q]) *dp[q] = (pixel)v[q];
-                    if (grp[q] == 64)
-                    {
-                        const int sum = xa_row16_sum(abs(xa_lane_had4x4(sv[q] - v[q], lane)));
-                        if (lane < 32 && (lane & 15) == 0) S.acc[ci4[q]][1 + ((lane >> 4) & 1)][0] = (unsigned int)sum;
-                    }
-                    else
-                    {
-                        const int raw = xa_wave_sum(abs(xa_lane_had8x8(sv[q] - v[q], lane)));
-                        if (lane == 0) atomicAdd(&S.acc[ci4[q]][pl4[q]][grp[q]], (unsigned int)raw);
-                    }
-                }
-            }
+        {
+            uint32_t validMask = 0;
+            for (int i = 0; i < nc; i++) validMask |= (uint32_t)(S.cand[i].valid != 0) << i;
+            static_assert(sizeof(S.acc[0]) == 4 * CU_PRED_ACC && cu_pred_min_lds(64) <= XA_SERVER_LDS - XA_CHAIN_HEADER, "cu_pred_cost's sums and LDS");
+            cu_pred_cost(smem + XA_CHAIN_HEADER, XA_SERVER_LDS - XA_CHAIN_HEADER, S.mc, nc, validMask, planes, J.stride, J.cstride, J.info.pic_width, J.info.pic_height,
+                         srcPlanes, J.stride, J.cstride, &S.acc[0][0][0], CU_PRED_ACC, false, tid, NT);
         }
         asm volatile("s_waitcnt vmcnt(0)" ::: "memory");
         __syncthreads();
diff --git a/x265-amod_amd/csrc/inter_search_dev.h b/x265-amod_amd/csrc/inter_search_dev.h
--- a/x265-amod_amd/csrc/inter_search_dev.h
+++ b/x265-amod_amd/csrc/inter_search_dev.h
@@ -54,6 +54,7 @@
     uint32_t rdBits[3], rdPsy, rdCbf[3], rdPad; uint64_t rdCost, rdLuma, rdChroma, fracD;
     uint32_t step[256];
     unsigned long long red[XA_SERVER_WAVES];
+    int redo;
 };
 #define XA_SEARCH_HEADER 8192
 #define XA_SEARCH_LDS_BELOW (XA_SERVER_LDS - XA_SEARCH_HEADER)
@@ -197,6 +198,16 @@
     }
 }
 
+#define XA_SEARCH_LDS_PRED 32
+
+template<int TAPS> XA_DEV int search_pred_tile(const x265amd_mc_job& j, const McSetup& su, const McPlane& P, const pixel* fenc, int fs, int tx, int ty, int lane)
+{
+    const int x = 8 * tx + (lane & 7), y = 8 * ty + (lane >> 3);
+    const int v = mc_one<TAPS>(P, j, su.mode, su.lsel, x, y);
+    P.dst[(long)y * P.dstStride + x] = (pixel)v;
+    return xa_wave_sum(abs(xa_lane_had8x8((int)fenc[y * fs + x] - v, lane)));
+}
+
 __device__ __noinline__ void xa_op_me_call(int which, const XaCmd& c, int tid);
 
 XA_DEV void block_inter_search(const XaSearchJob* jobAddr, char* smem, int tid)
@@ -224,7 +235,7 @@
     x265amd_me_job* meJobs = reinterpret_cast<x265amd_me_job*>(J.scratch);
     x265amd_me_group* meGroups = reinterpret_cast<x265amd_me_group*>(J.scratch + 4096);
     x265amd_me_result* meOut = reinterpret_cast<x265amd_me_result*>(J.scratch + 5120);
-    const uint64_t predScratch = J.scratch + 8192, tuScratch = J.scratch + 8192 + (uint64_t)2 * XA_SEARCH_MAX_REFS * 4096 * isz;
+    const uint64_t tuScratch = J.scratch + 8192 + (uint64_t)2 * XA_SEARCH_MAX_REFS * 4096 * isz;
     if (tid == 0)
         for (int r = 0; r < nr; r++)
             for (int k = 0; k < 2; k++)
@@ -233,7 +244,6 @@
                 j = x265amd_mc_job{};
                 int mx = J.ref[r].amvp[k][0], my = J.ref[r].amvp[k][1];
                 search_clip_mv(mx, my, x, y, J.pic_w, J.pic_h);
-                j.dst_y = predScratch + (uint64_t)(2 * r + k) * 4096 * isz; j.dst_stride = size;
                 j.x = (int16_t)x; j.y = (int16_t)y; j.cu_x = (int16_t)x; j.cu_y = (int16_t)y; j.w = (uint8_t)size; j.h = (uint8_t)size;
                 j.ref0 = (int8_t)J.ref[r].ref_pic; j.ref1 = -1; j.mv0[0] = (int16_t)mx; j.mv0[1] = (int16_t)my;
                 j.slice_type = 1; j.flags = 1; j.metric = 1; j.chroma_cost = 0;
@@ -241,14 +251,32 @@
             }
     __syncthreads();
     {
-        XaArgsMc a;
-        a.planes = planes; a.stride = J.stride; a.cstride = J.cstride; a.picW = J.pic_w; a.picH = J.pic_h; a.jobs = nullptr; a.n = 2 * nr;
-        a.fencPlanes = srcPlanes; a.fstride = J.stride; a.fcstride = J.cstride; a.cost = S.cost;
-        for (int t = wv; t < 2 * nr; t += XA_SERVER_WAVES)
-        {
-            const int r = t >> 1;
-            const bool differ = J.ref[r].amvp[0][0] != J.ref[r].amvp[1][0] || J.ref[r].amvp[0][1] != J.ref[r].amvp[1][1];
-            if (differ) wave_mc_rec<true>(a, S.mc[t], t, lane);
+        uint32_t differ = 0;
+        for (int r = 0; r < nr; r++)
+            if (J.ref[r].amvp[0][0] != J.ref[r].amvp[1][0] || J.ref[r].amvp[0][1] != J.ref[r].amvp[1][1]) differ |= 3u << (2 * r);
+        if (tid == 0)
+            XA_BYTES((unsigned long long)__builtin_popcount(differ) * (((unsigned)(size + 7) * (size + 7) + 2u * (unsigned)(size / 2 + 3) * (size / 2 + 3)) * sizeof(pixel) + 2ull * size * size * sizeof(pixel)));
+        static_assert(2 * XA_SEARCH_MAX_REFS <= CU_PRED_MAX_CANDS && cu_pred_min_lds(64) <= XA_SEARCH_LDS_BELOW, "cu_pred_cost's candidates and LDS");
+        if (differ && size >= XA_SEARCH_LDS_PRED)
+            cu_pred_cost(smem, XA_SEARCH_LDS_BELOW, S.mc, 2 * nr, differ, planes, J.stride, J.cstride, J.pic_w, J.pic_h, srcPlanes, J.stride, J.cstride, S.cost, 2, true, tid, NT);
+        else if (differ)
+        {
+            const pixel* src = reinterpret_cast<const pixel*>(srcPlanes[0]) + (size_t)y * J.stride + x;
+            for (int t = wv; t < 2 * nr; t += XA_SERVER_WAVES)
+            {
+                if (!((differ >> t) & 1)) continue;
+                const x265amd_mc_job& j = S.mc[t];
+                const McSetup su = mc_setup(j, J.pic_w, J.pic_h);
+                const McPlane P = mc_plane_of(j, su, planes, J.stride, J.cstride, 0);
+                int sum = 0;
+                for (int i = lane; i < size * size; i += 64)
+                {
+                    const int yy = i >> log2, xx = i & (size - 1);
+                    sum += abs((int)src[(size_t)yy * J.stride + xx] - mc_one<8>(P, j, su.mode, su.lsel, xx, yy));
+                }
+                sum = xa_wave_sum(sum);
+                if (lane == 0) S.cost[2 * t] = (uint32_t)sum;
+            }
         }
     }
     __syncthreads();
@@ -297,6 +325,7 @@
         p.groups = meGroups; p.jobs = meJobs; p.out = meOut; p.tables = reinterpret_cast<const uint16_t*>(J.me_tables); p.maxWinW = maxW; p.maxWinH = maxH;
         S.cmd = XaCmd{};
         S.cmd.count = (uint32_t)nr;
+        S.redo = 0;
         static_assert(sizeof(MeParams) <= sizeof(S.cmd.args), "MeParams is a command's argument record");
         *reinterpret_cast<MeParams*>(S.cmd.args) = p;
     }
@@ -304,7 +333,9 @@
     __syncthreads();
     xa_op_me_call((J.search_method & 0x7f) == X265AMD_ME_STAR ? 1 : 0, S.cmd, tid);
     __syncthreads();
-    xa_op_me_call(2, S.cmd, tid);
+    if (tid < nr && me_redo(*reinterpret_cast<const MeParams*>(S.cmd.args), tid)) S.redo = 1;
+    __syncthreads();
+    if (S.redo) xa_op_me_call(2, S.cmd, tid);
     asm volatile("s_waitcnt vmcnt(0)" ::: "memory");
     __syncthreads();
     if (tid == 0)
@@ -348,7 +379,7 @@
         }
     }
     if (tid == 0)
-        XA_BYTES(sizeof(XaSearchJob) + (unsigned long long)2 * nr * ((unsigned)(size + 7) * (size + 7) + (unsigned)size * size) * sizeof(pixel) +
+        XA_BYTES(sizeof(XaSearchJob) + (unsigned long long)2 * nr * ((unsigned)(size + 7) * (size + 7)) * sizeof(pixel) +
                  ((unsigned long long)(size + 7) * (size + 7) + 2ull * (size / 2 + 3) * (size / 2 + 3) + 6ull * size * size) * sizeof(pixel) + 256 + 3ull * size * size);
     for (int i = tid; i < 3 * 16; i += NT) (&S.acc[0][0])[i] = 0;
     __syncthreads();
@@ -357,6 +388,10 @@
         if (tid == 0) { struct alignas(8) H { uint32_t valid; int32_t best; } h{ 1u, -1 }; xa_st_result(reinterpret_cast<H*>(out), h); }
         return;
     }
+    static_assert(sizeof(S.acc) == 4 * CU_PRED_ACC, "cu_pred_cost's sums");
+    if (size >= XA_SEARCH_LDS_PRED)
+        cu_pred_cost(smem, XA_SEARCH_LDS_BELOW, S.mc, 1, 1u, planes, J.stride, J.cstride, J.pic_w, J.pic_h, srcPlanes, J.stride, J.cstride, &S.acc[0][0], CU_PRED_ACC, false, tid, NT);
+    else
     {
         const int C = size >> 1;
         const int tY = size >> 3, nY = tY * tY, tC = C >> 3, nC = tC * tC;
@@ -369,14 +404,14 @@
             {
                 const McPlane P = mc_plane_of(j, su, planes, J.stride, J.cstride, 0);
                 const int ty = t / tY, tx = t - ty * tY;
-                const int raw = chain_pred_tile<8>(j, su, P, reinterpret_cast<const pixel*>(srcPlanes[0]) + (size_t)y * J.stride + x, J.stride, tx, ty, lane);
+                const int raw = search_pred_tile<8>(j, su, P, reinterpret_cast<const pixel*>(srcPlanes[0]) + (size_t)y * J.stride + x, J.stride, tx, ty, lane);
                 if (lane == 0) atomicAdd(&S.acc[0][size == 8 ? 0 : (ty >> 1) * (size >> 4) + (tx >> 1)], (unsigned int)raw);
             }
             else if (nC)
             {
                 const int u = t - nY, pl = 1 + u / nC, k = u % nC, ty = k / tC, tx = k - ty * tC;
                 const McPlane P = mc_plane_of(j, su, planes, J.stride, J.cstride, pl);
-                const int raw = chain_pred_tile<4>(j, su, P, reinterpret_cast<const pixel*>(srcPlanes[pl]) + (size_t)(y >> 1) * J.cstride + (x >> 1), J.cstride, tx, ty, lane);
+                const int raw = search_pred_tile<4>(j, su, P, reinterpret_cast<const pixel*>(srcPlanes[pl]) + (size_t)(y >> 1) * J.cstride + (x >> 1), J.cstride, tx, ty, lane);
                 if (lane == 0) atomicAdd(&S.acc[pl][C == 8 ? 0 : (ty >> 1) * (C >> 4) + (tx >> 1)], (unsigned int)raw);
             }
             else
diff --git a/x265-amod_amd/csrc/mc_kernels.hip b/x265-amod_amd/csrc/mc_kernels.hip
--- a/x265-amod_amd/csrc/mc_kernels.hip
+++ b/x265-amod_amd/csrc/mc_kernels.hip
@@ -2,6 +2,7 @@
 #include "x265amd_host.h"
 
 #include "mc_dev.h"
+#include "cu_pred_dev.h"
 #include "xa_queue.h"
 
 template<bool COST>
@@ -36,3 +37,60 @@
     if (e != hipSuccess) return xa_fail(X265AMD_EHIP, hipGetErrorString(e));
     return X265AMD_OK;
 }
+
+#define CU_PRED_WG 512
+#define CU_PRED_AREA (64 * 1024 - CU_PRED_MAX_CANDS * ((int)sizeof(x265amd_mc_job) + 4 * CU_PRED_ACC) - 64)
+__global__ __launch_bounds__(CU_PRED_WG) void k_cu_pred_cost(XaArgsMc a, int per)
+{
+    static_assert(cu_pred_min_lds(64) <= CU_PRED_AREA, "LDS budget");
+    __shared__ __attribute__((aligned(16))) char area[CU_PRED_AREA];
+    __shared__ __attribute__((aligned(8))) x265amd_mc_job jobs[CU_PRED_MAX_CANDS];
+    __shared__ unsigned int acc[CU_PRED_MAX_CANDS * CU_PRED_ACC];
+    __shared__ int other;
+    const int tid = threadIdx.x, lane = tid & 63, wv = tid >> 6, first = blockIdx.x * per;
+    if (tid == 0) other = 0;
+    for (int i = tid; i < per * (int)(sizeof(x265amd_mc_job) / 8); i += CU_PRED_WG)
+        reinterpret_cast<uint64_t*>(jobs)[i] = __hip_atomic_load(reinterpret_cast<const uint64_t*>(a.jobs + first) + i, __ATOMIC_RELAXED, __HIP_MEMORY_SCOPE_SYSTEM);
+    __syncthreads();
+    if (tid < per) { const int m = mc_setup(jobs[tid], a.picW, a.picH).mode; if (m != 0 && m != 2) atomicOr(&other, 1); }
+    __syncthreads();
+    if (other)
+    {
+        for (int i = wv; i < per; i += CU_PRED_WG / 64) wave_mc_rec<true>(a, jobs[i], first + i, lane);
+        return;
+    }
+    const int metric = jobs[0].metric, size = jobs[0].w;
+    cu_pred_cost(area, CU_PRED_AREA, jobs, per, (1u << per) - 1, a.planes, a.stride, a.cstride, a.picW, a.picH, a.fencPlanes, a.fstride, a.fcstride, acc, CU_PRED_ACC,
+                 metric == 1, tid, CU_PRED_WG);
+    if (tid < per)
+    {
+        const unsigned int* A = acc + tid * CU_PRED_ACC;
+        unsigned int sy = 0, sc = 0;
+        if (metric == 1) sy = A[0];
+        else
+        {
+            const int C = size >> 1, gY = size == 8 ? 1 : (size >> 4) * (size >> 4), gC = C <= 8 ? 1 : (C >> 4) * (C >> 4);
+            for (int k = 0; k < gY; k++) sy += (A[k] + 2) >> 2;
+            for (int pl = 1; pl < 3; pl++)
+            {
+                if (C == 4) sc += A[pl * 16] >> 1;
+                else for (int k = 0; k < gC; k++) sc += (A[pl * 16 + k] + 2) >> 2;
+            }
+        }
+        a.cost[2 * (first + tid)] = sy; a.cost[2 * (first + tid) + 1] = sc;
+    }
+}
+
+extern "C" int x265amd_cu_pred_cost(void* stream, const uint64_t* d_planes, intptr_t stride, intptr_t cstride, int pic_w, int pic_h,
+                                    const x265amd_mc_job* d_jobs, int n, const uint64_t* d_fenc_planes, intptr_t fenc_stride, intptr_t fenc_cstride,
+                                    uint32_t* d_cost, int cands_per_cu)
+{
+    if (n <= 0) return X265AMD_OK;
+    if (!d_planes || !d_jobs || !d_fenc_planes || !d_cost || cands_per_cu < 1 || cands_per_cu > CU_PRED_MAX_CANDS || n % cands_per_cu || xa_is_queue(stream))
+        return xa_fail(X265AMD_EINVAL, "x265amd_cu_pred_cost: bad arguments");
+    const XaArgsMc qa = { d_planes, (long)stride, (long)cstride, pic_w, pic_h, d_jobs, n, d_fenc_planes, (long)fenc_stride, (long)fenc_cstride, d_cost };
+    hipLaunchKernelGGL(k_cu_pred_cost, dim3(n / cands_per_cu), dim3(CU_PRED_WG), 0, (hipStream_t)stream, qa, cands_per_cu);
+    const hipError_t e = hipGetLastError();
+    if (e != hipSuccess) return xa_fail(X265AMD_EHIP, hipGetErrorString(e));
+    return X265AMD_OK;
+}
```

Result: slower. 96.61 (-6.1%).
